# idonahum/photoVerse

Hardware: NVIDIA B200
Metric: images/sec @50 steps 512^2; dual-branch cross-attn TFLOP/s as % of B200 peak (higher is better)
Workload: dtype bf16

## Files before the change

include/photoverse_b200.h:

```cpp
#ifndef PHOTOVERSE_B200_H_
#define PHOTOVERSE_B200_H_

#include <stdint.h>

#ifdef __cplusplus
extern "C" {
#endif

#define PV_ABI_VERSION 2

enum { PV_OK = 0, PV_ERR_INVALID = 1, PV_ERR_CUDA = 2, PV_ERR_UNSUPPORTED = 3 };
typedef enum { PV_F32 = 0, PV_BF16 = 1, PV_F16 = 2 } pv_dtype;

#define PV_KEYS_PAD 96
#define PV_IMG_KEY_OFFSET 80

int pv_version(void);
const char* pv_last_error(void);
unsigned long long pv_launch_count(void);
int pv_set_option(const char* name, int value);
int pv_debug_trace(void* buf, int capacity_events);

int pv_pack_weight(pv_dtype out_dt, const float* W, const float* lora_A, const float* lora_B, float scaling,
                   void* W_eff, int out_features, int in_features, int r, void* stream);

int pv_linear_fwd(pv_dtype dt, pv_dtype out_dt, const void* A, const void* W, const float* bias, void* D,
                  int64_t M, int64_t N, int64_t K, int64_t batch, int64_t lda, int64_t ldw, int64_t ldd,
                  int64_t strideA, int64_t strideW, int64_t strideBias, int64_t strideD, void* stream);

int64_t pv_kv_tile_bytes(pv_dtype dt, int C, int H, int Lt, int Li);
int pv_kv_pack_fwd(pv_dtype dt, const void* text, const void* img, const void* Wkv_text, const void* Wkv_img,
                   float* kv_text_ws, float* kv_img_ws, void* Kp, void* Vp, float* v_ip_norm, int B, int Lt, int Li,
                   int Dc, int C, int H, void* stream);

int64_t pv_dual_attn_sync_words(int B, int S);
int pv_dual_attn_fwd(pv_dtype dt, const void* X, const void* Wq, const void* Kp, const void* Vp, const void* Wo,
                     const float* bo, void* Y, float* ws_q, void* ws_o, float* stats, unsigned int* ws_sync, int B, int S,
                     int C, int H, int Lt, int Li, float w_text, float w_img, void* stream);

int pv_dual_attn_core_fwd(pv_dtype dt, const void* XorQ, const void* Wq, const void* Kp, const void* Vp, void* O,
                          float* stats, int B, int S, int C, int H, int Lt, int Li, float w_text, float w_img,
                          void* stream);

int pv_ln_lrelu_fwd(pv_dtype out_dt, const float* x, const float* gamma, const float* beta, void* y,
                    float* save_mean, float* save_rstd, int64_t rows, int cols, int64_t ldx, int64_t ldy,
                    int64_t rows_per_group, float eps, float slope, void* stream);
int pv_group_mean_fwd(pv_dtype in_dt, pv_dtype out_dt, const void* x, void* y, int64_t groups, int P, int cols,
                      int64_t ldy, void* stream);


int pv_pack_weight_t(pv_dtype out_dt, const float* W, const float* lora_A, const float* lora_B, float scaling,
                     void* W_eff_t, int out_features, int in_features, int r, void* stream);

int pv_transpose_2d(pv_dtype dt, const void* in, void* out, int64_t rows, int64_t cols, int64_t ldi, int64_t ldo, void* stream);

int64_t pv_linear_bwd_weight_ws_bytes(pv_dtype dt, int64_t M, int64_t N, int64_t K);
int pv_linear_bwd_weight(pv_dtype dt, const void* G, const void* X, float* dW, void* ws, int64_t M, int64_t N, int64_t K,
                         int64_t ldg, int64_t ldx, float alpha, float beta, void* stream);

int64_t pv_lora_bwd_ws_bytes(int64_t M, int in_features, int out_features, int r);
int pv_lora_bwd(pv_dtype dt, const void* X, const void* G, const float* lora_A, const float* lora_B, float scaling, float* dAB,
                void* ws, int64_t M, int in_features, int out_features, int r, int64_t ldx, int64_t ldg, void* stream);

int64_t pv_col_sum_ws_bytes(int64_t M, int64_t N);
int pv_col_sum(pv_dtype dt, const void* G, float* out, void* ws, int64_t M, int64_t N, int64_t ldg, void* stream);

int64_t pv_ln_lrelu_bwd_ws_bytes(int64_t groups, int64_t rows_per_group, int cols);
int pv_ln_lrelu_bwd(pv_dtype dt, const void* da, const float* x, const float* mean, const float* rstd, const float* gamma,
                    const float* beta, void* dx, float* dgamma, float* dbeta, void* ws, int64_t groups,
                    int64_t rows_per_group, int cols, float slope, void* stream);

int pv_group_mean_bwd(pv_dtype dt, const void* dy, void* dx, int64_t groups, int P, int cols, int64_t ldy, void* stream);

int64_t pv_dual_attn_bwd_ws_bytes(int B, int S, int C, int H, int Lt, int Li);
int pv_dual_attn_bwd(pv_dtype dt, const void* dO, const void* Q, const float* kv_text, const float* kv_img,
                     const float* stats, void* dQ, void* ws, int B, int S, int C, int H, int Lt, int Li, float w_text,
                     float w_img, void* stream);
int pv_kv_pack_bwd(pv_dtype dt, const void* ws, const float* kv_img, const float* v_ip_norm, const float* d_v_ip_norm,
                   void* dkv_text, void* dkv_img, int B, int S, int Lt, int Li, int C, int H, void* stream);

int pv_inject_concept_fwd(pv_dtype dt, const void* inputs_embeds, const void* concept, const int* placeholder_idx,
                          void* out, int B, int L, int T, int cols, void* stream);
int pv_inject_concept_bwd(pv_dtype dt, const void* d_out, const int* placeholder_idx, void* d_inputs_embeds,
                          void* d_concept, int B, int L, int T, int cols, void* stream);

int64_t pv_train_loss_ws_bytes(void);
int pv_train_loss_fwd(pv_dtype dt, const void* noise_pred, const void* noise, int64_t n, const void* concept, int64_t m,
                      const void* v_ip_norms, int64_t k, float w_text, float w_vis, float* out4, void* ws, void* stream);
int pv_train_loss_bwd(pv_dtype dt, const void* noise_pred, const void* noise, int64_t n, const void* concept, int64_t m, int64_t k,
                      float w_text, float w_vis, const float* d_loss, void* d_noise_pred, void* d_concept, void* d_v_ip_norms,
                      void* stream);

int64_t pv_self_attn_ws_bytes(int B, int S, int C, int heads);
int pv_self_attn_fwd(const void* q, const void* k, const void* v, int64_t ld, void* out, void* ws, int B, int S, int C,
                     int heads, void* stream);

int pv_dropout_bwd_acc(pv_dtype dt, void* dst, const void* src, const uint8_t* keep_mask, float alpha, int64_t n,
                       void* stream);

int64_t pv_group_norm_nhwc_ws_bytes(int64_t B, int64_t HW, int C, int groups);
int pv_group_norm_nhwc_fwd(pv_dtype dt, const void* x, const float* add_bc, const float* gamma, const float* beta, void* y,
                           float* save_stats, void* ws, int64_t B, int64_t HW, int C, int groups, float eps, int silu,
                           void* stream);
int pv_group_norm_nhwc_bwd(pv_dtype dt, const void* x, const float* add_bc, const void* dy, const float* stats,
                           const float* gamma, const float* beta, void* dx, void* ws, int64_t B, int64_t HW, int C, int groups,
                           int silu, void* stream);
int pv_add_bias_nhwc_fwd(pv_dtype dt, const void* a, const void* b, const float* bias, void* out, int64_t rows, int C,
                         void* stream);
int pv_layer_norm_fwd(pv_dtype dt, const void* x, const void* residual, void* sum_out, const float* gamma, const float* beta,
                      void* y, int64_t rows, int C, float eps, void* stream);
int pv_layer_norm_bwd(pv_dtype dt, const void* x, const void* dy, const float* gamma, void* dx, int64_t rows, int C, float eps,
                      void* stream);
int pv_geglu_fwd(pv_dtype dt, const void* h, void* y, int64_t M, int N, int64_t ldh, void* stream);
int pv_geglu_bwd(pv_dtype dt, const void* h, const void* dy, void* dh, int64_t M, int N, int64_t ldh, void* stream);
int pv_linear_geglu_fwd(pv_dtype dt, const void* x, const void* w_packed, const float* b_packed, void* y, int64_t M, int64_t N,
                        int64_t K, int64_t ldx, int64_t ldy, void* stream);

int pv_convert_fwd(pv_dtype in_dt, pv_dtype out_dt, const void* src, void* dst, int64_t n, void* stream);

#ifdef __cplusplus
}
#endif
#endif
```

photoverse_b200/_lib.py:

```python
import ctypes
import os
from ctypes import c_char_p, c_float, c_int, c_int64, c_ulonglong, c_void_p

_HERE = os.path.dirname(os.path.abspath(__file__))
LIB_PATH = os.environ.get("PV_LIB_PATH") or os.path.join(_HERE, "libphotoverse_b200.so")

PV_F32 = 0
PV_BF16 = 1
PV_F16 = 2
PV_KEYS_PAD = 96


class PhotoverseB200Error(RuntimeError):
    pass


_lib = None

_SIGNATURES = {
    "pv_version": (c_int, []),
    "pv_last_error": (c_char_p, []),
    "pv_launch_count": (c_ulonglong, []),
    "pv_set_option": (c_int, [c_char_p, c_int]),
    "pv_debug_trace": (c_int, [c_void_p, c_int]),
    "pv_pack_weight": (c_int, [c_int, c_void_p, c_void_p, c_void_p, c_float, c_void_p, c_int, c_int, c_int, c_void_p]),
    "pv_linear_fwd": (c_int, [c_int, c_int, c_void_p, c_void_p, c_void_p, c_void_p] + [c_int64] * 11 + [c_void_p]),
    "pv_kv_tile_bytes": (c_int64, [c_int, c_int, c_int, c_int, c_int]),
    "pv_kv_pack_fwd": (c_int, [c_int] + [c_void_p] * 9 + [c_int] * 6 + [c_void_p]),
    "pv_dual_attn_sync_words": (c_int64, [c_int, c_int]),
    "pv_dual_attn_fwd": (c_int, [c_int] + [c_void_p] * 11 + [c_int] * 6 + [c_float, c_float, c_void_p]),
    "pv_dual_attn_core_fwd": (c_int, [c_int] + [c_void_p] * 6 + [c_int] * 6 + [c_float, c_float, c_void_p]),
    "pv_ln_lrelu_fwd": (c_int, [c_int] + [c_void_p] * 6 + [c_int64, c_int, c_int64, c_int64, c_int64, c_float, c_float, c_void_p]),
    "pv_group_mean_fwd": (c_int, [c_int, c_int, c_void_p, c_void_p, c_int64, c_int, c_int, c_int64, c_void_p]),
    "pv_inject_concept_fwd": (c_int, [c_int, c_void_p, c_void_p, c_void_p, c_void_p, c_int, c_int, c_int, c_int, c_void_p]),
    "pv_inject_concept_bwd": (c_int, [c_int, c_void_p, c_void_p, c_void_p, c_void_p, c_int, c_int, c_int, c_int, c_void_p]),
    "pv_train_loss_ws_bytes": (c_int64, []),
    "pv_train_loss_fwd": (c_int, [c_int, c_void_p, c_void_p, c_int64, c_void_p, c_int64, c_void_p, c_int64, c_float, c_float, c_void_p,
                                  c_void_p, c_void_p]),
    "pv_train_loss_bwd": (c_int, [c_int, c_void_p, c_void_p, c_int64, c_void_p, c_int64, c_int64, c_float, c_float, c_void_p, c_void_p,
                                  c_void_p, c_void_p, c_void_p]),
    "pv_self_attn_ws_bytes": (c_int64, [c_int, c_int, c_int, c_int]),
    "pv_self_attn_fwd": (c_int, [c_void_p, c_void_p, c_void_p, c_int64, c_void_p, c_void_p, c_int, c_int, c_int, c_int, c_void_p]),
    "pv_dropout_bwd_acc": (c_int, [c_int, c_void_p, c_void_p, c_void_p, c_float, c_int64, c_void_p]),
    "pv_pack_weight_t": (c_int, [c_int, c_void_p, c_void_p, c_void_p, c_float, c_void_p, c_int, c_int, c_int, c_void_p]),
    "pv_transpose_2d": (c_int, [c_int, c_void_p, c_void_p, c_int64, c_int64, c_int64, c_int64, c_void_p]),
    "pv_linear_bwd_weight_ws_bytes": (c_int64, [c_int, c_int64, c_int64, c_int64]),
    "pv_linear_bwd_weight": (c_int, [c_int, c_void_p, c_void_p, c_void_p, c_void_p] + [c_int64] * 5 + [c_float, c_float, c_void_p]),
    "pv_lora_bwd_ws_bytes": (c_int64, [c_int64, c_int, c_int, c_int]),
    "pv_lora_bwd": (c_int, [c_int, c_void_p, c_void_p, c_void_p, c_void_p, c_float, c_void_p, c_void_p, c_int64, c_int, c_int, c_int,
                            c_int64, c_int64, c_void_p]),
    "pv_col_sum_ws_bytes": (c_int64, [c_int64, c_int64]),
    "pv_col_sum": (c_int, [c_int, c_void_p, c_void_p, c_void_p, c_int64, c_int64, c_int64, c_void_p]),
    "pv_ln_lrelu_bwd_ws_bytes": (c_int64, [c_int64, c_int64, c_int]),
    "pv_ln_lrelu_bwd": (c_int, [c_int] + [c_void_p] * 10 + [c_int64, c_int64, c_int, c_float, c_void_p]),
    "pv_group_mean_bwd": (c_int, [c_int, c_void_p, c_void_p, c_int64, c_int, c_int, c_int64, c_void_p]),
    "pv_dual_attn_bwd_ws_bytes": (c_int64, [c_int] * 6),
    "pv_dual_attn_bwd": (c_int, [c_int] + [c_void_p] * 7 + [c_int] * 6 + [c_float, c_float, c_void_p]),
    "pv_kv_pack_bwd": (c_int, [c_int] + [c_void_p] * 6 + [c_int] * 6 + [c_void_p]),
    "pv_group_norm_nhwc_ws_bytes": (c_int64, [c_int64, c_int64, c_int, c_int]),
    "pv_group_norm_nhwc_fwd": (c_int, [c_int] + [c_void_p] * 7 + [c_int64, c_int64, c_int, c_int, c_float, c_int, c_void_p]),
    "pv_group_norm_nhwc_bwd": (c_int, [c_int] + [c_void_p] * 8 + [c_int64, c_int64, c_int, c_int, c_int, c_void_p]),
    "pv_add_bias_nhwc_fwd": (c_int, [c_int, c_void_p, c_void_p, c_void_p, c_void_p, c_int64, c_int, c_void_p]),
    "pv_layer_norm_fwd": (c_int, [c_int, c_void_p, c_void_p, c_void_p, c_void_p, c_void_p, c_void_p, c_int64, c_int, c_float, c_void_p]),
    "pv_layer_norm_bwd": (c_int, [c_int, c_void_p, c_void_p, c_void_p, c_void_p, c_int64, c_int, c_float, c_void_p]),
    "pv_geglu_fwd": (c_int, [c_int, c_void_p, c_void_p, c_int64, c_int, c_int64, c_void_p]),
    "pv_geglu_bwd": (c_int, [c_int, c_void_p, c_void_p, c_void_p, c_int64, c_int, c_int64, c_void_p]),
    "pv_linear_geglu_fwd": (c_int, [c_int, c_void_p, c_void_p, c_void_p, c_void_p] + [c_int64] * 5 + [c_void_p]),
    "pv_convert_fwd": (c_int, [c_int, c_int, c_void_p, c_void_p, c_int64, c_void_p]),
}

REQUIRED_SYMBOLS = list(_SIGNATURES)


def lib() -> ctypes.CDLL:
    global _lib
    if _lib is None:
        if not os.path.exists(LIB_PATH):
            raise PhotoverseB200Error(
                f"{LIB_PATH} is missing: build it with `python -m photoverse_b200.build` "
                "(photoverse_b200 has no CPU / PyTorch fallback)")
        l = ctypes.CDLL(LIB_PATH)
        for name, (res, args) in _SIGNATURES.items():
            try:
                fn = getattr(l, name)
            except AttributeError:
                if name in REQUIRED_SYMBOLS:
                    raise PhotoverseB200Error(f"{LIB_PATH} does not export {name}")
                continue
            fn.restype = res
            fn.argtypes = args
        _lib = l
    return _lib


def check(rc: int, what: str = "") -> None:
    if rc != 0:
        msg = lib().pv_last_error()
        raise PhotoverseB200Error(f"{what or 'photoverse_b200 call'} failed (code {rc}): "
                                  f"{msg.decode() if msg else '?'}")


def launch_count() -> int:
    return int(lib().pv_launch_count())


def set_option(name: str, value: int) -> None:
    check(lib().pv_set_option(name.encode(), int(value)), f"pv_set_option({name})")
```

photoverse_b200/csrc/pv_api.cu:

```cuda
#include <string.h>

#include <mutex>
#include <unordered_map>

#include "pv_host.h"
#include "../../include/photoverse_b200.h"

namespace pv {

int gemm_bf16(const void* A, const void* W, const float* bias, void* D, bool out_f32, long long M, long long N,
              long long K, long long batch, long long lda, long long ldw, long long ldd, long long strideA,
              long long strideW, long long strideBias, long long strideD, cudaStream_t stream, bool w_static = false,
              bool f16 = false);
int gemm_f32(const float* A, const float* W, const float* bias, float* D, long long M, long long N, long long K,
             long long batch, long long lda, long long ldw, long long ldd, long long strideA, long long strideW,
             long long strideBias, long long strideD, cudaStream_t stream);
int dual_attn_core_bf16_persistent(const void* X, const void* Wq, const void* Kp, const void* Vp, void* O, float* stats,
                                   int B, int S, int C, int H, int Lt, int Li, float w_text, float w_img,
                                   cudaStream_t stream, bool f16);
bool dual_attn_pair_roles_supported(int S, int C, int H);
bool dual_attn_pair_roles_fused_supported(int S, int C, int H);
int dual_attn_core_bf16_pair_roles(const void* X, const void* Wq, const void* Kp, const void* Vp, void* O, float* stats,
                                   int B, int S, int C, int H, int Lt, int Li, float w_text, float w_img,
                                   cudaStream_t stream, const void* Wo, const float* bo, void* Y, unsigned int* sync,
                                   bool f16);
int dual_attn_core_bf16_pair(const void* X, const void* Wq, const void* Kp, const void* Vp, void* O, float* stats, int B,
                             int S, int C, int H, int Lt, int Li, float w_text, float w_img, cudaStream_t stream,
                             const void* Wo, const float* bo, void* Y, unsigned int* sync, bool f16);
int dual_attn_core_f32(const float* Q, const float* Kp, const float* Vp, float* O, float* stats, int B, int S, int C,
                       int H, int Lt, int Li, float w_text, float w_img, cudaStream_t stream);
static int64_t attn_kv_tile_bytes(int d) { return static_cast<int64_t>(PV_KEYS_PAD) * ((d + 15) / 16 * 16) * 2; }
int pack_weight(pv_dtype out_dt, const float* W, const float* A, const float* Bm, float scaling, void* out, int out_f,
                int in_f, int r, cudaStream_t stream);
int kv_pack(pv_dtype dt, const float* kv_text, const float* kv_img, void* Kp, void* Vp, float* v_ip_norm, int B, int Lt,
            int Li, int C, int H, cudaStream_t stream);
int ln_lrelu(pv_dtype out_dt, const float* x, const float* gamma, const float* beta, void* y, float* save_mean,
             float* save_rstd, long long rows, int cols, long long ldx, long long ldy, long long rows_per_group,
             float eps, float slope, cudaStream_t stream);
int group_mean(pv_dtype in_dt, pv_dtype out_dt, const void* x, void* y, long long groups, int P, int cols, long long ldy,
               cudaStream_t stream);

int pack_weight_t(bool out_bf16, const float* W, const float* A, const float* Bm, float scaling, void* out, int out_f,
                  int in_f, int r, cudaStream_t stream);
int transpose_2d(bool bf16, const void* in, void* out, long long R, long long Cc, long long ldi, long long ldo, cudaStream_t stream);
long long wgrad_ws_bytes(bool bf16, long long M, long long N, long long K);
int linear_bwd_weight(bool bf16, const void* G, const void* X, float* dW, void* ws, long long M, long long N, long long K,
                      long long ldg, long long ldx, float alpha, float beta, cudaStream_t stream);
long long colsum_ws_bytes(long long M, long long N);
int col_sum(bool bf16, const void* G, float* out, void* ws, long long M, long long N, long long ldg, cudaStream_t stream);
long long ln_bwd_ws_bytes(long long groups, long long rows_per_group, int cols);
int ln_lrelu_bwd(bool bf16, const void* da, const float* x, const float* mean, const float* rstd, const float* gamma,
                 const float* beta, void* dx, float* dgamma, float* dbeta, void* ws, long long groups,
                 long long rows_per_group, int cols, float slope, cudaStream_t stream);
int group_mean_bwd(bool bf16, const void* dy, void* dx, long long groups, int P, int cols, long long ldy, cudaStream_t stream);
int attn_bwd_chunks(int S);
long long self_attn_ws_bytes(int B, int S, int C, int H);
int self_attn_fwd_bf16(const void* q, const void* k, const void* v, long long ld, void* out, void* ws, int B, int S, int C, int H,
                       cudaStream_t stream);
long long train_loss_ws_bytes();
int train_loss_fwd(bool bf16, const void* pred, const void* target, long long n, const void* concept, long long m, const void* vnorm,
                   long long k, float w_text, float w_vis, float* out4, void* ws, cudaStream_t stream);
int train_loss_bwd(bool bf16, const void* pred, const void* target, long long n, const void* concept, long long m, long long k,
                   float w_text, float w_vis, const float* gloss, void* d_pred, void* d_concept, void* d_vnorm, cudaStream_t stream);
bool lora_bwd_supported(int in_f, int out_f, int r);
long long lora_bwd_ws_bytes(long long M, int in_f, int out_f, int r);
int lora_bwd(bool bf16, const void* X, const void* G, const float* A, const float* Bm, float scaling, float* dAB, void* ws,
             long long M, int in_f, int out_f, int r, long long ldx, long long ldg, cudaStream_t stream);
int attn_bwd_chunks_used(bool bf16, int S, int d);
int dual_attn_bwd(bool bf16, const void* dO, const void* Q, const float* kv_text, const float* kv_img, const float* stats,
                  void* dQ, float* part, int B, int S, int C, int H, int Lt, int Li, float w_text, float w_img,
                  cudaStream_t stream);
int kv_pack_bwd(bool bf16, const float* part, const float* kv_img, const float* v_ip_norm, const float* d_vnorm,
                void* dkv_text, void* dkv_img, int nchunk, int B, int Lt, int Li, int C, int H, cudaStream_t stream);

int inject_concept_fwd(bool bf16, const void* in, const void* concept, const int* idx, void* out, int B, int L, int T,
                       int cols, cudaStream_t stream);
int inject_concept_bwd(bool bf16, const void* dout, const int* idx, void* din, void* dconcept, int B, int L, int T, int cols,
                       cudaStream_t stream);
long long group_norm_nhwc_ws_bytes(long long B, long long HW, int C, int G);
int group_norm_nhwc(const void* x, const float* add_bc, const float* gamma, const float* beta, void* y, float* save_stats,
                    void* ws, long long B, long long HW, int C, int G, float eps, bool silu, cudaStream_t stream);
int group_norm_nhwc_bwd(const void* x, const float* add_bc, const void* dy, const float* stats, const float* gamma,
                        const float* beta, void* dx, void* ws, long long B, long long HW, int C, int G, bool silu,
                        cudaStream_t stream);
int add_bias_nhwc(const void* a, const void* b, const float* bias, void* out, long long rows, int C, cudaStream_t stream);
int layer_norm_bf16(const void* x, const void* res, void* sum_out, const float* gamma, const float* beta, void* y, long long rows,
                    int C, float eps, cudaStream_t stream);
int layer_norm_bwd_bf16(const void* x, const void* dy, const float* gamma, void* dx, long long rows, int C, float eps,
                        cudaStream_t stream);
int geglu(const void* h, void* y, long long M, int N, long long ldh, cudaStream_t stream);
int linear_geglu_bf16(const void* x, const void* Wp, const float* bp, void* y, long long M, long long N, long long K,
                      long long ldx, long long ldy, cudaStream_t stream);
int geglu_bwd(const void* h, const void* dy, void* dh, long long M, int N, long long ldh, cudaStream_t stream);
int dropout_bwd_acc(bool bf16, void* dst, const void* src, const uint8_t* mask, float alpha, long long n,
                    cudaStream_t stream);

std::atomic<unsigned long long> g_launches{0};
int g_opt_epi_swizzle = 1;
int g_opt_force_bn = 0;
int g_opt_gemm_two_cta = 1;
int g_opt_pdl = 1;
int g_opt_gemm_persistent = 1;
int g_opt_fuse_out = 1;
int g_opt_bwd_mma = 1;
unsigned long long* g_attn3_trace = nullptr;
int g_attn3_trace_cap = 0;
int g_opt_bwd_tc = 1;
int g_opt_sattn_poly = 2;
int g_opt_attn6_prefetch = 1;
int g_opt_attn6_token = 1;
int g_opt_trace_block = 0;
static thread_local std::string t_error;

void set_error(const std::string& msg) { t_error = msg; }
const char* last_error_cstr() { return t_error.c_str(); }

int sm_count() {
  static std::atomic<int> cache[64];
  int dev = 0;
  if (cudaGetDevice(&dev) != cudaSuccess || dev < 0 || dev >= 64) return 148;
  int n = cache[dev].load(std::memory_order_relaxed);
  if (n == 0) {
    if (cudaDeviceGetAttribute(&n, cudaDevAttrMultiProcessorCount, dev) != cudaSuccess || n <= 0) n = 148;
    cache[dev].store(n, std::memory_order_relaxed);
  }
  return n;
}

cudaError_t set_max_smem_once_impl(const void* kern, int bytes, bool max_carveout) {
  static std::mutex mu;
  static std::unordered_map<uint64_t, int> done;
  int dev = 0;
  cudaError_t e = cudaGetDevice(&dev);
  if (e != cudaSuccess) return e;
  const uint64_t key = reinterpret_cast<uint64_t>(kern) * 131u + static_cast<uint64_t>(dev);
  std::lock_guard<std::mutex> lk(mu);
  auto it = done.find(key);
  if (it != done.end() && it->second >= bytes) return cudaSuccess;
  e = cudaFuncSetAttribute(kern, cudaFuncAttributeMaxDynamicSharedMemorySize, bytes);
  if (e == cudaSuccess && max_carveout)
    e = cudaFuncSetAttribute(kern, cudaFuncAttributePreferredSharedMemoryCarveout, cudaSharedmemCarveoutMaxShared);
  if (e == cudaSuccess) done[key] = bytes;
  return e;
}

typedef CUresult (*EncodeTiledFn)(CUtensorMap*, CUtensorMapDataType, cuuint32_t, void*, const cuuint64_t*,
                                  const cuuint64_t*, const cuuint32_t*, const cuuint32_t*, CUtensorMapInterleave,
                                  CUtensorMapSwizzle, CUtensorMapL2promotion, CUtensorMapFloatOOBfill);

static EncodeTiledFn get_encode_fn() {
  static EncodeTiledFn fn = nullptr;
  static std::once_flag once;
  std::call_once(once, [] {
    void* p = nullptr;
    cudaDriverEntryPointQueryResult qres;
    if (cudaGetDriverEntryPoint("cuTensorMapEncodeTiled", &p, cudaEnableDefault, &qres) == cudaSuccess &&
        qres == cudaDriverEntryPointSuccess)
      fn = reinterpret_cast<EncodeTiledFn>(p);
  });
  return fn;
}

struct TmapKey {
  uint64_t v[12];
  bool operator==(const TmapKey& o) const { return memcmp(v, o.v, sizeof(v)) == 0; }
};
struct TmapKeyHash {
  size_t operator()(const TmapKey& k) const {
    uint64_t h = 1469598103934665603ull;
    for (uint64_t x : k.v) { h ^= x; h *= 1099511628211ull; }
    return static_cast<size_t>(h);
  }
};

int make_tmap_3d(CUtensorMap* out, const void* base, int elem_bytes, uint64_t d0, uint64_t d1, uint64_t d2,
                 uint64_t stride1_bytes, uint64_t stride2_bytes, uint32_t b0, uint32_t b1, uint32_t b2, Swz swz, bool f16) {
  static std::mutex mu;
  static std::unordered_map<TmapKey, CUtensorMap, TmapKeyHash> cache;
  TmapKey key = {{reinterpret_cast<uint64_t>(base), static_cast<uint64_t>(elem_bytes), d0, d1, d2, stride1_bytes,
                  stride2_bytes, b0, b1, b2, static_cast<uint64_t>(swz), static_cast<uint64_t>(f16)}};
  {
    std::lock_guard<std::mutex> lk(mu);
    auto it = cache.find(key);
    if (it != cache.end()) { *out = it->second; return 0; }
  }
  EncodeTiledFn fn = get_encode_fn();
  if (!fn) { set_error("cuTensorMapEncodeTiled unavailable (no CUDA driver / device)"); return 1; }
  CUtensorMapDataType dt = elem_bytes != 2 ? CU_TENSOR_MAP_DATA_TYPE_FLOAT32
                           : f16       ? CU_TENSOR_MAP_DATA_TYPE_FLOAT16 : CU_TENSOR_MAP_DATA_TYPE_BFLOAT16;
  cuuint64_t dims[3] = {d0, d1, d2};
  cuuint64_t strides[2] = {stride1_bytes, stride2_bytes};
  cuuint32_t box[3] = {b0, b1, b2};
  cuuint32_t estr[3] = {1, 1, 1};
  CUtensorMapSwizzle sw = swz == Swz::B128 ? CU_TENSOR_MAP_SWIZZLE_128B
                          : swz == Swz::B64 ? CU_TENSOR_MAP_SWIZZLE_64B : CU_TENSOR_MAP_SWIZZLE_NONE;
  CUresult r = fn(out, dt, 3, const_cast<void*>(base), dims, strides, box, estr, CU_TENSOR_MAP_INTERLEAVE_NONE, sw,
                  CU_TENSOR_MAP_L2_PROMOTION_L2_256B, CU_TENSOR_MAP_FLOAT_OOB_FILL_NONE);
  if (r != CUDA_SUCCESS) {
    char buf[384];
    snprintf(buf, sizeof(buf),
             "cuTensorMapEncodeTiled failed (%d): base=%p elem=%d dims=(%llu,%llu,%llu) strides=(%llu,%llu) box=(%u,%u,%u) swz=%d",
             (int)r, base, elem_bytes, (unsigned long long)d0, (unsigned long long)d1, (unsigned long long)d2,
             (unsigned long long)stride1_bytes, (unsigned long long)stride2_bytes, b0, b1, b2, (int)swz);
    set_error(buf);
    return 1;
  }
  {
    std::lock_guard<std::mutex> lk(mu);
    if (cache.size() > 8192) cache.clear();
    cache.emplace(key, *out);
  }
  return 0;
}

static inline cudaStream_t as_stream(void* s) { return static_cast<cudaStream_t>(s); }
static inline bool is_16bit(pv_dtype dt) { return dt == PV_BF16 || dt == PV_F16; }
#define PV_NO_F16(dt)                                                                                             \
  do {                                                                                                            \
    if ((dt) == PV_F16) PV_FAIL(PV_ERR_UNSUPPORTED, "PV_F16 is not supported (fp16 runs the inference path only)"); \
  } while (0)

static int attn_core_bf16(const void* X, const void* Wq, const void* Kp, const void* Vp, void* O, float* stats, int B,
                          int S, int C, int H, int Lt, int Li, float w_text, float w_img, cudaStream_t st, bool f16,
                          const void* Wo = nullptr, const float* bo = nullptr, void* Y = nullptr, unsigned int* sync = nullptr,
                          bool* fused = nullptr) {
  if (fused) *fused = false;
  if (S > 128) {
    const bool want = Wo != nullptr && sync != nullptr && (g_opt_fuse_out >= 2 || (g_opt_fuse_out == 1 && C <= 320));
    if (dual_attn_pair_roles_supported(S, C, H)) {
      const bool f = want && dual_attn_pair_roles_fused_supported(S, C, H);
      if (fused) *fused = f;
      return dual_attn_core_bf16_pair_roles(X, Wq, Kp, Vp, O, stats, B, S, C, H, Lt, Li, w_text, w_img, st,
                                            f ? Wo : nullptr, bo, f ? Y : nullptr, f ? sync : nullptr, f16);
    }
    if (fused) *fused = want;
    return dual_attn_core_bf16_pair(X, Wq, Kp, Vp, O, stats, B, S, C, H, Lt, Li, w_text, w_img, st, want ? Wo : nullptr, bo,
                                    want ? Y : nullptr, want ? sync : nullptr, f16);
  }
  return dual_attn_core_bf16_persistent(X, Wq, Kp, Vp, O, stats, B, S, C, H, Lt, Li, w_text, w_img, st, f16);
}

}

using namespace pv;

extern "C" {

int pv_version(void) { return PV_ABI_VERSION; }
const char* pv_last_error(void) { return last_error_cstr(); }
unsigned long long pv_launch_count(void) { return g_launches.load(std::memory_order_relaxed); }

int pv_set_option(const char* name, int value) {
  if (!name) PV_FAIL(PV_ERR_INVALID, "null option name");
  if (!strcmp(name, "epi_swizzle")) { g_opt_epi_swizzle = value; return PV_OK; }
  if (!strcmp(name, "force_bn")) { g_opt_force_bn = value; return PV_OK; }
  if (!strcmp(name, "gemm_two_cta")) { g_opt_gemm_two_cta = value; return PV_OK; }
  if (!strcmp(name, "gemm_persistent")) { g_opt_gemm_persistent = value; return PV_OK; }
  if (!strcmp(name, "fuse_out")) { g_opt_fuse_out = value; return PV_OK; }
  if (!strcmp(name, "pdl")) { g_opt_pdl = value; return PV_OK; }
  if (!strcmp(name, "bwd_mma")) { g_opt_bwd_mma = value; return PV_OK; }
  if (!strcmp(name, "bwd_tc")) { g_opt_bwd_tc = value; return PV_OK; }
  if (!strcmp(name, "sattn_poly")) { g_opt_sattn_poly = value; return PV_OK; }
  if (!strcmp(name, "attn6_prefetch")) { g_opt_attn6_prefetch = value; return PV_OK; }
  if (!strcmp(name, "attn6_token")) { g_opt_attn6_token = value; return PV_OK; }
  if (!strcmp(name, "trace_block")) { g_opt_trace_block = value; return PV_OK; }
  PV_FAIL(PV_ERR_INVALID, "unknown option '%s'", name);
}

int pv_debug_trace(void* buf, int capacity_events) {
#ifdef PV_TRACE
  g_attn3_trace = static_cast<unsigned long long*>(buf);
  g_attn3_trace_cap = buf ? capacity_events : 0;
  return PV_OK;
#else
  (void)capacity_events;
  if (buf == nullptr) return PV_OK;
  PV_FAIL(PV_ERR_INVALID, "this build records no device timeline (rebuild with PV_TRACE=1 python -m photoverse_b200.build --force)");
#endif
}

int pv_pack_weight(pv_dtype out_dt, const float* W, const float* lora_A, const float* lora_B, float scaling,
                   void* W_eff, int out_features, int in_features, int r, void* stream) {
  PV_REQUIRE(W && W_eff, "null pointer");
  PV_REQUIRE(out_dt == PV_F32 || is_16bit(out_dt), "unknown dtype %d", (int)out_dt);
  return pack_weight(out_dt, W, lora_A, lora_B, scaling, W_eff, out_features, in_features, r, as_stream(stream));
}

int pv_linear_fwd(pv_dtype dt, pv_dtype out_dt, const void* A, const void* W, const float* bias, void* D, int64_t M,
                  int64_t N, int64_t K, int64_t batch, int64_t lda, int64_t ldw, int64_t ldd, int64_t strideA,
                  int64_t strideW, int64_t strideBias, int64_t strideD, void* stream) {
  PV_REQUIRE(A && W && D, "null pointer");
  if (is_16bit(dt)) {
    PV_REQUIRE(out_dt == dt || out_dt == PV_F32, "%s inputs produce %s or fp32 outputs", dt == PV_F16 ? "PV_F16" : "PV_BF16",
               dt == PV_F16 ? "PV_F16" : "PV_BF16");
    return gemm_bf16(A, W, bias, D, out_dt == PV_F32, M, N, K, batch, lda, ldw, ldd, strideA, strideW, strideBias,
                     strideD, as_stream(stream), false, dt == PV_F16);
  }
  PV_REQUIRE(out_dt == PV_F32, "fp32 inputs produce fp32 outputs");
  return gemm_f32(static_cast<const float*>(A), static_cast<const float*>(W), bias, static_cast<float*>(D), M, N, K,
                  batch, lda, ldw, ldd, strideA, strideW, strideBias, strideD, as_stream(stream));
}

int64_t pv_kv_tile_bytes(pv_dtype dt, int C, int H, int Lt, int Li) {
  if (H <= 0 || C % H != 0) return -1;
  const int d = C / H;
  if (is_16bit(dt)) return attn_kv_tile_bytes(d);
  return static_cast<int64_t>(Lt + Li) * d * 4;
}

int pv_kv_pack_fwd(pv_dtype dt, const void* text, const void* img, const void* Wkv_text, const void* Wkv_img,
                   float* kv_text_ws, float* kv_img_ws, void* Kp, void* Vp, float* v_ip_norm, int B, int Lt, int Li,
                   int Dc, int C, int H, void* stream) {
  PV_REQUIRE(text && img && Wkv_text && Wkv_img && kv_text_ws && kv_img_ws && Kp && Vp && v_ip_norm, "null pointer");
  PV_REQUIRE(B > 0 && Lt >= 1 && Li >= 1 && Lt + Li <= PV_KEYS_PAD && C > 0 && H > 0 && C % H == 0 && Dc > 0,
             "bad shape B=%d Lt=%d Li=%d Dc=%d C=%d H=%d", B, Lt, Li, Dc, C, H);
  PV_REQUIRE(dt == PV_F32 || is_16bit(dt), "unknown dtype %d", (int)dt);
  PV_REQUIRE(!is_16bit(dt) || (Lt <= PV_IMG_KEY_OFFSET && Li <= PV_KEYS_PAD - PV_IMG_KEY_OFFSET),
             "PV_BF16 / PV_F16 tiles hold at most %d text and %d image keys (Lt=%d Li=%d)", PV_IMG_KEY_OFFSET,
             PV_KEYS_PAD - PV_IMG_KEY_OFFSET, Lt, Li);
  cudaStream_t st = as_stream(stream);
  int rc;
  if (is_16bit(dt)) {
    const bool f16 = dt == PV_F16;
    rc = gemm_bf16(text, Wkv_text, nullptr, kv_text_ws, true, (long long)B * Lt, 2 * C, Dc, 1, Dc, Dc, 2 * C, 0, 0, 0, 0, st,
                   false, f16);
    if (rc) return rc;
    rc = gemm_bf16(img, Wkv_img, nullptr, kv_img_ws, true, (long long)B * Li, 2 * C, Dc, 1, Dc, Dc, 2 * C, 0, 0, 0, 0, st,
                   false, f16);
    if (rc) return rc;
  } else {
    rc = gemm_f32(static_cast<const float*>(text), static_cast<const float*>(Wkv_text), nullptr, kv_text_ws,
                  (long long)B * Lt, 2 * C, Dc, 1, Dc, Dc, 2 * C, 0, 0, 0, 0, st);
    if (rc) return rc;
    rc = gemm_f32(static_cast<const float*>(img), static_cast<const float*>(Wkv_img), nullptr, kv_img_ws,
                  (long long)B * Li, 2 * C, Dc, 1, Dc, Dc, 2 * C, 0, 0, 0, 0, st);
    if (rc) return rc;
  }
  return kv_pack(dt, kv_text_ws, kv_img_ws, Kp, Vp, v_ip_norm, B, Lt, Li, C, H, st);
}

int64_t pv_dual_attn_sync_words(int B, int S) {
  if (B <= 0 || S <= 0) return -1;
  return 2ll * B * ((S + 255) / 256);
}

int pv_dual_attn_fwd(pv_dtype dt, const void* X, const void* Wq, const void* Kp, const void* Vp, const void* Wo,
                     const float* bo, void* Y, float* ws_q, void* ws_o, float* stats, unsigned int* ws_sync, int B, int S,
                     int C, int H, int Lt, int Li, float w_text, float w_img, void* stream) {
  PV_REQUIRE(X && Wq && Kp && Vp && Wo && Y && ws_o, "null pointer");
  cudaStream_t st = as_stream(stream);
  int rc;
  if (is_16bit(dt)) {
    const bool f16 = dt == PV_F16;
    bool fused = false;
    rc = attn_core_bf16(X, Wq, Kp, Vp, ws_o, stats, B, S, C, H, Lt, Li, w_text, w_img, st, f16, Wo, bo, Y, ws_sync, &fused);
    if (rc || fused) return rc;
    return gemm_bf16(ws_o, Wo, bo, Y, false, (long long)B * S, C, C, 1, C, C, C, 0, 0, 0, 0, st, true, f16);
  }
  PV_REQUIRE(dt == PV_F32, "unknown dtype %d", (int)dt);
  PV_REQUIRE(ws_q != nullptr, "PV_F32 needs the ws_q scratch");
  rc = gemm_f32(static_cast<const float*>(X), static_cast<const float*>(Wq), nullptr, ws_q, (long long)B * S, C, C, 1, C,
                C, C, 0, 0, 0, 0, st);
  if (rc) return rc;
  rc = dual_attn_core_f32(ws_q, static_cast<const float*>(Kp), static_cast<const float*>(Vp),
                          static_cast<float*>(ws_o), stats, B, S, C, H, Lt, Li, w_text, w_img, st);
  if (rc) return rc;
  return gemm_f32(static_cast<const float*>(ws_o), static_cast<const float*>(Wo), bo, static_cast<float*>(Y),
                  (long long)B * S, C, C, 1, C, C, C, 0, 0, 0, 0, st);
}

int pv_dual_attn_core_fwd(pv_dtype dt, const void* XorQ, const void* Wq, const void* Kp, const void* Vp, void* O,
                          float* stats, int B, int S, int C, int H, int Lt, int Li, float w_text, float w_img,
                          void* stream) {
  PV_REQUIRE(XorQ && Kp && Vp && O, "null pointer");
  if (is_16bit(dt)) {
    PV_REQUIRE(Wq != nullptr, "PV_BF16 / PV_F16 fuse the Q projection: Wq required");
    return attn_core_bf16(XorQ, Wq, Kp, Vp, O, stats, B, S, C, H, Lt, Li, w_text, w_img, as_stream(stream), dt == PV_F16);
  }
  PV_REQUIRE(dt == PV_F32, "unknown dtype %d", (int)dt);
  return dual_attn_core_f32(static_cast<const float*>(XorQ), static_cast<const float*>(Kp),
                            static_cast<const float*>(Vp), static_cast<float*>(O), stats, B, S, C, H, Lt, Li, w_text,
                            w_img, as_stream(stream));
}

int pv_ln_lrelu_fwd(pv_dtype out_dt, const float* x, const float* gamma, const float* beta, void* y, float* save_mean,
                    float* save_rstd, int64_t rows, int cols, int64_t ldx, int64_t ldy, int64_t rows_per_group,
                    float eps, float slope, void* stream) {
  PV_REQUIRE(x && gamma && beta && y, "null pointer");
  PV_REQUIRE(out_dt == PV_F32 || is_16bit(out_dt), "unknown dtype %d", (int)out_dt);
  return ln_lrelu(out_dt, x, gamma, beta, y, save_mean, save_rstd, rows, cols, ldx, ldy, rows_per_group, eps,
                  slope, as_stream(stream));
}

int pv_group_mean_fwd(pv_dtype in_dt, pv_dtype out_dt, const void* x, void* y, int64_t groups, int P, int cols,
                      int64_t ldy, void* stream) {
  PV_REQUIRE(x && y, "null pointer");
  PV_REQUIRE((in_dt == PV_F32 || is_16bit(in_dt)) && (out_dt == PV_F32 || is_16bit(out_dt)), "unknown dtype");
  PV_REQUIRE(!(is_16bit(in_dt) && is_16bit(out_dt) && in_dt != out_dt), "16-bit input and output must have one type");
  return group_mean(in_dt, out_dt, x, y, groups, P, cols, ldy, as_stream(stream));
}

int pv_pack_weight_t(pv_dtype out_dt, const float* W, const float* lora_A, const float* lora_B, float scaling,
                     void* W_eff_t, int out_features, int in_features, int r, void* stream) {
  PV_NO_F16(out_dt);
  PV_REQUIRE(W && W_eff_t, "null pointer");
  return pack_weight_t(out_dt == PV_BF16, W, lora_A, lora_B, scaling, W_eff_t, out_features, in_features, r, as_stream(stream));
}

int pv_transpose_2d(pv_dtype dt, const void* in, void* out, int64_t rows, int64_t cols, int64_t ldi, int64_t ldo, void* stream) {
  PV_NO_F16(dt);
  PV_REQUIRE(in && out, "null pointer");
  return transpose_2d(dt == PV_BF16, in, out, rows, cols, ldi, ldo, as_stream(stream));
}

int64_t pv_linear_bwd_weight_ws_bytes(pv_dtype dt, int64_t M, int64_t N, int64_t K) {
  if (dt == PV_F16) { set_error("pv_linear_bwd_weight_ws_bytes: PV_F16 is not supported (fp16 runs the inference path only)"); return -1; }
  return wgrad_ws_bytes(dt == PV_BF16, M, N, K);
}

int pv_linear_bwd_weight(pv_dtype dt, const void* G, const void* X, float* dW, void* ws, int64_t M, int64_t N, int64_t K,
                         int64_t ldg, int64_t ldx, float alpha, float beta, void* stream) {
  PV_NO_F16(dt);
  PV_REQUIRE(G && X && dW, "null pointer");
  return linear_bwd_weight(dt == PV_BF16, G, X, dW, ws, M, N, K, ldg, ldx, alpha, beta, as_stream(stream));
}

int64_t pv_lora_bwd_ws_bytes(int64_t M, int in_features, int out_features, int r) {
  if (M <= 0 || !lora_bwd_supported(in_features, out_features, r)) return -1;
  return lora_bwd_ws_bytes(M, in_features, out_features, r);
}

int pv_lora_bwd(pv_dtype dt, const void* X, const void* G, const float* lora_A, const float* lora_B, float scaling, float* dAB,
                void* ws, int64_t M, int in_features, int out_features, int r, int64_t ldx, int64_t ldg, void* stream) {
  PV_NO_F16(dt);
  PV_REQUIRE(X && G && lora_A && lora_B && dAB, "null pointer");
  return lora_bwd(dt == PV_BF16, X, G, lora_A, lora_B, scaling, dAB, ws, M, in_features, out_features, r, ldx, ldg, as_stream(stream));
}

int64_t pv_col_sum_ws_bytes(int64_t M, int64_t N) { return colsum_ws_bytes(M, N); }

int pv_col_sum(pv_dtype dt, const void* G, float* out, void* ws, int64_t M, int64_t N, int64_t ldg, void* stream) {
  PV_NO_F16(dt);
  PV_REQUIRE(G && out, "null pointer");
  return col_sum(dt == PV_BF16, G, out, ws, M, N, ldg, as_stream(stream));
}

int64_t pv_ln_lrelu_bwd_ws_bytes(int64_t groups, int64_t rows_per_group, int cols) {
  return ln_bwd_ws_bytes(groups, rows_per_group, cols);
}

int pv_ln_lrelu_bwd(pv_dtype dt, const void* da, const float* x, const float* mean, const float* rstd, const float* gamma,
                    const float* beta, void* dx, float* dgamma, float* dbeta, void* ws, int64_t groups,
                    int64_t rows_per_group, int cols, float slope, void* stream) {
  PV_NO_F16(dt);
  PV_REQUIRE(da && x && mean && rstd && gamma && beta && dx && dgamma && dbeta && ws, "null pointer");
  return ln_lrelu_bwd(dt == PV_BF16, da, x, mean, rstd, gamma, beta, dx, dgamma, dbeta, ws, groups, rows_per_group, cols,
                      slope, as_stream(stream));
}

int pv_group_mean_bwd(pv_dtype dt, const void* dy, void* dx, int64_t groups, int P, int cols, int64_t ldy, void* stream) {
  PV_NO_F16(dt);
  PV_REQUIRE(dy && dx, "null pointer");
  return group_mean_bwd(dt == PV_BF16, dy, dx, groups, P, cols, ldy, as_stream(stream));
}

int64_t pv_dual_attn_bwd_ws_bytes(int B, int S, int C, int H, int Lt, int Li) {
  if (H <= 0 || C % H != 0) return -1;
  return static_cast<int64_t>(attn_bwd_chunks(S)) * B * H * 2 * (Lt + Li) * (C / H) * 4;
}

int pv_dual_attn_bwd(pv_dtype dt, const void* dO, const void* Q, const float* kv_text, const float* kv_img,
                     const float* stats, void* dQ, void* ws, int B, int S, int C, int H, int Lt, int Li, float w_text,
                     float w_img, void* stream) {
  PV_NO_F16(dt);
  PV_REQUIRE(dO && Q && kv_text && kv_img && stats && dQ && ws, "null pointer");
  return dual_attn_bwd(dt == PV_BF16, dO, Q, kv_text, kv_img, stats, dQ, static_cast<float*>(ws), B, S, C, H, Lt, Li, w_text,
                       w_img, as_stream(stream));
}

int pv_kv_pack_bwd(pv_dtype dt, const void* ws, const float* kv_img, const float* v_ip_norm, const float* d_v_ip_norm,
                   void* dkv_text, void* dkv_img, int B, int S, int Lt, int Li, int C, int H, void* stream) {
  PV_NO_F16(dt);
  PV_REQUIRE(ws && kv_img && v_ip_norm && dkv_text && dkv_img, "null pointer");
  return kv_pack_bwd(dt == PV_BF16, static_cast<const float*>(ws), kv_img, v_ip_norm, d_v_ip_norm, dkv_text, dkv_img,
                     attn_bwd_chunks_used(dt == PV_BF16, S, H > 0 ? C / H : 0), B, Lt, Li, C, H, as_stream(stream));
}

int pv_inject_concept_fwd(pv_dtype dt, const void* inputs_embeds, const void* concept, const int* placeholder_idx,
                          void* out, int B, int L, int T, int cols, void* stream) {
  PV_NO_F16(dt);
  PV_REQUIRE(inputs_embeds && concept && placeholder_idx && out, "null pointer");
  return inject_concept_fwd(dt == PV_BF16, inputs_embeds, concept, placeholder_idx, out, B, L, T, cols, as_stream(stream));
}

int pv_inject_concept_bwd(pv_dtype dt, const void* d_out, const int* placeholder_idx, void* d_inputs_embeds,
                          void* d_concept, int B, int L, int T, int cols, void* stream) {
  PV_NO_F16(dt);
  PV_REQUIRE(d_out && placeholder_idx && d_inputs_embeds && d_concept, "null pointer");
  return inject_concept_bwd(dt == PV_BF16, d_out, placeholder_idx, d_inputs_embeds, d_concept, B, L, T, cols, as_stream(stream));
}

int64_t pv_train_loss_ws_bytes(void) { return train_loss_ws_bytes(); }

int pv_train_loss_fwd(pv_dtype dt, const void* noise_pred, const void* noise, int64_t n, const void* concept, int64_t m,
                      const void* v_ip_norms, int64_t k, float w_text, float w_vis, float* out4, void* ws, void* stream) {
  PV_NO_F16(dt);
  PV_REQUIRE(noise_pred && noise && out4 && (m == 0 || concept) && (k == 0 || v_ip_norms), "null pointer");
  return train_loss_fwd(dt == PV_BF16, noise_pred, noise, n, concept, m, v_ip_norms, k, w_text, w_vis, out4, ws, as_stream(stream));
}

int pv_train_loss_bwd(pv_dtype dt, const void* noise_pred, const void* noise, int64_t n, const void* concept, int64_t m, int64_t k,
                      float w_text, float w_vis, const float* d_loss, void* d_noise_pred, void* d_concept, void* d_v_ip_norms,
                      void* stream) {
  PV_NO_F16(dt);
  PV_REQUIRE(noise_pred && noise && d_loss && d_noise_pred && (m == 0 || (concept && d_concept)) && (k == 0 || d_v_ip_norms), "null pointer");
  return train_loss_bwd(dt == PV_BF16, noise_pred, noise, n, concept, m, k, w_text, w_vis, d_loss, d_noise_pred, d_concept,
                        d_v_ip_norms, as_stream(stream));
}

int64_t pv_self_attn_ws_bytes(int B, int S, int C, int heads) { return self_attn_ws_bytes(B, S, C, heads); }

int pv_self_attn_fwd(const void* q, const void* k, const void* v, int64_t ld, void* out, void* ws, int B, int S, int C,
                     int heads, void* stream) {
  PV_REQUIRE(q && k && v && out && ws, "null pointer");
  return self_attn_fwd_bf16(q, k, v, ld, out, ws, B, S, C, heads, as_stream(stream));
}

int pv_dropout_bwd_acc(pv_dtype dt, void* dst, const void* src, const uint8_t* keep_mask, float alpha, int64_t n,
                       void* stream) {
  PV_NO_F16(dt);
  PV_REQUIRE(dst && src && keep_mask, "null pointer");
  return dropout_bwd_acc(dt == PV_BF16, dst, src, keep_mask, alpha, n, as_stream(stream));
}

int64_t pv_group_norm_nhwc_ws_bytes(int64_t B, int64_t HW, int C, int groups) { return group_norm_nhwc_ws_bytes(B, HW, C, groups); }

int pv_group_norm_nhwc_fwd(pv_dtype dt, const void* x, const float* add_bc, const float* gamma, const float* beta, void* y,
                           float* save_stats, void* ws, int64_t B, int64_t HW, int C, int groups, float eps, int silu,
                           void* stream) {
  PV_NO_F16(dt);
  PV_REQUIRE(x && gamma && beta && y && ws, "null pointer");
  PV_REQUIRE(dt == PV_BF16, "bf16 activations only (the fp32 parity mode keeps the stock GroupNorm)");
  return group_norm_nhwc(x, add_bc, gamma, beta, y, save_stats, ws, B, HW, C, groups, eps, silu != 0, as_stream(stream));
}

int pv_group_norm_nhwc_bwd(pv_dtype dt, const void* x, const float* add_bc, const void* dy, const float* stats,
                           const float* gamma, const float* beta, void* dx, void* ws, int64_t B, int64_t HW, int C, int groups,
                           int silu, void* stream) {
  PV_NO_F16(dt);
  PV_REQUIRE(x && dy && stats && gamma && beta && dx && ws, "null pointer");
  PV_REQUIRE(dt == PV_BF16, "bf16 activations only");
  return group_norm_nhwc_bwd(x, add_bc, dy, stats, gamma, beta, dx, ws, B, HW, C, groups, silu != 0, as_stream(stream));
}

int pv_add_bias_nhwc_fwd(pv_dtype dt, const void* a, const void* b, const float* bias, void* out, int64_t rows, int C,
                         void* stream) {
  PV_NO_F16(dt);
  PV_REQUIRE(a && b && bias && out, "null pointer");
  PV_REQUIRE(dt == PV_BF16, "bf16 activations only");
  return add_bias_nhwc(a, b, bias, out, rows, C, as_stream(stream));
}

int pv_layer_norm_fwd(pv_dtype dt, const void* x, const void* residual, void* sum_out, const float* gamma, const float* beta,
                      void* y, int64_t rows, int C, float eps, void* stream) {
  PV_NO_F16(dt);
  PV_REQUIRE(x && gamma && beta && y, "null pointer");
  PV_REQUIRE(dt == PV_BF16, "bf16 activations only");
  return layer_norm_bf16(x, residual, sum_out, gamma, beta, y, rows, C, eps, as_stream(stream));
}

int pv_layer_norm_bwd(pv_dtype dt, const void* x, const void* dy, const float* gamma, void* dx, int64_t rows, int C, float eps,
                      void* stream) {
  PV_NO_F16(dt);
  PV_REQUIRE(x && dy && gamma && dx, "null pointer");
  PV_REQUIRE(dt == PV_BF16, "bf16 activations only");
  return layer_norm_bwd_bf16(x, dy, gamma, dx, rows, C, eps, as_stream(stream));
}

int pv_geglu_fwd(pv_dtype dt, const void* h, void* y, int64_t M, int N, int64_t ldh, void* stream) {
  PV_NO_F16(dt);
  PV_REQUIRE(h && y, "null pointer");
  PV_REQUIRE(dt == PV_BF16, "bf16 activations only");
  return geglu(h, y, M, N, ldh, as_stream(stream));
}

int pv_geglu_bwd(pv_dtype dt, const void* h, const void* dy, void* dh, int64_t M, int N, int64_t ldh, void* stream) {
  PV_NO_F16(dt);
  PV_REQUIRE(h && dy && dh, "null pointer");
  PV_REQUIRE(dt == PV_BF16, "bf16 activations only");
  return geglu_bwd(h, dy, dh, M, N, ldh, as_stream(stream));
}

int pv_linear_geglu_fwd(pv_dtype dt, const void* x, const void* w_packed, const float* b_packed, void* y, int64_t M, int64_t N,
                        int64_t K, int64_t ldx, int64_t ldy, void* stream) {
  PV_NO_F16(dt);
  PV_REQUIRE(x && w_packed && y, "null pointer");
  PV_REQUIRE(dt == PV_BF16, "bf16 activations only");
  return linear_geglu_bf16(x, w_packed, b_packed, y, M, N, K, ldx, ldy, as_stream(stream));
}

}
```

photoverse_b200/csrc/pv_backbone.cu:

```cuda
#include "pv_common.cuh"
#include "pv_host.h"
#include "../../include/photoverse_b200.h"

namespace pv {

constexpr int GN_THREADS_MAX = 512;
constexpr int GN_MAX_G = 64;
constexpr int GN_UNROLL = 4;

__device__ __forceinline__ void bf16x8_unpack(const uint4& v, float* f) {
  const uint32_t w[4] = {v.x, v.y, v.z, v.w};
#pragma unroll
  for (int i = 0; i < 4; ++i) {
    f[2 * i] = __uint_as_float(w[i] << 16);
    f[2 * i + 1] = __uint_as_float(w[i] & 0xffff0000u);
  }
}
__device__ __forceinline__ uint4 bf16x8_pack(const float* f) {
  uint32_t w[4];
#pragma unroll
  for (int i = 0; i < 4; ++i) {
    const __nv_bfloat162 p = __floats2bfloat162_rn(f[2 * i], f[2 * i + 1]);
    w[i] = *reinterpret_cast<const uint32_t*>(&p);
  }
  return make_uint4(w[0], w[1], w[2], w[3]);
}

__global__ void __launch_bounds__(GN_THREADS_MAX)
gn_stats_nhwc_kernel(const __nv_bfloat16* __restrict__ x, const float* __restrict__ addv, float* __restrict__ part,
                     long long HW, int C, int G, int rows_per_cta, int k) {
  extern __shared__ float gn_smem[];
  const int vecs = C >> 3;
  const int v = threadIdx.x % vecs;
  const int pl = threadIdx.x / vecs;
  const int b = blockIdx.y;
  const int cpg = C / G;
  const __nv_bfloat16* xb = x + static_cast<size_t>(b) * HW * C;
  float shift[8];
#pragma unroll
  for (int j = 0; j < 8; ++j) {
    const int c = v * 8 + j, c0 = (c / cpg) * cpg;
    shift[j] = __bfloat162float(xb[c0]);
    if (addv != nullptr) shift[j] += addv[static_cast<size_t>(b) * C + c0] - addv[static_cast<size_t>(b) * C + c];
  }
  float s[8], q[8];
#pragma unroll
  for (int j = 0; j < 8; ++j) s[j] = q[j] = 0.f;
  const long long p0 = static_cast<long long>(blockIdx.x) * rows_per_cta;
  const long long p1 = p0 + rows_per_cta < HW ? p0 + rows_per_cta : HW;
  const uint4* xv = reinterpret_cast<const uint4*>(xb);
  for (long long p = p0 + pl; p < p1; p += static_cast<long long>(GN_UNROLL) * k) {
    uint4 raw[GN_UNROLL];
#pragma unroll
    for (int u = 0; u < GN_UNROLL; ++u) {
      const long long pp = p + static_cast<long long>(u) * k;
      if (pp < p1) raw[u] = __ldg(xv + pp * vecs + v);
    }
#pragma unroll
    for (int u = 0; u < GN_UNROLL; ++u) {
      if (p + static_cast<long long>(u) * k < p1) {
        float f[8];
        bf16x8_unpack(raw[u], f);
#pragma unroll
        for (int j = 0; j < 8; ++j) {
          const float d = f[j] - shift[j];
          s[j] += d;
          q[j] = fmaf(d, d, q[j]);
        }
      }
    }
  }
  float* ss = gn_smem;
  float* sq = gn_smem + k * C;
#pragma unroll
  for (int j = 0; j < 8; ++j) {
    ss[pl * C + v * 8 + j] = s[j];
    sq[pl * C + v * 8 + j] = q[j];
  }
  __syncthreads();
  for (int c = threadIdx.x; c < C; c += blockDim.x) {
    float a = 0.f, d = 0.f;
    for (int l = 0; l < k; ++l) {
      a += ss[l * C + c];
      d += sq[l * C + c];
    }
    ss[c] = a;
    sq[c] = d;
  }
  __syncthreads();
  for (int g = threadIdx.x; g < G; g += blockDim.x) {
    float a = 0.f, d = 0.f;
    for (int c = g * cpg; c < (g + 1) * cpg; ++c) {
      a += ss[c];
      d += sq[c];
    }
    float* o = part + ((static_cast<size_t>(b) * gridDim.x + blockIdx.x) * G + g) * 2;
    o[0] = a;
    o[1] = d;
  }
}

template <bool SILU>
__global__ void __launch_bounds__(GN_THREADS_MAX)
gn_apply_nhwc_kernel(const __nv_bfloat16* __restrict__ x, const float* __restrict__ addv, const float* __restrict__ part,
                     const float* __restrict__ gamma, const float* __restrict__ beta, __nv_bfloat16* __restrict__ y,
                     float* __restrict__ save_stats, long long HW, int C, int G, int stat_chunks, int rows_per_cta, int k,
                     float eps) {
  __shared__ float s_mean[GN_MAX_G], s_rstd[GN_MAX_G];
  const int vecs = C >> 3;
  const int v = threadIdx.x % vecs;
  const int pl = threadIdx.x / vecs;
  const int b = blockIdx.y;
  const int cpg = C / G;
  const __nv_bfloat16* xb = x + static_cast<size_t>(b) * HW * C;
  for (int g = threadIdx.x; g < G; g += blockDim.x) {
    float a = 0.f, d = 0.f;
    const float* pp = part + (static_cast<size_t>(b) * stat_chunks * G + g) * 2;
    for (int c = 0; c < stat_chunks; ++c) {
      a += pp[static_cast<size_t>(c) * G * 2];
      d += pp[static_cast<size_t>(c) * G * 2 + 1];
    }
    const float n = static_cast<float>(HW) * static_cast<float>(cpg);
    const float m = a / n;
    const float var = fmaxf(d / n - m * m, 0.f);
    s_mean[g] = __bfloat162float(xb[g * cpg]) + (addv != nullptr ? addv[static_cast<size_t>(b) * C + g * cpg] : 0.f) + m;
    s_rstd[g] = rsqrtf(var + eps);
    if (save_stats != nullptr && blockIdx.x == 0) {
      save_stats[(static_cast<size_t>(b) * G + g) * 2] = s_mean[g];
      save_stats[(static_cast<size_t>(b) * G + g) * 2 + 1] = s_rstd[g];
    }
  }
  __syncthreads();
  float sc[8], sf[8];
#pragma unroll
  for (int j = 0; j < 8; ++j) {
    const int c = v * 8 + j;
    const int g = c / cpg;
    sc[j] = __ldg(gamma + c) * s_rstd[g];
    const float a = addv != nullptr ? addv[static_cast<size_t>(b) * C + c] : 0.f;
    sf[j] = fmaf(a - s_mean[g], sc[j], __ldg(beta + c));
  }
  const long long p0 = static_cast<long long>(blockIdx.x) * rows_per_cta;
  const long long p1 = p0 + rows_per_cta < HW ? p0 + rows_per_cta : HW;
  const uint4* xv = reinterpret_cast<const uint4*>(xb);
  uint4* yv = reinterpret_cast<uint4*>(y + static_cast<size_t>(b) * HW * C);
  for (long long p = p0 + pl; p < p1; p += static_cast<long long>(GN_UNROLL) * k) {
    uint4 raw[GN_UNROLL];
#pragma unroll
    for (int u = 0; u < GN_UNROLL; ++u) {
      const long long pp = p + static_cast<long long>(u) * k;
      if (pp < p1) raw[u] = __ldg(xv + pp * vecs + v);
    }
#pragma unroll
    for (int u = 0; u < GN_UNROLL; ++u) {
      const long long pp = p + static_cast<long long>(u) * k;
      if (pp < p1) {
        float f[8];
        bf16x8_unpack(raw[u], f);
#pragma unroll
        for (int j = 0; j < 8; ++j) {
          float t = fmaf(f[j], sc[j], sf[j]);
          if (SILU) t = __fdividef(t, 1.f + __expf(-t));
          f[j] = t;
        }
        yv[pp * vecs + v] = bf16x8_pack(f);
      }
    }
  }
}

static void gn_geometry(long long B, long long HW, int C, int* k, int* chunks, int* rows_per_cta) {
  (void)B;
  const int vecs = C / 8;
  int kk = GN_THREADS_MAX / vecs;
  if (kk < 1) kk = 1;
  if (kk > 16) kk = 16;
  if (kk > HW) kk = static_cast<int>(HW);
  long long rows = (65536 + 2ll * C - 1) / (2ll * C);
  rows = (rows + kk - 1) / kk * kk;
  if (rows > HW) rows = (HW + kk - 1) / kk * kk;
  *k = kk;
  *rows_per_cta = static_cast<int>(rows);
  *chunks = static_cast<int>((HW + rows - 1) / rows);
}

long long group_norm_nhwc_ws_bytes(long long B, long long HW, int C, int G) {
  if (B <= 0 || HW <= 0 || C <= 0 || G <= 0 || C % 8 != 0 || C % G != 0 || G > GN_MAX_G || C / 8 > GN_THREADS_MAX) return -1;
  int k, chunks, rows;
  gn_geometry(B, HW, C, &k, &chunks, &rows);
  return B * chunks * G * 2ll * static_cast<long long>(sizeof(float));
}

int group_norm_nhwc(const void* x, const float* add_bc, const float* gamma, const float* beta, void* y, float* save_stats,
                    void* ws, long long B, long long HW, int C, int G, float eps, bool silu, cudaStream_t stream) {
  PV_REQUIRE(group_norm_nhwc_ws_bytes(B, HW, C, G) >= 0,
             "need C %% 8 == 0, C %% G == 0, G <= %d, C <= %d (B=%lld HW=%lld C=%d G=%d)", GN_MAX_G, 8 * GN_THREADS_MAX, B, HW, C, G);
  PV_REQUIRE(B <= 65535, "batch too large for one launch (B=%lld)", B);
  PV_REQUIRE((reinterpret_cast<uintptr_t>(x) | reinterpret_cast<uintptr_t>(y)) % 16 == 0, "x / y must be 16-byte aligned");
  int k, chunks, rows;
  gn_geometry(B, HW, C, &k, &chunks, &rows);
  const int threads = (C / 8) * k;
  const size_t smem = 2ull * k * C * sizeof(float);
  auto stats = gn_stats_nhwc_kernel;
  if (smem > 48 * 1024) PV_CUDA(set_max_smem_once(stats, static_cast<int>(smem)));
  stats<<<dim3(chunks, static_cast<unsigned>(B)), threads, smem, stream>>>(static_cast<const __nv_bfloat16*>(x), add_bc,
                                                                            static_cast<float*>(ws), HW, C, G, rows, k);
  PV_LAUNCHED();
  if (silu)
    gn_apply_nhwc_kernel<true><<<dim3(chunks, static_cast<unsigned>(B)), threads, 0, stream>>>(
        static_cast<const __nv_bfloat16*>(x), add_bc, static_cast<const float*>(ws), gamma, beta, static_cast<__nv_bfloat16*>(y),
        save_stats, HW, C, G, chunks, rows, k, eps);
  else
    gn_apply_nhwc_kernel<false><<<dim3(chunks, static_cast<unsigned>(B)), threads, 0, stream>>>(
        static_cast<const __nv_bfloat16*>(x), add_bc, static_cast<const float*>(ws), gamma, beta, static_cast<__nv_bfloat16*>(y),
        save_stats, HW, C, G, chunks, rows, k, eps);
  PV_LAUNCHED();
  return PV_OK;
}

struct GnBwdChan {
  float g[8], bt[8], xs[8], xo[8];
};
__device__ __forceinline__ void gn_bwd_chan(GnBwdChan& ch, const float* __restrict__ stats, const float* __restrict__ addv,
                                            const float* __restrict__ gamma, const float* __restrict__ beta, int b, int v,
                                            int C, int G, int cpg) {
#pragma unroll
  for (int j = 0; j < 8; ++j) {
    const int c = v * 8 + j;
    const int g = c / cpg;
    const float mean = stats[(static_cast<size_t>(b) * G + g) * 2], rstd = stats[(static_cast<size_t>(b) * G + g) * 2 + 1];
    const float a = addv != nullptr ? addv[static_cast<size_t>(b) * C + c] : 0.f;
    ch.g[j] = __ldg(gamma + c);
    ch.bt[j] = __ldg(beta + c);
    ch.xs[j] = rstd;
    ch.xo[j] = (a - mean) * rstd;
  }
}
template <bool SILU>
__device__ __forceinline__ float gn_dz(float dy, float z) {
  if (!SILU) return dy;
  const float sg = __fdividef(1.f, 1.f + __expf(-z));
  return dy * sg * fmaf(z, 1.f - sg, 1.f);
}

template <bool SILU>
__global__ void __launch_bounds__(GN_THREADS_MAX)
gn_bwd_stats_nhwc_kernel(const __nv_bfloat16* __restrict__ x, const float* __restrict__ addv, const __nv_bfloat16* __restrict__ dy,
                         const float* __restrict__ stats, const float* __restrict__ gamma, const float* __restrict__ beta,
                         float* __restrict__ part, long long HW, int C, int G, int rows_per_cta, int k) {
  extern __shared__ float gn_smem[];
  const int vecs = C >> 3;
  const int v = threadIdx.x % vecs;
  const int pl = threadIdx.x / vecs;
  const int b = blockIdx.y;
  const int cpg = C / G;
  GnBwdChan ch;
  gn_bwd_chan(ch, stats, addv, gamma, beta, b, v, C, G, cpg);
  float s[8], q[8];
#pragma unroll
  for (int j = 0; j < 8; ++j) s[j] = q[j] = 0.f;
  const long long p0 = static_cast<long long>(blockIdx.x) * rows_per_cta;
  const long long p1 = p0 + rows_per_cta < HW ? p0 + rows_per_cta : HW;
  const uint4* xv = reinterpret_cast<const uint4*>(x + static_cast<size_t>(b) * HW * C);
  const uint4* dv = reinterpret_cast<const uint4*>(dy + static_cast<size_t>(b) * HW * C);
  for (long long p = p0 + pl; p < p1; p += 2ll * k) {
    uint4 rx[2], rd[2];
#pragma unroll
    for (int u = 0; u < 2; ++u) {
      const long long pp = p + static_cast<long long>(u) * k;
      if (pp < p1) {
        rx[u] = __ldg(xv + pp * vecs + v);
        rd[u] = __ldg(dv + pp * vecs + v);
      }
    }
#pragma unroll
    for (int u = 0; u < 2; ++u) {
      if (p + static_cast<long long>(u) * k < p1) {
        float f[8], d[8];
        bf16x8_unpack(rx[u], f);
        bf16x8_unpack(rd[u], d);
#pragma unroll
        for (int j = 0; j < 8; ++j) {
          const float xh = fmaf(f[j], ch.xs[j], ch.xo[j]);
          const float t = gn_dz<SILU>(d[j], fmaf(xh, ch.g[j], ch.bt[j])) * ch.g[j];
          s[j] += t;
          q[j] = fmaf(t, xh, q[j]);
        }
      }
    }
  }
  float* ss = gn_smem;
  float* sq = gn_smem + k * C;
#pragma unroll
  for (int j = 0; j < 8; ++j) {
    ss[pl * C + v * 8 + j] = s[j];
    sq[pl * C + v * 8 + j] = q[j];
  }
  __syncthreads();
  for (int c = threadIdx.x; c < C; c += blockDim.x) {
    float a = 0.f, d = 0.f;
    for (int l = 0; l < k; ++l) {
      a += ss[l * C + c];
      d += sq[l * C + c];
    }
    ss[c] = a;
    sq[c] = d;
  }
  __syncthreads();
  for (int g = threadIdx.x; g < G; g += blockDim.x) {
    float a = 0.f, d = 0.f;
    for (int c = g * cpg; c < (g + 1) * cpg; ++c) {
      a += ss[c];
      d += sq[c];
    }
    float* o = part + ((static_cast<size_t>(b) * gridDim.x + blockIdx.x) * G + g) * 2;
    o[0] = a;
    o[1] = d;
  }
}

template <bool SILU>
__global__ void __launch_bounds__(GN_THREADS_MAX)
gn_bwd_apply_nhwc_kernel(const __nv_bfloat16* __restrict__ x, const float* __restrict__ addv, const __nv_bfloat16* __restrict__ dy,
                         const float* __restrict__ stats, const float* __restrict__ part, const float* __restrict__ gamma,
                         const float* __restrict__ beta, __nv_bfloat16* __restrict__ dx, long long HW, int C, int G,
                         int stat_chunks, int rows_per_cta, int k) {
  __shared__ float s_m1[GN_MAX_G], s_m2[GN_MAX_G];
  const int vecs = C >> 3;
  const int v = threadIdx.x % vecs;
  const int pl = threadIdx.x / vecs;
  const int b = blockIdx.y;
  const int cpg = C / G;
  for (int g = threadIdx.x; g < G; g += blockDim.x) {
    float a = 0.f, d = 0.f;
    const float* pp = part + (static_cast<size_t>(b) * stat_chunks * G + g) * 2;
    for (int c = 0; c < stat_chunks; ++c) {
      a += pp[static_cast<size_t>(c) * G * 2];
      d += pp[static_cast<size_t>(c) * G * 2 + 1];
    }
    const float n = static_cast<float>(HW) * static_cast<float>(cpg);
    s_m1[g] = a / n;
    s_m2[g] = d / n;
  }
  GnBwdChan ch;
  gn_bwd_chan(ch, stats, addv, gamma, beta, b, v, C, G, cpg);
  __syncthreads();
  float m1[8], m2[8];
#pragma unroll
  for (int j = 0; j < 8; ++j) {
    const int g = (v * 8 + j) / cpg;
    m1[j] = s_m1[g];
    m2[j] = s_m2[g];
  }
  const long long p0 = static_cast<long long>(blockIdx.x) * rows_per_cta;
  const long long p1 = p0 + rows_per_cta < HW ? p0 + rows_per_cta : HW;
  const uint4* xv = reinterpret_cast<const uint4*>(x + static_cast<size_t>(b) * HW * C);
  const uint4* dv = reinterpret_cast<const uint4*>(dy + static_cast<size_t>(b) * HW * C);
  uint4* ov = reinterpret_cast<uint4*>(dx + static_cast<size_t>(b) * HW * C);
  for (long long p = p0 + pl; p < p1; p += 2ll * k) {
    uint4 rx[2], rd[2];
#pragma unroll
    for (int u = 0; u < 2; ++u) {
      const long long pp = p + static_cast<long long>(u) * k;
      if (pp < p1) {
        rx[u] = __ldg(xv + pp * vecs + v);
        rd[u] = __ldg(dv + pp * vecs + v);
      }
    }
#pragma unroll
    for (int u = 0; u < 2; ++u) {
      const long long pp = p + static_cast<long long>(u) * k;
      if (pp < p1) {
        float f[8], d[8];
        bf16x8_unpack(rx[u], f);
        bf16x8_unpack(rd[u], d);
#pragma unroll
        for (int j = 0; j < 8; ++j) {
          const float xh = fmaf(f[j], ch.xs[j], ch.xo[j]);
          const float t = gn_dz<SILU>(d[j], fmaf(xh, ch.g[j], ch.bt[j])) * ch.g[j];
          f[j] = ch.xs[j] * (t - m1[j] - xh * m2[j]);
        }
        ov[pp * vecs + v] = bf16x8_pack(f);
      }
    }
  }
}

int group_norm_nhwc_bwd(const void* x, const float* add_bc, const void* dy, const float* stats, const float* gamma,
                        const float* beta, void* dx, void* ws, long long B, long long HW, int C, int G, bool silu,
                        cudaStream_t stream) {
  PV_REQUIRE(group_norm_nhwc_ws_bytes(B, HW, C, G) >= 0,
             "need C %% 8 == 0, C %% G == 0, G <= %d, C <= %d (B=%lld HW=%lld C=%d G=%d)", GN_MAX_G, 8 * GN_THREADS_MAX, B, HW, C, G);
  PV_REQUIRE(B <= 65535, "batch too large for one launch (B=%lld)", B);
  PV_REQUIRE((reinterpret_cast<uintptr_t>(x) | reinterpret_cast<uintptr_t>(dy) | reinterpret_cast<uintptr_t>(dx)) % 16 == 0,
             "x / dy / dx must be 16-byte aligned");
  int k, chunks, rows;
  gn_geometry(B, HW, C, &k, &chunks, &rows);
  const int threads = (C / 8) * k;
  const size_t smem = 2ull * k * C * sizeof(float);
  const dim3 grid(chunks, static_cast<unsigned>(B));
  const __nv_bfloat16* xx = static_cast<const __nv_bfloat16*>(x);
  const __nv_bfloat16* dd = static_cast<const __nv_bfloat16*>(dy);
  if (silu) {
    gn_bwd_stats_nhwc_kernel<true><<<grid, threads, smem, stream>>>(xx, add_bc, dd, stats, gamma, beta, static_cast<float*>(ws), HW, C, G, rows, k);
    PV_LAUNCHED();
    gn_bwd_apply_nhwc_kernel<true><<<grid, threads, 0, stream>>>(xx, add_bc, dd, stats, static_cast<const float*>(ws), gamma, beta,
                                                                 static_cast<__nv_bfloat16*>(dx), HW, C, G, chunks, rows, k);
  } else {
    gn_bwd_stats_nhwc_kernel<false><<<grid, threads, smem, stream>>>(xx, add_bc, dd, stats, gamma, beta, static_cast<float*>(ws), HW, C, G, rows, k);
    PV_LAUNCHED();
    gn_bwd_apply_nhwc_kernel<false><<<grid, threads, 0, stream>>>(xx, add_bc, dd, stats, static_cast<const float*>(ws), gamma, beta,
                                                                  static_cast<__nv_bfloat16*>(dx), HW, C, G, chunks, rows, k);
  }
  PV_LAUNCHED();
  return PV_OK;
}

__global__ void __launch_bounds__(256)
add_bias_nhwc_kernel(const __nv_bfloat16* a, const __nv_bfloat16* b, const float* __restrict__ bias, __nv_bfloat16* out,
                     long long rows, int C) {
  const int vecs = C >> 3;
  const long long total = rows * vecs;
  for (long long i = static_cast<long long>(blockIdx.x) * blockDim.x + threadIdx.x; i < total;
       i += static_cast<long long>(gridDim.x) * blockDim.x) {
    const int v = static_cast<int>(i % vecs);
    float fa[8], fb[8];
    bf16x8_unpack(reinterpret_cast<const uint4*>(a)[i], fa);
    bf16x8_unpack(reinterpret_cast<const uint4*>(b)[i], fb);
    const float4 b0 = __ldg(reinterpret_cast<const float4*>(bias) + 2 * v), b1 = __ldg(reinterpret_cast<const float4*>(bias) + 2 * v + 1);
    const float bb[8] = {b0.x, b0.y, b0.z, b0.w, b1.x, b1.y, b1.z, b1.w};
#pragma unroll
    for (int j = 0; j < 8; ++j) fa[j] = fa[j] + (fb[j] + bb[j]);
    reinterpret_cast<uint4*>(out)[i] = bf16x8_pack(fa);
  }
}

int add_bias_nhwc(const void* a, const void* b, const float* bias, void* out, long long rows, int C, cudaStream_t stream) {
  PV_REQUIRE(rows > 0 && C > 0 && C % 8 == 0, "need C %% 8 == 0 (rows=%lld C=%d)", rows, C);
  PV_REQUIRE((reinterpret_cast<uintptr_t>(a) | reinterpret_cast<uintptr_t>(b) | reinterpret_cast<uintptr_t>(out) |
              reinterpret_cast<uintptr_t>(bias)) % 16 == 0, "pointers must be 16-byte aligned");
  const long long total = rows * (C / 8);
  long long blocks = (total + 255) / 256;
  const long long cap = 8ll * sm_count();
  if (blocks > cap) blocks = cap;
  add_bias_nhwc_kernel<<<static_cast<unsigned>(blocks), 256, 0, stream>>>(static_cast<const __nv_bfloat16*>(a), static_cast<const __nv_bfloat16*>(b),
                                                                         bias, static_cast<__nv_bfloat16*>(out), rows, C);
  PV_LAUNCHED();
  return PV_OK;
}

template <int NV>
__global__ void __launch_bounds__(256)
layer_norm_bf16_kernel(const __nv_bfloat16* __restrict__ x, const __nv_bfloat16* __restrict__ res,
                       __nv_bfloat16* __restrict__ sum_out, const float* __restrict__ gamma, const float* __restrict__ beta,
                       __nv_bfloat16* __restrict__ y, long long rows, int C, float eps) {
  const long long row = static_cast<long long>(blockIdx.x) * (blockDim.x >> 5) + (threadIdx.x >> 5);
  if (row >= rows) return;
  const int lane = threadIdx.x & 31;
  const int vecs = C >> 3;
  const uint4* xr = reinterpret_cast<const uint4*>(x + row * C);
  float f[NV][8];
  float s = 0.f;
#pragma unroll
  for (int i = 0; i < NV; ++i) {
    const int idx = i * 32 + lane;
    if (idx < vecs) {
      bf16x8_unpack(__ldg(xr + idx), f[i]);
      if (res != nullptr) {
        float r[8];
        bf16x8_unpack(__ldg(reinterpret_cast<const uint4*>(res + row * C) + idx), r);
#pragma unroll
        for (int j = 0; j < 8; ++j) f[i][j] += r[j];
        const uint4 packed = bf16x8_pack(f[i]);
        reinterpret_cast<uint4*>(sum_out + row * C)[idx] = packed;
        bf16x8_unpack(packed, f[i]);
      }
#pragma unroll
      for (int j = 0; j < 8; ++j) s += f[i][j];
    }
  }
#pragma unroll
  for (int o = 16; o > 0; o >>= 1) s += __shfl_xor_sync(0xffffffffu, s, o);
  const float mean = s / static_cast<float>(C);
  float ss = 0.f;
#pragma unroll
  for (int i = 0; i < NV; ++i) {
    if (i * 32 + lane < vecs) {
#pragma unroll
      for (int j = 0; j < 8; ++j) {
        const float d = f[i][j] - mean;
        ss = fmaf(d, d, ss);
      }
    }
  }
#pragma unroll
  for (int o = 16; o > 0; o >>= 1) ss += __shfl_xor_sync(0xffffffffu, ss, o);
  const float rstd = rsqrtf(ss / static_cast<float>(C) + eps);
  uint4* yr = reinterpret_cast<uint4*>(y + row * C);
#pragma unroll
  for (int i = 0; i < NV; ++i) {
    const int idx = i * 32 + lane;
    if (idx < vecs) {
      const float4 g0 = __ldg(reinterpret_cast<const float4*>(gamma) + 2 * idx), g1 = __ldg(reinterpret_cast<const float4*>(gamma) + 2 * idx + 1);
      const float4 b0 = __ldg(reinterpret_cast<const float4*>(beta) + 2 * idx), b1 = __ldg(reinterpret_cast<const float4*>(beta) + 2 * idx + 1);
      const float gg[8] = {g0.x, g0.y, g0.z, g0.w, g1.x, g1.y, g1.z, g1.w};
      const float bb[8] = {b0.x, b0.y, b0.z, b0.w, b1.x, b1.y, b1.z, b1.w};
      float o[8];
#pragma unroll
      for (int j = 0; j < 8; ++j) o[j] = fmaf((f[i][j] - mean) * rstd, gg[j], bb[j]);
      yr[idx] = bf16x8_pack(o);
    }
  }
}

int layer_norm_bf16(const void* x, const void* res, void* sum_out, const float* gamma, const float* beta, void* y, long long rows,
                    int C, float eps, cudaStream_t stream) {
  PV_REQUIRE(rows > 0 && C > 0 && C % 8 == 0 && C <= 8 * 32 * 5, "need C %% 8 == 0 and C <= 1280 (rows=%lld C=%d)", rows, C);
  PV_REQUIRE((res == nullptr) == (sum_out == nullptr), "res and sum_out go together");
  PV_REQUIRE((reinterpret_cast<uintptr_t>(x) | reinterpret_cast<uintptr_t>(y) | reinterpret_cast<uintptr_t>(gamma) |
              reinterpret_cast<uintptr_t>(beta) | reinterpret_cast<uintptr_t>(res) | reinterpret_cast<uintptr_t>(sum_out)) % 16 == 0,
             "pointers must be 16-byte aligned");
  const int nv = (C / 8 + 31) / 32;
  const unsigned blocks = static_cast<unsigned>((rows + 7) / 8);
  const __nv_bfloat16* xx = static_cast<const __nv_bfloat16*>(x);
  const __nv_bfloat16* rr = static_cast<const __nv_bfloat16*>(res);
  __nv_bfloat16* so = static_cast<__nv_bfloat16*>(sum_out);
  __nv_bfloat16* yy = static_cast<__nv_bfloat16*>(y);
  switch (nv) {
    case 1: layer_norm_bf16_kernel<1><<<blocks, 256, 0, stream>>>(xx, rr, so, gamma, beta, yy, rows, C, eps); break;
    case 2: layer_norm_bf16_kernel<2><<<blocks, 256, 0, stream>>>(xx, rr, so, gamma, beta, yy, rows, C, eps); break;
    case 3: layer_norm_bf16_kernel<3><<<blocks, 256, 0, stream>>>(xx, rr, so, gamma, beta, yy, rows, C, eps); break;
    case 4: layer_norm_bf16_kernel<4><<<blocks, 256, 0, stream>>>(xx, rr, so, gamma, beta, yy, rows, C, eps); break;
    default: layer_norm_bf16_kernel<5><<<blocks, 256, 0, stream>>>(xx, rr, so, gamma, beta, yy, rows, C, eps); break;
  }
  PV_LAUNCHED();
  return PV_OK;
}

template <int NV>
__global__ void __launch_bounds__(256)
layer_norm_bwd_bf16_kernel(const __nv_bfloat16* __restrict__ x, const __nv_bfloat16* __restrict__ dy, const float* __restrict__ gamma,
                           __nv_bfloat16* __restrict__ dx, long long rows, int C, float eps) {
  const long long row = static_cast<long long>(blockIdx.x) * (blockDim.x >> 5) + (threadIdx.x >> 5);
  if (row >= rows) return;
  const int lane = threadIdx.x & 31;
  const int vecs = C >> 3;
  const uint4* xr = reinterpret_cast<const uint4*>(x + row * C);
  const uint4* dr = reinterpret_cast<const uint4*>(dy + row * C);
  float f[NV][8], t[NV][8];
  float s = 0.f;
#pragma unroll
  for (int i = 0; i < NV; ++i) {
    const int idx = i * 32 + lane;
    if (idx < vecs) {
      bf16x8_unpack(__ldg(xr + idx), f[i]);
      bf16x8_unpack(__ldg(dr + idx), t[i]);
#pragma unroll
      for (int j = 0; j < 8; ++j) s += f[i][j];
    }
  }
#pragma unroll
  for (int o = 16; o > 0; o >>= 1) s += __shfl_xor_sync(0xffffffffu, s, o);
  const float mean = s / static_cast<float>(C);
  float ss = 0.f;
#pragma unroll
  for (int i = 0; i < NV; ++i) {
    if (i * 32 + lane < vecs) {
#pragma unroll
      for (int j = 0; j < 8; ++j) {
        const float d = f[i][j] - mean;
        ss = fmaf(d, d, ss);
      }
    }
  }
#pragma unroll
  for (int o = 16; o > 0; o >>= 1) ss += __shfl_xor_sync(0xffffffffu, ss, o);
  const float rstd = rsqrtf(ss / static_cast<float>(C) + eps);
  float s1 = 0.f, s2 = 0.f;
#pragma unroll
  for (int i = 0; i < NV; ++i) {
    const int idx = i * 32 + lane;
    if (idx < vecs) {
      const float4 g0 = __ldg(reinterpret_cast<const float4*>(gamma) + 2 * idx), g1 = __ldg(reinterpret_cast<const float4*>(gamma) + 2 * idx + 1);
      const float gg[8] = {g0.x, g0.y, g0.z, g0.w, g1.x, g1.y, g1.z, g1.w};
#pragma unroll
      for (int j = 0; j < 8; ++j) {
        f[i][j] = (f[i][j] - mean) * rstd;
        t[i][j] *= gg[j];
        s1 += t[i][j];
        s2 = fmaf(t[i][j], f[i][j], s2);
      }
    }
  }
#pragma unroll
  for (int o = 16; o > 0; o >>= 1) {
    s1 += __shfl_xor_sync(0xffffffffu, s1, o);
    s2 += __shfl_xor_sync(0xffffffffu, s2, o);
  }
  const float m1 = s1 / static_cast<float>(C), m2 = s2 / static_cast<float>(C);
  uint4* outr = reinterpret_cast<uint4*>(dx + row * C);
#pragma unroll
  for (int i = 0; i < NV; ++i) {
    const int idx = i * 32 + lane;
    if (idx < vecs) {
      float o[8];
#pragma unroll
      for (int j = 0; j < 8; ++j) o[j] = rstd * (t[i][j] - m1 - f[i][j] * m2);
      outr[idx] = bf16x8_pack(o);
    }
  }
}

int layer_norm_bwd_bf16(const void* x, const void* dy, const float* gamma, void* dx, long long rows, int C, float eps,
                        cudaStream_t stream) {
  PV_REQUIRE(rows > 0 && C > 0 && C % 8 == 0 && C <= 8 * 32 * 5, "need C %% 8 == 0 and C <= 1280 (rows=%lld C=%d)", rows, C);
  PV_REQUIRE((reinterpret_cast<uintptr_t>(x) | reinterpret_cast<uintptr_t>(dy) | reinterpret_cast<uintptr_t>(dx) |
              reinterpret_cast<uintptr_t>(gamma)) % 16 == 0, "pointers must be 16-byte aligned");
  const int nv = (C / 8 + 31) / 32;
  const unsigned blocks = static_cast<unsigned>((rows + 7) / 8);
  const __nv_bfloat16* xx = static_cast<const __nv_bfloat16*>(x);
  const __nv_bfloat16* dd = static_cast<const __nv_bfloat16*>(dy);
  __nv_bfloat16* oo = static_cast<__nv_bfloat16*>(dx);
  switch (nv) {
    case 1: layer_norm_bwd_bf16_kernel<1><<<blocks, 256, 0, stream>>>(xx, dd, gamma, oo, rows, C, eps); break;
    case 2: layer_norm_bwd_bf16_kernel<2><<<blocks, 256, 0, stream>>>(xx, dd, gamma, oo, rows, C, eps); break;
    case 3: layer_norm_bwd_bf16_kernel<3><<<blocks, 256, 0, stream>>>(xx, dd, gamma, oo, rows, C, eps); break;
    case 4: layer_norm_bwd_bf16_kernel<4><<<blocks, 256, 0, stream>>>(xx, dd, gamma, oo, rows, C, eps); break;
    default: layer_norm_bwd_bf16_kernel<5><<<blocks, 256, 0, stream>>>(xx, dd, gamma, oo, rows, C, eps); break;
  }
  PV_LAUNCHED();
  return PV_OK;
}

__global__ void __launch_bounds__(256)
geglu_kernel(const __nv_bfloat16* __restrict__ h, __nv_bfloat16* __restrict__ y, long long M, int N, long long ldh) {
  const int vecs = N >> 3;
  const long long total = M * vecs;
  for (long long i = static_cast<long long>(blockIdx.x) * blockDim.x + threadIdx.x; i < total;
       i += static_cast<long long>(gridDim.x) * blockDim.x) {
    const long long m = i / vecs;
    const int v = static_cast<int>(i - m * vecs);
    const uint4* row = reinterpret_cast<const uint4*>(h + m * ldh);
    float a[8], g[8];
    bf16x8_unpack(__ldg(row + v), a);
    bf16x8_unpack(__ldg(row + vecs + v), g);
#pragma unroll
    for (int j = 0; j < 8; ++j) {
      const float ge = __bfloat162float(__float2bfloat16_rn(0.5f * g[j] * (1.f + erff(g[j] * 0.70710678118654752f))));
      a[j] *= ge;
    }
    reinterpret_cast<uint4*>(y + m * N)[v] = bf16x8_pack(a);
  }
}

int geglu(const void* h, void* y, long long M, int N, long long ldh, cudaStream_t stream) {
  PV_REQUIRE(M > 0 && N > 0 && N % 8 == 0 && ldh >= 2ll * N && ldh % 8 == 0, "need N %% 8 == 0 and ldh >= 2N, ldh %% 8 == 0 (M=%lld N=%d ldh=%lld)", M, N, ldh);
  PV_REQUIRE((reinterpret_cast<uintptr_t>(h) | reinterpret_cast<uintptr_t>(y)) % 16 == 0, "h / y must be 16-byte aligned");
  const long long total = M * (N / 8);
  long long blocks = (total + 255) / 256;
  const long long cap = 8ll * sm_count();
  if (blocks > cap) blocks = cap;
  geglu_kernel<<<static_cast<unsigned>(blocks), 256, 0, stream>>>(static_cast<const __nv_bfloat16*>(h), static_cast<__nv_bfloat16*>(y), M, N, ldh);
  PV_LAUNCHED();
  return PV_OK;
}

__global__ void __launch_bounds__(256)
geglu_bwd_kernel(const __nv_bfloat16* __restrict__ h, const __nv_bfloat16* __restrict__ dy, __nv_bfloat16* __restrict__ dh,
                 long long M, int N, long long ldh) {
  const int vecs = N >> 3;
  const long long total = M * vecs;
  for (long long i = static_cast<long long>(blockIdx.x) * blockDim.x + threadIdx.x; i < total;
       i += static_cast<long long>(gridDim.x) * blockDim.x) {
    const long long m = i / vecs;
    const int v = static_cast<int>(i - m * vecs);
    const uint4* row = reinterpret_cast<const uint4*>(h + m * ldh);
    float a[8], g[8], d[8];
    bf16x8_unpack(__ldg(row + v), a);
    bf16x8_unpack(__ldg(row + vecs + v), g);
    bf16x8_unpack(__ldg(reinterpret_cast<const uint4*>(dy + m * N) + v), d);
#pragma unroll
    for (int j = 0; j < 8; ++j) {
      const float cdf = 0.5f * (1.f + erff(g[j] * 0.70710678118654752f));
      const float pdf = 0.3989422804014327f * __expf(-0.5f * g[j] * g[j]);
      const float da = d[j] * (g[j] * cdf);
      const float dg = d[j] * a[j] * fmaf(g[j], pdf, cdf);
      a[j] = da;
      g[j] = dg;
    }
    uint4* orow = reinterpret_cast<uint4*>(dh + m * 2 * N);
    orow[v] = bf16x8_pack(a);
    orow[vecs + v] = bf16x8_pack(g);
  }
}

int geglu_bwd(const void* h, const void* dy, void* dh, long long M, int N, long long ldh, cudaStream_t stream) {
  PV_REQUIRE(M > 0 && N > 0 && N % 8 == 0 && ldh >= 2ll * N && ldh % 8 == 0, "need N %% 8 == 0 and ldh >= 2N, ldh %% 8 == 0 (M=%lld N=%d ldh=%lld)", M, N, ldh);
  PV_REQUIRE((reinterpret_cast<uintptr_t>(h) | reinterpret_cast<uintptr_t>(dy) | reinterpret_cast<uintptr_t>(dh)) % 16 == 0,
             "h / dy / dh must be 16-byte aligned");
  const long long total = M * (N / 8);
  long long blocks = (total + 255) / 256;
  const long long cap = 8ll * sm_count();
  if (blocks > cap) blocks = cap;
  geglu_bwd_kernel<<<static_cast<unsigned>(blocks), 256, 0, stream>>>(static_cast<const __nv_bfloat16*>(h), static_cast<const __nv_bfloat16*>(dy),
                                                                     static_cast<__nv_bfloat16*>(dh), M, N, ldh);
  PV_LAUNCHED();
  return PV_OK;
}

}
```

photoverse_b200/csrc/pv_gemm3.cu:

```cuda
#include "pv_common.cuh"
#include "pv_outproj.cuh"
#include "pv_host.h"
#include "../../include/photoverse_b200.h"

namespace pv {

constexpr int G3_THREADS = 384;

template <typename Cfg, int EPI, typename T>
__global__ void __cluster_dims__(2, 1, 1) __launch_bounds__(G3_THREADS, 1)
gemm3_pair_persistent_kernel(const __grid_constant__ CUtensorMap tmA, const __grid_constant__ CUtensorMap tmW,
                             const __grid_constant__ CUtensorMap tmD, const float* __restrict__ bias, int G, int V, int K,
                             int w_static) {
  extern __shared__ uint8_t smem_raw[];
  uint8_t* smem = reinterpret_cast<uint8_t*>((reinterpret_cast<uintptr_t>(smem_raw) + 1023) & ~uintptr_t(1023));
  uint64_t* bars = reinterpret_cast<uint64_t*>(smem + (Cfg::BYTES + 15) / 16 * 16);
  uint32_t* tmem_slot = reinterpret_cast<uint32_t*>(bars + OP_BAR_BYTES / 8 + (EPI == OP_EPI_GEGLU ? 1 : 0));
  const int warp = threadIdx.x >> 5;
  const int pair = blockIdx.x >> 1;
  const int npairs = gridDim.x >> 1;
  int g, u0, u1;
  if constexpr (EPI == OP_EPI_GEGLU) {
    const long long T = static_cast<long long>(G) * V;
    u0 = static_cast<int>(T * pair / npairs);
    u1 = static_cast<int>(T * (pair + 1) / npairs);
    g = u0 / V;
  } else {
    g = pair % G;
    const int r_pair = pair / G;
    const int npair_g = (npairs - g + G - 1) / G;
    u0 = static_cast<int>((static_cast<long long>(V) * r_pair) / npair_g);
    u1 = static_cast<int>((static_cast<long long>(V) * (r_pair + 1)) / npair_g);
  }

  if (warp == 0 && (threadIdx.x & 31) == 0) {
    tma_prefetch_desc(&tmA);
    tma_prefetch_desc(&tmW);
    tma_prefetch_desc(&tmD);
    op_mbar_init(bars);
    if constexpr (EPI == OP_EPI_GEGLU) mbar_init(bars + OP_W_FREE, 1);
    fence_barrier_init();
  }
  if (warp == 2) tmem_alloc_2sm<512>(tmem_slot);
  tc_fence_before();
  __syncthreads();
  cluster_sync_all();
  tc_fence_after();
  const uint32_t tmem = *tmem_slot;
  if constexpr (Cfg::WSTAT) {
    if (w_static && warp == 0 && u0 < u1) {
      if (elect_one()) op_preload_w<Cfg>(smem, bars, &tmW, g, cluster_ctarank());
      __syncwarp();
    }
  }
  pdl_wait();
  pdl_launch_dependents();

  OutProjArgs oa;
  oa.bias = bias;
  oa.sync = nullptr;
  oa.G = G; oa.C = K; oa.V = V;
  oa.MTP = V > 0 ? V : 1;
  oa.u0 = u0;
  oa.u1 = u1;
  oa.g = g;
  oa.ready_target = 0;
  oa.w_preloaded = Cfg::WSTAT && w_static && u0 < u1;
  oa.trace = nullptr; oa.trace_cap = 0; oa.trace_block = 0;
  outproj_phase<Cfg, EPI, T>(smem, bars, tmem, &tmA, &tmW, &tmD, oa);

  tc_fence_before();
  __syncthreads();
  cluster_sync_all();
  tc_fence_after();
  if (warp == 2) tmem_dealloc_2sm<512>(tmem);
}

template <int KB_RES, int STAGES, int EPI, typename T>
static int launch_g3(const CUtensorMap& tmA, const CUtensorMap& tmW, const CUtensorMap& tmD, const float* bias, int G, int V,
                     int K, int w_static, cudaStream_t stream) {
  using Cfg = OutProjCfg<KB_RES, STAGES>;
  constexpr int SMEM_BYTES = (Cfg::BYTES + 15) / 16 * 16 + 256 + 1024;
  static_assert(OP_BAR_BYTES + 8 + 8 <= 256 && SMEM_BYTES <= 227 * 1024, "shared memory budget");
  auto kern = gemm3_pair_persistent_kernel<Cfg, EPI, T>;
  PV_CUDA(set_max_smem_once(kern, SMEM_BYTES));
  const long long units = static_cast<long long>(G) * V;
  const long long max_pairs = sm_count() / 2;
  const int npairs = static_cast<int>(units < max_pairs ? units : max_pairs);
  PV_CUDA(launch_pdl(kern, dim3(2 * npairs), dim3(G3_THREADS), SMEM_BYTES, stream, tmA, tmW, tmD, bias, G, V, K, w_static));
  PV_LAUNCHED();
  return PV_OK;
}

int gemm3_bf16(const void* A, const void* W, const float* bias, void* D, long long M, long long N, long long K, long long lda,
               long long ldw, long long ldd, cudaStream_t stream, bool w_static, bool f16) {
  PV_REQUIRE(M > 0 && N % OP_BN == 0 && K % OP_BK == 0 && N > 0 && K > 0, "gemm3: need N %% 160 == 0 and K %% 64 == 0 (N=%lld K=%lld)", N, K);
  PV_REQUIRE((lda * 2) % 16 == 0 && (ldw * 2) % 16 == 0 && (ldd * 2) % 16 == 0, "row strides must be 16-byte multiples");
  CUtensorMap tmA, tmW, tmD;
  if (make_tmap_3d(&tmA, A, 2, K, M, 1, lda * 2, lda * M * 2, OP_BK, 128, 1, Swz::B128, f16)) return PV_ERR_CUDA;
  if (make_tmap_3d(&tmW, W, 2, K, N, 1, ldw * 2, ldw * N * 2, OP_BK, OP_BN / 2, 1, Swz::B128, f16)) return PV_ERR_CUDA;
  if (make_tmap_3d(&tmD, D, 2, N, M, 1, ldd * 2, ldd * M * 2, 80, 32, 1, Swz::None, f16)) return PV_ERR_CUDA;
  const int G = static_cast<int>(N / OP_BN);
  const long long V = (M + 255) / 256;
  PV_REQUIRE(V * G < (1ll << 30), "too many tiles");
#define PV_G3(KB, ST)                                                                                                    \
  (f16 ? launch_g3<KB, ST, OP_EPI_BIAS, __half>(tmA, tmW, tmD, bias, G, static_cast<int>(V), static_cast<int>(K), w_static, stream) \
       : launch_g3<KB, ST, OP_EPI_BIAS, __nv_bfloat16>(tmA, tmW, tmD, bias, G, static_cast<int>(V), static_cast<int>(K), w_static, stream))
  if (K == 320) return PV_G3(5, 8);
  if (K == 640) return PV_G3(10, 5);
  return PV_G3(0, 7);
#undef PV_G3
}

int linear_geglu_bf16(const void* x, const void* Wp, const float* bp, void* y, long long M, long long N, long long K,
                      long long ldx, long long ldy, cudaStream_t stream) {
  PV_REQUIRE(M > 0 && N > 0 && K > 0 && N % (OP_BN / 2) == 0 && K % OP_BK == 0,
             "linear_geglu: need M > 0, N %% 80 == 0 and K %% 64 == 0 (M=%lld N=%lld K=%lld)", M, N, K);
  PV_REQUIRE(ldx >= K && ldy >= N && ldx % 8 == 0 && ldy % 8 == 0, "linear_geglu: row strides must be >= the row and 16-byte multiples (ldx=%lld ldy=%lld)", ldx, ldy);
  PV_REQUIRE((reinterpret_cast<uintptr_t>(x) | reinterpret_cast<uintptr_t>(Wp) | reinterpret_cast<uintptr_t>(y)) % 16 == 0,
             "linear_geglu: pointers must be 16-byte aligned");
  const long long G = 2 * N / OP_BN;
  const long long V = (M + 255) / 256;
  PV_REQUIRE(V * G < (1ll << 30), "too many tiles");
  CUtensorMap tmA, tmW, tmD;
  if (make_tmap_3d(&tmA, x, 2, K, M, 1, ldx * 2, ldx * M * 2, OP_BK, 128, 1, Swz::B128)) return PV_ERR_CUDA;
  if (make_tmap_3d(&tmW, Wp, 2, K, 2 * N, 1, K * 2, K * 2 * N * 2, OP_BK, OP_BN / 2, 1, Swz::B128)) return PV_ERR_CUDA;
  if (make_tmap_3d(&tmD, y, 2, N, M, 1, ldy * 2, ldy * M * 2, 40, 32, 1, Swz::None)) return PV_ERR_CUDA;
  if (K == 320) return launch_g3<5, 8, OP_EPI_GEGLU, __nv_bfloat16>(tmA, tmW, tmD, bp, static_cast<int>(G), static_cast<int>(V), static_cast<int>(K), 1, stream);
  if (K == 640) return launch_g3<10, 5, OP_EPI_GEGLU, __nv_bfloat16>(tmA, tmW, tmD, bp, static_cast<int>(G), static_cast<int>(V), static_cast<int>(K), 1, stream);
  return launch_g3<0, 7, OP_EPI_GEGLU, __nv_bfloat16>(tmA, tmW, tmD, bp, static_cast<int>(G), static_cast<int>(V), static_cast<int>(K), 1, stream);
}

}
```

photoverse_b200/csrc/pv_outproj.cuh:

```cuda
#pragma once
#include "pv_common.cuh"
#include "pv_softmax.cuh"

namespace pv {

constexpr int OP_BN = 160;
constexpr int OP_BK = 64;
constexpr int OP_A_BYTES = 128 * OP_BK * 2;
constexpr int OP_WH_BYTES = (OP_BN / 2) * OP_BK * 2;
constexpr int OP_MAX_STAGES = 8;
constexpr int OP_BAR_BYTES = (2 * OP_MAX_STAGES + 5) * 8;
constexpr int OP_W_FREE = 2 * OP_MAX_STAGES + 5;

constexpr int OP_EPI_BIAS = 0;
constexpr int OP_EPI_GEGLU = 1;

template <int KB_RES, int NSTAGES>
struct OutProjCfg {
  static constexpr bool WSTAT = KB_RES > 0;
  static constexpr int KB_RESIDENT = KB_RES;
  static constexpr int W_RES_BYTES = KB_RES * OP_WH_BYTES;
  static constexpr int STAGES = NSTAGES;
  static constexpr int STAGE_BYTES = WSTAT ? OP_A_BYTES : OP_A_BYTES + OP_WH_BYTES;
  static constexpr int OFF_W = 0;
  static constexpr int OFF_STAGES = W_RES_BYTES;
  static constexpr int OFF_OST = OFF_STAGES + STAGES * STAGE_BYTES;
  static constexpr int OST_WARP_BYTES = 32 * 80 * 2;
  static constexpr int OFF_BIAS = OFF_OST + 8 * OST_WARP_BYTES;
  static constexpr int BYTES = OFF_BIAS + OP_BN * 4;
  static_assert(STAGES <= OP_MAX_STAGES, "barrier array");
};

struct OutProjArgs {
  const float* bias;
  unsigned int* sync;
  int G, MTP, C;
  int V;
  int u0, u1;
  int g;
  unsigned int ready_target;
  int w_preloaded;
  unsigned long long* trace;
  int trace_cap, trace_block;
};

__device__ __forceinline__ void op_mbar_init(uint64_t* pb) {
  uint64_t* full = pb;
  uint64_t* empty = full + OP_MAX_STAGES;
  uint64_t* acc_full = empty + OP_MAX_STAGES;
  uint64_t* slot_free = acc_full + 2;
  uint64_t* w_full = slot_free + 2;
  for (int s = 0; s < OP_MAX_STAGES; ++s) {
    mbar_init(&full[s], 1);
    mbar_init(&empty[s], 1);
  }
  for (int i = 0; i < 2; ++i) {
    mbar_init(&acc_full[i], 1);
    mbar_init(&slot_free[i], 16);
  }
  mbar_init(w_full, 1);
}

template <typename Cfg>
__device__ __forceinline__ void op_preload_w(uint8_t* smem, uint64_t* pb, const CUtensorMap* tmW, int g, uint32_t rank) {
  uint64_t* w_full = pb + 2 * OP_MAX_STAGES + 4;
  const uint32_t bar = mapa_u32(smem_u32(w_full), 0);
  const uint64_t pol_w = l2_policy_evict_last();
  if (rank == 0) mbar_expect_tx(w_full, 2 * Cfg::W_RES_BYTES);
  for (int kb = 0; kb < Cfg::KB_RESIDENT; ++kb)
    tma_load_3d_2sm_hint(smem + Cfg::OFF_W + kb * OP_WH_BYTES, tmW, bar, kb * OP_BK, g * OP_BN + static_cast<int>(rank) * (OP_BN / 2), 0,
                         pol_w);
}

__device__ __forceinline__ void op_signal_unit(unsigned int* sync, int u) {
  asm volatile("fence.proxy.async;" ::: "memory");
  asm volatile("red.release.gpu.global.add.u32 [%0], 1;" ::"l"(sync + u) : "memory");
}
__device__ __forceinline__ void op_signal_units(unsigned int* sync, int u0, int n) {
  asm volatile("fence.proxy.async;" ::: "memory");
  asm volatile("fence.acq_rel.gpu;" ::: "memory");
  for (int k = 0; k < n; ++k) asm volatile("red.relaxed.gpu.global.add.u32 [%0], 1;" ::"l"(sync + u0 + k) : "memory");
}
template <int N>
__device__ __forceinline__ void bulk_wait_all() {
  asm volatile("cp.async.bulk.wait_group %0;" ::"n"(N) : "memory");
}

__device__ __forceinline__ float op_gelu_erf(float g) { return 0.5f * g * (1.f + erff(g * 0.70710678118654752f)); }

__device__ __forceinline__ void op_geglu_epilogue(uint8_t* smem_ost, float* sbias, uint64_t* acc_full, uint64_t* slot_free,
                                                  uint32_t tmem, const CUtensorMap* tmD, const OutProjArgs& a) {
  const int warp = threadIdx.x >> 5;
  const int lane = threadIdx.x & 31;
  const uint32_t rank = cluster_ctarank();
  const int w = (warp - 4) >> 2;
  const int q = warp & 3;
  const uint32_t tlane = tmem + (static_cast<uint32_t>(q * 32) << 16);
  uint8_t* ost = smem_ost + (warp - 4) * (32 * 80 * 2);
  float* gbias = sbias + 80 * w;
  const uint32_t bias_a = smem_u32(gbias);
  const uint32_t ost_a = smem_u32(ost);
  auto load_bias = [&](int g) {
    for (int c = q * 32 + lane; c < 80; c += 128)
      gbias[c] = a.bias ? a.bias[g * OP_BN + (c < 40 ? 40 * w + c : 80 + 40 * w + (c - 40))] : 0.f;
  };
  int gb = a.u0 < a.u1 ? a.u0 / a.V : 0;
  load_bias(gb);
  named_bar_sync(9 + w, 128);
  int i = 0;
  for (int f = a.u0; f < a.u1; ++f, ++i) {
    const int g = f / a.V;
    const int u = f - g * a.V;
    const int slot = i & 1;
    const int m0 = (2 * u + static_cast<int>(rank)) * 128;
    if (g != gb) {
      named_bar_sync(9 + w, 128);
      gb = g;
      load_bias(gb);
      named_bar_sync(9 + w, 128);
    }
    mbar_wait(&acc_full[slot], (i >> 1) & 1);
    tc_fence_after();
    uint32_t v[80];
    const uint32_t src = tlane + slot * OP_BN + 40 * w;
    tmem_ld32_raw(src, v);
    tmem_ld_x8(src + 32, *reinterpret_cast<uint32_t(*)[8]>(v + 32));
    tmem_ld32_raw(src + 80, v + 40);
    tmem_ld_x8(src + 112, *reinterpret_cast<uint32_t(*)[8]>(v + 72));
    tmem_ld_wait();
    tc_fence_before();
    __syncwarp();
    if (elect_one()) mbar_arrive_cluster(mapa_u32(smem_u32(&slot_free[slot]), 0));
    if (elect_one()) bulk_wait_read<0>();
    __syncwarp();
    uint32_t y[20];
#pragma unroll
    for (int c = 0; c < 10; ++c) {
      float4 ba, bg;
      asm volatile("ld.shared.v4.f32 {%0, %1, %2, %3}, [%4];" : "=f"(ba.x), "=f"(ba.y), "=f"(ba.z), "=f"(ba.w) : "r"(bias_a + c * 16));
      asm volatile("ld.shared.v4.f32 {%0, %1, %2, %3}, [%4];" : "=f"(bg.x), "=f"(bg.y), "=f"(bg.z), "=f"(bg.w) : "r"(bias_a + 160 + c * 16));
      const float bav[4] = {ba.x, ba.y, ba.z, ba.w};
      const float bgv[4] = {bg.x, bg.y, bg.z, bg.w};
#pragma unroll
      for (int k = 0; k < 2; ++k) {
        const int j = 4 * c + 2 * k;
        const uint32_t ha = pack_bf16x2(__uint_as_float(v[j]) + bav[2 * k], __uint_as_float(v[j + 1]) + bav[2 * k + 1]);
        const uint32_t hg = pack_bf16x2(__uint_as_float(v[40 + j]) + bgv[2 * k], __uint_as_float(v[41 + j]) + bgv[2 * k + 1]);
        const uint32_t ge = pack_bf16x2(op_gelu_erf(__uint_as_float(hg << 16)), op_gelu_erf(__uint_as_float(hg & 0xffff0000u)));
        uint32_t p;
        asm("fma.rn.bf16x2 %0, %1, %2, %3;" : "=r"(p) : "r"(ha), "r"(ge), "r"(0x80008000u));
        y[2 * c + k] = p;
      }
    }
    const uint32_t row_a = ost_a + lane * 80;
#pragma unroll
    for (int c = 0; c < 5; ++c) st_shared_v4_a(row_a + c * 16, y[4 * c], y[4 * c + 1], y[4 * c + 2], y[4 * c + 3]);
    fence_proxy_async_smem();
    __syncwarp();
    if (elect_one()) {
      tma_store_3d(tmD, ost, 80 * g + 40 * w, m0 + q * 32, 0);
      bulk_commit();
    }
    __syncwarp();
  }
  if (elect_one()) bulk_wait_read<0>();
  __syncwarp();
}

template <typename Cfg, int EPI = OP_EPI_BIAS, typename T = __nv_bfloat16>
__device__ __forceinline__ void outproj_phase(uint8_t* smem, uint64_t* pb, uint32_t tmem, const CUtensorMap* tmA,
                                              const CUtensorMap* tmW, const CUtensorMap* tmD, const OutProjArgs& a) {
  constexpr bool WSTAT = Cfg::WSTAT;
  constexpr bool GEGLU = EPI == OP_EPI_GEGLU;
  static_assert(!GEGLU || std::is_same<T, __nv_bfloat16>::value, "the GEGLU epilogue rounds like the bf16 geglu_kernel");
  constexpr int nst = Cfg::STAGES;
  uint64_t* full = pb;
  uint64_t* empty = full + OP_MAX_STAGES;
  uint64_t* acc_full = empty + OP_MAX_STAGES;
  uint64_t* slot_free = acc_full + 2;
  uint64_t* w_full = slot_free + 2;
  uint64_t* w_free = pb + OP_W_FREE;
  float* sbias = reinterpret_cast<float*>(smem + Cfg::OFF_BIAS);
  const int warp = threadIdx.x >> 5;
  const int lane = threadIdx.x & 31;
  const uint32_t rank = cluster_ctarank();
  const int kblocks = a.C / OP_BK;
  const int n0 = a.g * OP_BN;
  auto group_of = [&](int u) -> int {
    if constexpr (GEGLU) return u / a.V;
    else return a.g;
  };
  auto unit_of = [&](int u) -> int {
    if constexpr (GEGLU) return u - (u / a.V) * a.V;
    else return u;
  };

  if (warp == 0) {
    A3Trace tr = a3_trace_init_raw(a.trace, a.trace_cap, 4, a.trace_block);
    a3_trace(tr, 50, 0);
    uint32_t it = 0;
    const uint64_t pol_a = l2_policy_evict_first();
    const bool has_sync = a.sync != nullptr;
    const unsigned int target = a.ready_target;
    unsigned int* ready = a.sync;
    unsigned int* seen = a.sync + a.V;
    auto probe32 = [&](int t0, uint32_t known) -> uint32_t {
      const int u = a.u0 + t0 + lane;
      bool ok = false;
      if (u < a.u1 && !((known >> lane) & 1u)) {
        unsigned int v;
        asm volatile("ld.acquire.gpu.global.u32 %0, [%1];" : "=r"(v) : "l"(ready + u) : "memory");
        ok = v >= target;
      }
      return known | __ballot_sync(0xffffffffu, ok);
    };
    uint32_t ready_mask = 0;
    if (has_sync && a.u0 < a.u1) {
      ready_mask = probe32(0, 0u);
      __syncwarp();
      a3_pair_time(a.trace, a.trace_block, 5);
      asm volatile("fence.proxy.async;" ::: "memory");
    }
    if constexpr (WSTAT) {
      if (!a.w_preloaded && a.u0 < a.u1 && elect_one()) op_preload_w<Cfg>(smem, pb, tmW, a.g, rank);
      __syncwarp();
    }
    [[maybe_unused]] int gw = a.g;
    [[maybe_unused]] uint32_t w_loads = 0;
    for (int u = a.u0; u < a.u1; ++u) {
      if constexpr (GEGLU && WSTAT) {
        if (group_of(u) != gw) {
          mbar_wait(w_free, w_loads & 1);
          ++w_loads;
          gw = group_of(u);
          if (elect_one()) op_preload_w<Cfg>(smem, pb, tmW, gw, rank);
          __syncwarp();
        }
      }
      const int b = unit_of(u) / a.MTP;
      const int mt = 2 * (unit_of(u) - b * a.MTP) + static_cast<int>(rank);
      const int t = u - a.u0;
      if (has_sync) {
        bool observed = false;
        if ((t & 31) == 0 && t > 0) { ready_mask = probe32(t, 0u); observed = true; }
        if (!((ready_mask >> (t & 31)) & 1u)) {
          ready_mask = probe32(t & ~31, ready_mask);
          observed = true;
          if (!((ready_mask >> (t & 31)) & 1u)) {
            if (lane == 0) {
              unsigned int v;
              uint32_t tries = 0;
              for (;;) {
                asm volatile("ld.acquire.gpu.global.u32 %0, [%1];" : "=r"(v) : "l"(ready + u) : "memory");
                if (v >= target) break;
                __nanosleep(32);
                if (++tries > 20000000u) __trap();
              }
            }
            ready_mask |= 1u << (t & 31);
          }
        }
        a3_trace(tr, 51, t);
        if (t == 0) a3_pair_time(a.trace, a.trace_block, 2);
        if (u == a.u1 - 1) a3_pair_time(a.trace, a.trace_block, 6);
        if (observed) {
          __syncwarp();
          asm volatile("fence.proxy.async;" ::: "memory");
        }
      }
      for (int kb = 0; kb < kblocks; ++kb, ++it) {
        const int s = it % nst;
        const uint32_t ph = (it / nst) & 1;
        mbar_wait(&empty[s], ph ^ 1);
        if (elect_one()) {
          uint8_t* a_dst = smem + Cfg::OFF_STAGES + s * Cfg::STAGE_BYTES;
          const uint32_t bar = mapa_u32(smem_u32(&full[s]), 0);
          if (rank == 0) mbar_expect_tx(&full[s], 2 * Cfg::STAGE_BYTES);
          tma_load_3d_2sm_hint(a_dst, tmA, bar, kb * OP_BK, mt * 128, b, pol_a);
          if constexpr (!WSTAT)
            tma_load_3d_2sm(a_dst + OP_A_BYTES, tmW, bar, kb * OP_BK, group_of(u) * OP_BN + static_cast<int>(rank) * (OP_BN / 2), 0);
        }
        __syncwarp();
      }
      a3_trace(tr, 52, t);
    }
    if (has_sync) {
      for (int u = a.u0 + lane; u < a.u1; u += 32) {
        unsigned int old;
        asm volatile("atom.acq_rel.gpu.global.add.u32 %0, [%1], 1;" : "=r"(old) : "l"(seen + u) : "memory");
        if (old == static_cast<unsigned int>(2 * a.G - 1)) {
          asm volatile("st.relaxed.gpu.global.u32 [%0], %1;" ::"l"(ready + u), "r"(0u) : "memory");
          asm volatile("st.relaxed.gpu.global.u32 [%0], %1;" ::"l"(seen + u), "r"(0u) : "memory");
        }
      }
    }
    a3_trace_done_raw(a.trace, tr, 4);
  } else if (warp == 1) {
    if (rank == 0) {
      constexpr uint32_t idesc = umma_idesc<T>(256, OP_BN);
      A3Trace tr = a3_trace_init_raw(a.trace, a.trace_cap, 5, a.trace_block);
      uint32_t it = 0;
      int i = 0;
      if constexpr (WSTAT) {
        if (a.u0 < a.u1) mbar_wait(w_full, 0);
      }
      [[maybe_unused]] int gw = a.g;
      [[maybe_unused]] uint32_t w_loads = 0;
      for (int u = a.u0; u < a.u1; ++u, ++i) {
        const int slot = i & 1;
        if (i >= 2) mbar_wait(&slot_free[slot], ((i >> 1) - 1) & 1);
        if constexpr (GEGLU && WSTAT) {
          if (group_of(u) != gw) {
            ++w_loads;
            gw = group_of(u);
            mbar_wait(w_full, w_loads & 1);
          }
        }
        tc_fence_after();
        for (int kb = 0; kb < kblocks; ++kb, ++it) {
          const int s = it % nst;
          const uint32_t ph = (it / nst) & 1;
          mbar_wait(&full[s], ph);
          tc_fence_after();
          if (kb == 0) a3_trace(tr, 60, i);
          if (elect_one()) {
            const uint8_t* a_src = smem + Cfg::OFF_STAGES + s * Cfg::STAGE_BYTES;
            const uint64_t da = umma_desc_sw128(a_src);
            const uint64_t dw = umma_desc_sw128(WSTAT ? smem + Cfg::OFF_W + kb * OP_WH_BYTES : a_src + OP_A_BYTES);
#pragma unroll
            for (int k = 0; k < OP_BK / 16; ++k) umma_bf16_ss_2sm(tmem + slot * OP_BN, da + 2 * k, dw + 2 * k, idesc, (kb | k) != 0);
            umma_commit_2sm(&empty[s]);
            if (kb == kblocks - 1) umma_commit_2sm(&acc_full[slot]);
            if constexpr (GEGLU && WSTAT) {
              if (kb == kblocks - 1 && u + 1 < a.u1 && group_of(u + 1) != gw) umma_commit_2sm(w_free);
            }
          }
          __syncwarp();
        }
        a3_trace(tr, 61, i);
      }
      a3_trace_done_raw(a.trace, tr, 5);
    }
  } else if (GEGLU && warp >= 4 && warp < 12) {
    op_geglu_epilogue(smem + Cfg::OFF_OST, sbias, acc_full, slot_free, tmem, tmD, a);
  } else if (warp >= 4 && warp < 12) {
    const int w = (warp - 4) >> 2;
    const int q = warp & 3;
    const uint32_t tlane = tmem + (static_cast<uint32_t>(q * 32) << 16);
    uint8_t* ost = smem + Cfg::OFF_OST + (warp - 4) * Cfg::OST_WARP_BYTES;
    const uint32_t bias_a = smem_u32(sbias + 80 * w);
    const uint32_t ost_a = smem_u32(ost);
    for (int c = (warp & 3) * 32 + lane; c < 80; c += 128) sbias[80 * w + c] = a.bias ? a.bias[n0 + 80 * w + c] : 0.f;
    named_bar_sync(9 + w, 128);
    A3Trace tr = a3_trace_init_raw(a.trace, a.trace_cap, 6, a.trace_block);
    if (warp != 4) tr.base = nullptr;
    int i = 0;
    for (int u = a.u0; u < a.u1; ++u, ++i) {
      const int slot = i & 1;
      const int b = u / a.MTP;
      const int m0 = (2 * (u - b * a.MTP) + static_cast<int>(rank)) * 128;
      mbar_wait(&acc_full[slot], (i >> 1) & 1);
      tc_fence_after();
      a3_trace(tr, 70, i);
      uint32_t v[80];
      const uint32_t src = tlane + slot * OP_BN + 80 * w;
      tmem_ld32_raw(src, v);
      tmem_ld32_raw(src + 32, v + 32);
      tmem_ld16_raw(src + 64, v + 64);
      tmem_ld_wait();
      tc_fence_before();
      __syncwarp();
      a3_trace(tr, 73, i);
      if (elect_one()) mbar_arrive_cluster(mapa_u32(smem_u32(&slot_free[slot]), 0));
      if (elect_one()) bulk_wait_read<0>();
      __syncwarp();
      a3_trace(tr, 74, i);
#pragma unroll
      for (int c = 0; c < 10; ++c) {
        float4 b0, b1;
        asm volatile("ld.shared.v4.f32 {%0, %1, %2, %3}, [%4];" : "=f"(b0.x), "=f"(b0.y), "=f"(b0.z), "=f"(b0.w) : "r"(bias_a + c * 32));
        asm volatile("ld.shared.v4.f32 {%0, %1, %2, %3}, [%4];" : "=f"(b1.x), "=f"(b1.y), "=f"(b1.z), "=f"(b1.w) : "r"(bias_a + c * 32 + 16));
        v[4 * c + 0] = pack_x2<T>(__uint_as_float(v[8 * c + 0]) + b0.x, __uint_as_float(v[8 * c + 1]) + b0.y);
        v[4 * c + 1] = pack_x2<T>(__uint_as_float(v[8 * c + 2]) + b0.z, __uint_as_float(v[8 * c + 3]) + b0.w);
        v[4 * c + 2] = pack_x2<T>(__uint_as_float(v[8 * c + 4]) + b1.x, __uint_as_float(v[8 * c + 5]) + b1.y);
        v[4 * c + 3] = pack_x2<T>(__uint_as_float(v[8 * c + 6]) + b1.z, __uint_as_float(v[8 * c + 7]) + b1.w);
      }
      {
        const bool hi = (lane & 4) != 0;
        const uint32_t row_a = ost_a + lane * 160;
#pragma unroll
        for (int c = 0; c < 10; ++c) {
          const int c2 = (c + 1) % 10;
          const uint32_t w0 = hi ? v[4 * c2 + 0] : v[4 * c + 0];
          const uint32_t w1 = hi ? v[4 * c2 + 1] : v[4 * c + 1];
          const uint32_t w2 = hi ? v[4 * c2 + 2] : v[4 * c + 2];
          const uint32_t w3 = hi ? v[4 * c2 + 3] : v[4 * c + 3];
          st_shared_v4_a(row_a + (hi ? c2 : c) * 16, w0, w1, w2, w3);
        }
      }
      a3_trace(tr, 75, i);
      fence_proxy_async_smem();
      __syncwarp();
      if (elect_one()) {
        tma_store_3d(tmD, ost, n0 + 80 * w, m0 + q * 32, b);
        bulk_commit();
      }
      __syncwarp();
      a3_trace(tr, 71, i);
    }
    if (elect_one()) bulk_wait_read<0>();
    __syncwarp();
    a3_trace(tr, 72, 0);
    a3_trace_done_raw(a.trace, tr, 6);
  }
}

}
```

photoverse_b200/host/unet_sd15.py:

```python
import math
from types import SimpleNamespace
from typing import Dict, Optional, Tuple

import torch
import torch.nn.functional as F
from torch import nn


FUSED_EPILOGUES = True


def _enabled(mod: nn.Module, x: torch.Tensor) -> bool:
    return FUSED_EPILOGUES and getattr(mod, "_pv_fused", True) and x.is_cuda and x.dtype == torch.bfloat16


def _fused(mod: nn.Module, x: torch.Tensor) -> bool:
    return _enabled(mod, x) and not torch.is_grad_enabled()


def _frozen(*tensors) -> bool:
    return not any(t is not None and t.requires_grad for t in tensors)


def _f32_params(mod: nn.Module, *names):
    ps = [getattr(mod, n) for n in names]
    key = tuple((p.data_ptr(), p._version) for p in ps)
    cached = getattr(mod, "_pv_f32", None)
    if cached is None or cached[0] != key:
        cached = (key, [p.detach().float().contiguous() for p in ps])
        mod._pv_f32 = cached
    return cached[1]


def _nhwc(x: torch.Tensor) -> bool:
    return (x.dim() == 4 and x.shape[1] % 8 == 0 and x.shape[1] <= 4096 and x.is_contiguous(memory_format=torch.channels_last)
            and not x.is_contiguous())


class _GroupNormActFn(torch.autograd.Function):

    @staticmethod
    def forward(ctx, x, add, gamma, beta, groups, eps, silu):
        from .. import ops
        y, stats = ops.group_norm_nhwc(x, gamma, beta, groups, eps, silu, add, save_stats=True)
        ctx.save_for_backward(x, stats, gamma, beta, *([] if add is None else [add]))
        ctx.cfg = (groups, silu)
        return y

    @staticmethod
    def backward(ctx, dy):
        from .. import ops
        x, stats, gamma, beta, *rest = ctx.saved_tensors
        dy = dy.contiguous(memory_format=torch.channels_last)
        dx = ops.group_norm_nhwc_bwd(x, dy, stats, gamma, beta, *ctx.cfg, add=rest[0] if rest else None)
        return dx, None, None, None, None, None, None


class _AddBiasFn(torch.autograd.Function):

    @staticmethod
    def forward(ctx, a, b, bias):
        from .. import ops
        return ops.add_bias_nhwc(a, b, bias)

    @staticmethod
    def backward(ctx, dy):
        return dy, dy, None


def group_norm_act(norm: nn.GroupNorm, x: torch.Tensor, silu: bool, add: Optional[torch.Tensor] = None) -> torch.Tensor:
    if _enabled(norm, x) and _nhwc(x):
        gamma, beta = _f32_params(norm, "weight", "bias")
        if not torch.is_grad_enabled():
            from .. import ops
            return ops.group_norm_nhwc(x, gamma, beta, norm.num_groups, norm.eps, silu, add)
        if _frozen(norm.weight, norm.bias, add):
            return _GroupNormActFn.apply(x, add, gamma, beta, norm.num_groups, norm.eps, silu)
    if add is not None:
        x = x + add.to(x.dtype)[:, :, None, None]
    y = norm(x)
    return F.silu(y) if silu else y


class _LayerNormFn(torch.autograd.Function):

    @staticmethod
    def forward(ctx, x, gamma, beta, eps):
        from .. import ops
        ctx.save_for_backward(x, gamma)
        ctx.eps = eps
        return ops.layer_norm(x, gamma, beta, eps)

    @staticmethod
    def backward(ctx, dy):
        from .. import ops
        x, gamma = ctx.saved_tensors
        return ops.layer_norm_bwd(x, dy.contiguous(), gamma, ctx.eps), None, None, None


def layer_norm(norm: nn.LayerNorm, x: torch.Tensor) -> torch.Tensor:
    if _enabled(norm, x) and x.is_contiguous() and x.shape[-1] % 8 == 0 and x.shape[-1] <= 1280:
        gamma, beta = _f32_params(norm, "weight", "bias")
        if not torch.is_grad_enabled():
            from .. import ops
            return ops.layer_norm(x, gamma, beta, norm.eps)
        if _frozen(norm.weight, norm.bias):
            return _LayerNormFn.apply(x, gamma, beta, norm.eps)
    return norm(x)


class AttnProcessor2_0:

    def __call__(self, attn, hidden_states, encoder_hidden_states=None, attention_mask=None, temb=None, **kw):
        B, S, C = hidden_states.shape
        ctx = hidden_states if encoder_hidden_states is None else encoder_hidden_states
        if isinstance(ctx, tuple):
            ctx = ctx[0]
        h = attn.heads
        q = attn.to_q(hidden_states).view(B, -1, h, C // h).transpose(1, 2)
        k = attn.to_k(ctx).view(B, -1, h, C // h).transpose(1, 2)
        v = attn.to_v(ctx).view(B, -1, h, C // h).transpose(1, 2)
        o = F.scaled_dot_product_attention(q, k, v, dropout_p=0.0, is_causal=False)
        o = o.transpose(1, 2).reshape(B, -1, C).to(q.dtype)
        return attn.to_out[1](attn.to_out[0](o))


class Attention(nn.Module):

    def __init__(self, query_dim: int, cross_attention_dim: Optional[int] = None, heads: int = 8):
        super().__init__()
        self.heads = heads
        self.inner_dim = query_dim
        self.cross_attention_dim = cross_attention_dim if cross_attention_dim is not None else query_dim
        self.scale = (query_dim // heads) ** -0.5
        self.to_q = nn.Linear(query_dim, query_dim, bias=False)
        self.to_k = nn.Linear(self.cross_attention_dim, query_dim, bias=False)
        self.to_v = nn.Linear(self.cross_attention_dim, query_dim, bias=False)
        self.to_out = nn.ModuleList([nn.Linear(query_dim, query_dim, bias=True), nn.Dropout(0.0)])
        self.spatial_norm = None
        self.group_norm = None
        self.norm_cross = None
        self.norm_encoder_hidden_states = None
        self.residual_connection = False
        self.rescale_output_factor = 1.0
        self.processor = AttnProcessor2_0()

    def set_processor(self, processor):
        if isinstance(getattr(self, "processor", None), nn.Module) and not isinstance(processor, nn.Module):
            self._modules.pop("processor", None)
        self.processor = processor

    def prepare_attention_mask(self, *a, **k):
        raise NotImplementedError("attention masks are not used by SD-1.5")

    def forward(self, hidden_states, encoder_hidden_states=None, attention_mask=None, **kw):
        return self.processor(self, hidden_states, encoder_hidden_states=encoder_hidden_states,
                              attention_mask=attention_mask, **kw)


class _GegluFn(torch.autograd.Function):

    @staticmethod
    def forward(ctx, h):
        from .. import ops
        ctx.save_for_backward(h)
        return ops.geglu(h)

    @staticmethod
    def backward(ctx, dy):
        from .. import ops
        (h,) = ctx.saved_tensors
        return ops.geglu_bwd(h, dy.contiguous())


class GEGLU(nn.Module):
    def __init__(self, dim_in, dim_out):
        super().__init__()
        self.proj = nn.Linear(dim_in, dim_out * 2)

    def _packed(self):
        ps = (self.proj.weight, self.proj.bias)
        key = tuple((p.data_ptr(), p._version) for p in ps)
        cached = getattr(self, "_pv_geglu", None)
        if cached is None or cached[0] != key:
            from .. import ops
            cached = (key, ops.pack_geglu_weight(*ps))
            self._pv_geglu = cached
        return cached[1]

    def forward(self, x):
        if (_fused(self, x) and x.is_contiguous() and x.shape[-1] % 64 == 0 and self.proj.out_features % 160 == 0
                and self.proj.bias is not None):
            from .. import ops
            return ops.linear_geglu(x, *self._packed())
        h = self.proj(x)
        if _enabled(self, h) and h.is_contiguous() and h.shape[-1] % 16 == 0:
            if torch.is_grad_enabled() and h.requires_grad:
                return _GegluFn.apply(h)
            from .. import ops
            return ops.geglu(h)
        x, gate = h.chunk(2, dim=-1)
        return x * F.gelu(gate)


class FeedForward(nn.Module):
    def __init__(self, dim):
        super().__init__()
        self.net = nn.ModuleList([GEGLU(dim, dim * 4), nn.Dropout(0.0), nn.Linear(dim * 4, dim)])

    def forward(self, x):
        for m in self.net:
            x = m(x)
        return x


class BasicTransformerBlock(nn.Module):
    def __init__(self, dim, heads, cross_attention_dim):
        super().__init__()
        self.norm1 = nn.LayerNorm(dim)
        self.attn1 = Attention(dim, None, heads)
        self.norm2 = nn.LayerNorm(dim)
        self.attn2 = Attention(dim, cross_attention_dim, heads)
        self.norm3 = nn.LayerNorm(dim)
        self.ff = FeedForward(dim)

    def forward(self, x, encoder_hidden_states):
        if (_fused(self.norm2, x) and _fused(self.norm3, x) and x.is_contiguous() and x.shape[-1] % 8 == 0
                and x.shape[-1] <= 1280):
            from .. import ops
            h = self.attn1(layer_norm(self.norm1, x))
            x, n = ops.add_layer_norm(h.contiguous(), x, *_f32_params(self.norm2, "weight", "bias"), self.norm2.eps)
            h = self.attn2(n, encoder_hidden_states=encoder_hidden_states)
            x, n = ops.add_layer_norm(h.contiguous(), x, *_f32_params(self.norm3, "weight", "bias"), self.norm3.eps)
            return self.ff(n) + x
        x = self.attn1(layer_norm(self.norm1, x)) + x
        x = self.attn2(layer_norm(self.norm2, x), encoder_hidden_states=encoder_hidden_states) + x
        return self.ff(layer_norm(self.norm3, x)) + x


class Transformer2DModel(nn.Module):
    def __init__(self, channels, heads, cross_attention_dim, groups=32):
        super().__init__()
        self.norm = nn.GroupNorm(groups, channels, eps=1e-6)
        self.proj_in = nn.Conv2d(channels, channels, 1)
        self.transformer_blocks = nn.ModuleList([BasicTransformerBlock(channels, heads, cross_attention_dim)])
        self.proj_out = nn.Conv2d(channels, channels, 1)

    def forward(self, x, encoder_hidden_states):
        B, C, H, W = x.shape
        res = x
        if _enabled(self.norm, x) and _nhwc(x):
            h = group_norm_act(self.norm, x, False).permute(0, 2, 3, 1).reshape(B, H * W, C)
            h = F.linear(h, self.proj_in.weight.view(C, C), self.proj_in.bias)
            for blk in self.transformer_blocks:
                h = blk(h, encoder_hidden_states)
            h = F.linear(h, self.proj_out.weight.view(C, C), self.proj_out.bias)
            h = h + res.permute(0, 2, 3, 1).reshape(B, H * W, C)
            return h.reshape(B, H, W, C).permute(0, 3, 1, 2)
        h = self.proj_in(group_norm_act(self.norm, x, False))
        h = h.permute(0, 2, 3, 1).reshape(B, H * W, C)
        for blk in self.transformer_blocks:
            h = blk(h, encoder_hidden_states)
        h = h.reshape(B, H, W, C).permute(0, 3, 1, 2)
        return self.proj_out(h) + res


class ResnetBlock2D(nn.Module):
    def __init__(self, cin, cout, temb_ch, groups=32):
        super().__init__()
        self.norm1 = nn.GroupNorm(groups, cin, eps=1e-5)
        self.conv1 = nn.Conv2d(cin, cout, 3, padding=1)
        self.time_emb_proj = nn.Linear(temb_ch, cout)
        self.norm2 = nn.GroupNorm(groups, cout, eps=1e-5)
        self.dropout = nn.Dropout(0.0)
        self.conv2 = nn.Conv2d(cout, cout, 3, padding=1)
        self.conv_shortcut = nn.Conv2d(cin, cout, 1) if cin != cout else None

    def forward(self, x, temb):
        if (_enabled(self.norm1, x) and _nhwc(x) and self.conv1.out_channels % 8 == 0
                and (not torch.is_grad_enabled()
                     or _frozen(temb, self.conv1.bias, self.conv2.bias, self.time_emb_proj.weight, self.time_emb_proj.bias,
                                None if self.conv_shortcut is None else self.conv_shortcut.bias))):
            c1, c2, cs = self.conv1, self.conv2, self.conv_shortcut
            h = F.conv2d(group_norm_act(self.norm1, x, True), c1.weight, None, c1.stride, c1.padding)
            add = self.time_emb_proj(F.silu(temb)).float() + _f32_params(c1, "bias")[0]
            h = F.conv2d(group_norm_act(self.norm2, h, True, add), c2.weight, None, c2.stride, c2.padding)
            bias = _f32_params(c2, "bias")[0]
            if cs is not None:
                x = F.conv2d(x, cs.weight, None, cs.stride, cs.padding)
                bias = self._shortcut_bias()
            if torch.is_grad_enabled() and (x.requires_grad or h.requires_grad):
                return _AddBiasFn.apply(x, h, bias)
            from .. import ops
            return ops.add_bias_nhwc(x, h, bias)
        h = self.conv1(group_norm_act(self.norm1, x, True))
        h = h + self.time_emb_proj(F.silu(temb))[:, :, None, None]
        h = self.conv2(self.dropout(group_norm_act(self.norm2, h, True)))
        if self.conv_shortcut is not None:
            x = self.conv_shortcut(x)
        return x + h


def _resnet_shortcut_bias(self):
    c2, cs = self.conv2, self.conv_shortcut
    key = (c2.bias.data_ptr(), c2.bias._version, cs.bias.data_ptr(), cs.bias._version)
    cached = getattr(self, "_pv_sum_bias", None)
    if cached is None or cached[0] != key:
        cached = (key, (c2.bias.detach().float() + cs.bias.detach().float()).contiguous())
        self._pv_sum_bias = cached
    return cached[1]


ResnetBlock2D._shortcut_bias = _resnet_shortcut_bias


class Downsample2D(nn.Module):
    def __init__(self, ch):
        super().__init__()
        self.conv = nn.Conv2d(ch, ch, 3, stride=2, padding=1)

    def forward(self, x):
        return self.conv(x)


class Upsample2D(nn.Module):
    def __init__(self, ch):
        super().__init__()
        self.conv = nn.Conv2d(ch, ch, 3, padding=1)

    def forward(self, x):
        return self.conv(F.interpolate(x, scale_factor=2.0, mode="nearest"))


class DownBlock(nn.Module):
    def __init__(self, cin, cout, temb_ch, layers, heads, cross_dim, has_attn, add_down):
        super().__init__()
        self.resnets = nn.ModuleList([ResnetBlock2D(cin if i == 0 else cout, cout, temb_ch) for i in range(layers)])
        self.attentions = nn.ModuleList(
            [Transformer2DModel(cout, heads, cross_dim) for _ in range(layers)]) if has_attn else None
        self.downsamplers = nn.ModuleList([Downsample2D(cout)]) if add_down else None

    def forward(self, x, temb, ctx):
        outs = []
        for i, r in enumerate(self.resnets):
            x = r(x, temb)
            if self.attentions is not None:
                x = self.attentions[i](x, ctx)
            outs.append(x)
        if self.downsamplers is not None:
            x = self.downsamplers[0](x)
            outs.append(x)
        return x, outs


class UpBlock(nn.Module):
    def __init__(self, cin, cout, prev_out, temb_ch, layers, heads, cross_dim, has_attn, add_up):
        super().__init__()
        res = []
        for i in range(layers):
            skip = cin if i == layers - 1 else cout
            rin = prev_out if i == 0 else cout
            res.append(ResnetBlock2D(rin + skip, cout, temb_ch))
        self.resnets = nn.ModuleList(res)
        self.attentions = nn.ModuleList(
            [Transformer2DModel(cout, heads, cross_dim) for _ in range(layers)]) if has_attn else None
        self.upsamplers = nn.ModuleList([Upsample2D(cout)]) if add_up else None

    def forward(self, x, skips, temb, ctx):
        for i, r in enumerate(self.resnets):
            x = torch.cat([x, skips.pop()], dim=1)
            x = r(x, temb)
            if self.attentions is not None:
                x = self.attentions[i](x, ctx)
        if self.upsamplers is not None:
            x = self.upsamplers[0](x)
        return x


class MidBlock(nn.Module):
    def __init__(self, ch, temb_ch, heads, cross_dim):
        super().__init__()
        self.resnets = nn.ModuleList([ResnetBlock2D(ch, ch, temb_ch), ResnetBlock2D(ch, ch, temb_ch)])
        self.attentions = nn.ModuleList([Transformer2DModel(ch, heads, cross_dim)])

    def forward(self, x, temb, ctx):
        x = self.resnets[0](x, temb)
        x = self.attentions[0](x, ctx)
        return self.resnets[1](x, temb)


class TimestepEmbedding(nn.Module):
    def __init__(self, cin, cout):
        super().__init__()
        self.linear_1 = nn.Linear(cin, cout)
        self.linear_2 = nn.Linear(cout, cout)

    def forward(self, x):
        return self.linear_2(F.silu(self.linear_1(x)))


def timestep_sinusoid(t: torch.Tensor, dim: int) -> torch.Tensor:
    half = dim // 2
    freqs = torch.exp(-math.log(10000.0) * torch.arange(half, dtype=torch.float32, device=t.device) / half)
    args = t.float()[:, None] * freqs[None]
    return torch.cat([torch.cos(args), torch.sin(args)], dim=-1)


class UNetSD15(nn.Module):

    def __init__(self, in_channels=4, out_channels=4, block_out_channels: Tuple[int, ...] = (320, 640, 1280, 1280),
                 layers_per_block=2, heads=8, cross_attention_dim=768, sample_size=64):
        super().__init__()
        boc = tuple(block_out_channels)
        n = len(boc)
        self.config = SimpleNamespace(in_channels=in_channels, out_channels=out_channels, block_out_channels=boc,
                                      layers_per_block=layers_per_block, attention_head_dim=heads,
                                      cross_attention_dim=cross_attention_dim, sample_size=sample_size)
        temb_ch = boc[0] * 4
        self.conv_in = nn.Conv2d(in_channels, boc[0], 3, padding=1)
        self.time_embedding = TimestepEmbedding(boc[0], temb_ch)
        self.down_blocks = nn.ModuleList()
        cout = boc[0]
        for i in range(n):
            cin, cout = cout, boc[i]
            last = i == n - 1
            self.down_blocks.append(DownBlock(cin, cout, temb_ch, layers_per_block, heads, cross_attention_dim,
                                              has_attn=not last or n == 1, add_down=not last))
        self.mid_block = MidBlock(boc[-1], temb_ch, heads, cross_attention_dim)
        self.up_blocks = nn.ModuleList()
        rev = list(reversed(boc))
        cout = rev[0]
        for i in range(n):
            prev_out, cout = cout, rev[i]
            cin = rev[min(i + 1, n - 1)]
            last = i == n - 1
            self.up_blocks.append(UpBlock(cin, cout, prev_out, temb_ch, layers_per_block + 1, heads,
                                          cross_attention_dim, has_attn=i > 0 or n == 1, add_up=not last))
        self.conv_norm_out = nn.GroupNorm(32, boc[0], eps=1e-5)
        self.conv_out = nn.Conv2d(boc[0], out_channels, 3, padding=1)

    @property
    def attn_processors(self) -> Dict[str, object]:
        procs = {}
        for name, m in self.named_modules():
            if isinstance(m, Attention):
                procs[f"{name}.processor"] = m.processor
        return procs

    def set_attn_processor(self, processor):
        mods = {f"{name}.processor": m for name, m in self.named_modules() if isinstance(m, Attention)}
        if isinstance(processor, dict):
            if len(processor) != len(mods):
                raise ValueError(f"A dict of processors was passed, but the number of processors {len(processor)} "
                                 f"does not match the number of attention layers: {len(mods)}.")
            for k, m in mods.items():
                m.set_processor(processor[k])
        else:
            for m in mods.values():
                m.set_processor(processor)

    def set_fused_epilogues(self, enabled: bool):
        for m in self.modules():
            if isinstance(m, (nn.GroupNorm, nn.LayerNorm, GEGLU)):
                m._pv_fused = bool(enabled)
        return self

    def forward(self, sample, timestep, encoder_hidden_states):
        if not torch.is_tensor(timestep):
            timestep = torch.tensor([timestep], device=sample.device)
        t = timestep.reshape(-1).expand(sample.shape[0]) if timestep.numel() == 1 else timestep
        temb = self.time_embedding(timestep_sinusoid(t, self.config.block_out_channels[0]).to(sample.dtype))
        x = self.conv_in(sample)
        skips = [x]
        for blk in self.down_blocks:
            x, outs = blk(x, temb, encoder_hidden_states)
            skips += outs
        x = self.mid_block(x, temb, encoder_hidden_states)
        for blk in self.up_blocks:
            x = blk(x, skips, temb, encoder_hidden_states)
        x = self.conv_out(group_norm_act(self.conv_norm_out, x, True))
        return SimpleNamespace(sample=x)
```

photoverse_b200/ops.py:

```python
import ctypes
from typing import Optional

import torch

from . import _lib
from ._lib import PV_BF16, PV_F16, PV_F32, PV_KEYS_PAD, check


_CODES = {torch.bfloat16: PV_BF16, torch.float32: PV_F32, torch.float16: PV_F16}
HALF_DTYPES = (torch.bfloat16, torch.float16)


def _code(dtype: torch.dtype) -> int:
    code = _CODES.get(dtype)
    if code is None:
        raise _lib.PhotoverseB200Error(f"unsupported dtype {dtype}: photoverse_b200 computes in bfloat16, float16 "
                                       "(inference only) or float32")
    return code


def _dt(t: torch.Tensor) -> int:
    return _code(t.dtype)


def _ptr(t: Optional[torch.Tensor]):
    if t is None:
        return None
    if not t.is_cuda:
        raise _lib.PhotoverseB200Error("photoverse_b200 ops need CUDA tensors (no CPU fallback)")
    return ctypes.c_void_p(t.data_ptr())


def _stream():
    return ctypes.c_void_p(torch.cuda.current_stream().cuda_stream)


def _f32(t: Optional[torch.Tensor]) -> Optional[torch.Tensor]:
    if t is None:
        return None
    assert t.dtype == torch.float32 and t.is_contiguous()
    return t


def resolve_compute_dtype(tensor_dtype: torch.dtype, grad_mode: bool, autocast_dtype: Optional[torch.dtype]) -> torch.dtype:
    if autocast_dtype not in HALF_DTYPES or tensor_dtype != torch.float32:
        return tensor_dtype
    if autocast_dtype == torch.float16 and grad_mode:
        return torch.float32
    return autocast_dtype


def autocast_dtype() -> Optional[torch.dtype]:
    return torch.get_autocast_dtype("cuda") if torch.is_autocast_enabled("cuda") else None


def compute_dtype(tensor_dtype: torch.dtype, grad_mode: bool) -> torch.dtype:
    return resolve_compute_dtype(tensor_dtype, grad_mode, autocast_dtype())


def convert(x: torch.Tensor, dtype: torch.dtype) -> torch.Tensor:
    if not x.is_cuda:
        raise _lib.PhotoverseB200Error("convert: CUDA tensor required (there is no CPU path)")
    src = x.contiguous()
    out = torch.empty(src.shape, device=src.device, dtype=dtype)
    check(_lib.lib().pv_convert_fwd(_dt(src), _code(dtype), _ptr(src), _ptr(out), src.numel(), _stream()), "pv_convert_fwd")
    return out


def pack_weight(w: torch.Tensor, out: torch.Tensor, lora_A=None, lora_B=None, scaling: float = 0.0) -> torch.Tensor:
    out_f, in_f = w.shape
    assert out.shape == w.shape and out.is_contiguous() and w.is_contiguous() and w.dtype == torch.float32
    r = 0
    if lora_A is not None:
        r = lora_A.shape[0]
        assert lora_A.shape == (r, in_f) and lora_B.shape == (out_f, r)
        lora_A, lora_B = _f32(lora_A.contiguous()), _f32(lora_B.contiguous())
    check(_lib.lib().pv_pack_weight(_dt(out), _ptr(w), _ptr(lora_A), _ptr(lora_B), float(scaling), _ptr(out),
                                    out_f, in_f, r, _stream()), "pv_pack_weight")
    return out


def linear(a: torch.Tensor, w: torch.Tensor, bias: Optional[torch.Tensor] = None,
           out: Optional[torch.Tensor] = None, out_dtype: Optional[torch.dtype] = None) -> torch.Tensor:
    batched = a.dim() == 3
    if not batched:
        a3 = a.unsqueeze(0)
    else:
        a3 = a
    batch, M, K = a3.shape
    w3 = w if w.dim() == 3 else w.unsqueeze(0)
    N = w3.shape[1]
    assert w3.shape[2] == K and a3.stride(2) == 1 and w3.stride(2) == 1
    assert a.dtype == w.dtype, (a.dtype, w.dtype)
    if out_dtype is None:
        out_dtype = a.dtype if out is None else out.dtype
    if out is None:
        out = torch.empty((batch, M, N) if batched else (M, N), device=a.device, dtype=out_dtype)
    o3 = out if out.dim() == 3 else out.unsqueeze(0)
    assert o3.shape == (batch, M, N) and o3.stride(2) == 1
    stride_w = w3.stride(0) if (w.dim() == 3 and w3.shape[0] > 1) else 0
    if w.dim() == 3 and w3.shape[0] not in (1, batch):
        raise ValueError("weight batch must be 1 or match the activation batch")
    stride_b = 0
    if bias is not None:
        assert bias.dtype == torch.float32 and bias.stride(-1) == 1
        stride_b = bias.stride(0) if (bias.dim() == 2 and bias.shape[0] > 1) else 0
    check(_lib.lib().pv_linear_fwd(_dt(a), _code(out_dtype), _ptr(a3), _ptr(w3), _ptr(bias), _ptr(o3),
                                   M, N, K, batch, a3.stride(1), w3.stride(1), o3.stride(1),
                                   a3.stride(0) if batch > 1 else 0, stride_w, stride_b,
                                   o3.stride(0) if batch > 1 else 0, _stream()), "pv_linear_fwd")
    return out


def kv_tile_bytes(dtype: torch.dtype, C: int, H: int, Lt: int, Li: int) -> int:
    n = int(_lib.lib().pv_kv_tile_bytes(_code(dtype), C, H, Lt, Li))
    if n <= 0:
        raise _lib.PhotoverseB200Error(f"bad K/V tile query C={C} H={H}")
    return n


class PackedKV:
    __slots__ = ("Kp", "Vp", "v_ip_norm", "kv_text", "kv_img", "B", "Lt", "Li", "C", "H", "dtype", "_keepalive", "vnorm_act")


def kv_pack(text: torch.Tensor, img: torch.Tensor, wkv_text: torch.Tensor, wkv_img: torch.Tensor, H: int,
            out: Optional["PackedKV"] = None) -> PackedKV:
    B, Lt, Dc = text.shape
    Li = img.shape[1]
    C = wkv_text.shape[0] // 2
    assert text.is_contiguous() and img.is_contiguous() and wkv_text.is_contiguous() and wkv_img.is_contiguous()
    assert text.dtype == img.dtype == wkv_text.dtype == wkv_img.dtype
    dev = text.device
    if out is not None and (out.B, out.Lt, out.Li, out.C, out.H, out.dtype) == (B, Lt, Li, C, H, text.dtype):
        kv = out
    else:
        kv = PackedKV()
        kv.B, kv.Lt, kv.Li, kv.C, kv.H, kv.dtype = B, Lt, Li, C, H, text.dtype
        tile = kv_tile_bytes(text.dtype, C, H, Lt, Li)
        kv.Kp = torch.empty(B * H * tile, device=dev, dtype=torch.uint8)
        kv.Vp = torch.empty(B * H * tile, device=dev, dtype=torch.uint8)
        kv.kv_text = torch.empty(B * Lt, 2 * C, device=dev, dtype=torch.float32)
        kv.kv_img = torch.empty(B * Li, 2 * C, device=dev, dtype=torch.float32)
        kv.v_ip_norm = torch.empty(B, H, Li, device=dev, dtype=torch.float32)
    check(_lib.lib().pv_kv_pack_fwd(_dt(text), _ptr(text), _ptr(img), _ptr(wkv_text), _ptr(wkv_img),
                                    _ptr(kv.kv_text), _ptr(kv.kv_img), _ptr(kv.Kp), _ptr(kv.Vp), _ptr(kv.v_ip_norm),
                                    B, Lt, Li, Dc, C, H, _stream()), "pv_kv_pack_fwd")
    if getattr(kv, "vnorm_act", None) is None:
        kv.vnorm_act = kv.v_ip_norm.to(text.dtype).unsqueeze(-1)
    else:
        kv.vnorm_act.copy_(kv.v_ip_norm.unsqueeze(-1))
    return kv


_SYNC = {}


def _sync_words(B: int, S: int, device) -> torch.Tensor:
    need = int(_lib.lib().pv_dual_attn_sync_words(B, S))
    key = (device.index, torch.cuda.current_stream(device).cuda_stream)
    buf = _SYNC.get(key)
    if buf is None or buf.numel() < need:
        buf = torch.zeros(max(need, 1 << 16), device=device, dtype=torch.int32)
        _SYNC[key] = buf
    return buf


def dual_attn(x: torch.Tensor, wq: torch.Tensor, kv: PackedKV, wo: torch.Tensor, bo: torch.Tensor,
              w_text: float = 1.0, w_img: float = 1.0, want_stats: bool = False):
    B, S, C = x.shape
    sync = _sync_words(B, S, x.device) if x.dtype in HALF_DTYPES else None
    assert x.is_contiguous() and wq.is_contiguous() and wo.is_contiguous()
    assert x.dtype == wq.dtype == wo.dtype == kv.dtype and bo.dtype == torch.float32
    assert (kv.B, kv.C) == (B, C)
    y = torch.empty_like(x)
    o = torch.empty_like(x)
    q = torch.empty(B, S, C, device=x.device, dtype=torch.float32) if x.dtype == torch.float32 else None
    stats = torch.empty(B, kv.H, S, 4, device=x.device, dtype=torch.float32) if want_stats else None
    check(_lib.lib().pv_dual_attn_fwd(_dt(x), _ptr(x), _ptr(wq), _ptr(kv.Kp), _ptr(kv.Vp), _ptr(wo), _ptr(bo),
                                      _ptr(y), _ptr(q), _ptr(o), _ptr(stats), _ptr(sync), B, S, C, kv.H, kv.Lt, kv.Li,
                                      float(w_text), float(w_img), _stream()), "pv_dual_attn_fwd")
    return y, o, stats, q


def dual_attn_core(x_or_q: torch.Tensor, wq: Optional[torch.Tensor], kv: PackedKV, w_text: float = 1.0,
                   w_img: float = 1.0, want_stats: bool = False):
    B, S, C = x_or_q.shape
    assert x_or_q.is_contiguous() and x_or_q.dtype == kv.dtype and (kv.B, kv.C) == (B, C)
    if x_or_q.dtype in HALF_DTYPES:
        assert wq is not None and wq.is_contiguous() and wq.dtype == x_or_q.dtype and wq.shape == (C, C)
    o = torch.empty_like(x_or_q)
    stats = torch.empty(B, kv.H, S, 4, device=o.device, dtype=torch.float32) if want_stats else None
    check(_lib.lib().pv_dual_attn_core_fwd(_dt(x_or_q), _ptr(x_or_q), _ptr(wq), _ptr(kv.Kp), _ptr(kv.Vp), _ptr(o),
                                           _ptr(stats), B, S, C, kv.H, kv.Lt, kv.Li, float(w_text), float(w_img),
                                           _stream()), "pv_dual_attn_core_fwd")
    return o, stats


def ln_lrelu(x: torch.Tensor, gamma: torch.Tensor, beta: torch.Tensor, out: torch.Tensor,
             rows_per_group: int = 0, eps: float = 1e-5, slope: float = 0.01, save_stats: bool = False):
    rows, cols = x.shape
    assert x.dtype == torch.float32 and x.stride(1) == 1 and out.stride(1) == 1 and out.shape == x.shape
    assert gamma.dtype == beta.dtype == torch.float32 and gamma.is_contiguous() and beta.is_contiguous()
    mean = rstd = None
    if save_stats:
        mean = torch.empty(rows, device=x.device, dtype=torch.float32)
        rstd = torch.empty(rows, device=x.device, dtype=torch.float32)
    check(_lib.lib().pv_ln_lrelu_fwd(_dt(out), _ptr(x), _ptr(gamma), _ptr(beta), _ptr(out), _ptr(mean), _ptr(rstd),
                                     rows, cols, x.stride(0), out.stride(0), rows_per_group, eps, slope, _stream()),
          "pv_ln_lrelu_fwd")
    return out, mean, rstd


def group_mean(x: torch.Tensor, out: torch.Tensor) -> torch.Tensor:
    groups, P, cols = x.shape
    assert x.is_contiguous() and out.shape == (groups, cols) and out.stride(1) == 1
    check(_lib.lib().pv_group_mean_fwd(_dt(x), _dt(out), _ptr(x), _ptr(out), groups, P, cols, out.stride(0),
                                       _stream()), "pv_group_mean_fwd")
    return out


_WS = {}


def _workspace(nbytes: int, device) -> torch.Tensor:
    key = (device.type, device.index)
    buf = _WS.get(key)
    if buf is None or buf.numel() < nbytes:
        buf = torch.empty(max(int(nbytes), 1 << 20), device=device, dtype=torch.uint8)
        _WS[key] = buf
    return buf


def transpose(x: torch.Tensor, out: Optional[torch.Tensor] = None) -> torch.Tensor:
    R, C = x.shape
    assert x.stride(1) == 1
    if out is None:
        out = torch.empty(C, R, device=x.device, dtype=x.dtype)
    assert out.shape == (C, R) and out.stride(1) == 1
    if out.stride(0) != R:
        raise ValueError(f"transpose: out must have row stride {R} (got {out.stride(0)}); columns up to the row stride "
                         "would be zero-filled")
    check(_lib.lib().pv_transpose_2d(_dt(x), _ptr(x), _ptr(out), R, C, x.stride(0), out.stride(0), _stream()), "pv_transpose_2d")
    return out


def linear_bwd_weight(g: torch.Tensor, x: torch.Tensor, out: Optional[torch.Tensor] = None, alpha: float = 1.0,
                      beta: float = 0.0) -> torch.Tensor:
    M, N = g.shape
    K = x.shape[1]
    assert x.shape[0] == M and g.dtype == x.dtype and g.stride(1) == 1 and x.stride(1) == 1
    if out is None:
        assert beta == 0.0
        out = torch.empty(N, K, device=g.device, dtype=torch.float32)
    assert out.shape == (N, K) and out.is_contiguous() and out.dtype == torch.float32
    lib = _lib.lib()
    ws = _workspace(lib.pv_linear_bwd_weight_ws_bytes(_dt(g), M, N, K), g.device)
    check(lib.pv_linear_bwd_weight(_dt(g), _ptr(g), _ptr(x), _ptr(out), _ptr(ws), M, N, K, g.stride(0), x.stride(0),
                                   float(alpha), float(beta), _stream()), "pv_linear_bwd_weight")
    return out


def lora_bwd(x: torch.Tensor, g: torch.Tensor, lora_A: torch.Tensor, lora_B: torch.Tensor, scaling: float):
    M, in_f = x.shape
    out_f = g.shape[1]
    r = lora_A.shape[0]
    assert g.shape[0] == M and x.dtype == g.dtype and x.stride(1) == 1 and g.stride(1) == 1
    assert lora_A.shape == (r, in_f) and lora_B.shape == (out_f, r)
    lib = _lib.lib()
    nbytes = int(lib.pv_lora_bwd_ws_bytes(M, in_f, out_f, r))
    if nbytes < 0:
        return None
    a32, b32 = _f32(lora_A.detach().float().contiguous()), _f32(lora_B.detach().float().contiguous())
    out = torch.empty(r * in_f + out_f * r, device=x.device, dtype=torch.float32)
    ws = _workspace(nbytes, x.device)
    check(lib.pv_lora_bwd(_dt(x), _ptr(x), _ptr(g), _ptr(a32), _ptr(b32), float(scaling), _ptr(out), _ptr(ws), M, in_f, out_f, r,
                          x.stride(0), g.stride(0), _stream()), "pv_lora_bwd")
    return out[:r * in_f].view(r, in_f), out[r * in_f:].view(out_f, r)


def col_sum(g: torch.Tensor) -> torch.Tensor:
    M, N = g.shape
    assert g.stride(1) == 1
    out = torch.empty(N, device=g.device, dtype=torch.float32)
    lib = _lib.lib()
    ws = _workspace(lib.pv_col_sum_ws_bytes(M, N), g.device)
    check(lib.pv_col_sum(_dt(g), _ptr(g), _ptr(out), _ptr(ws), M, N, g.stride(0), _stream()), "pv_col_sum")
    return out


def ln_lrelu_bwd(da: torch.Tensor, x: torch.Tensor, mean: torch.Tensor, rstd: torch.Tensor, gamma: torch.Tensor,
                 beta: torch.Tensor, groups: int, rows_per_group: int, slope: float = 0.01):
    rows, cols = da.shape
    assert rows == groups * rows_per_group and da.is_contiguous() and x.is_contiguous() and x.dtype == torch.float32
    dx = torch.empty_like(da)
    dgamma = torch.empty(groups, cols, device=da.device, dtype=torch.float32)
    dbeta = torch.empty_like(dgamma)
    lib = _lib.lib()
    ws = _workspace(lib.pv_ln_lrelu_bwd_ws_bytes(groups, rows_per_group, cols), da.device)
    check(lib.pv_ln_lrelu_bwd(_dt(da), _ptr(da), _ptr(x), _ptr(mean), _ptr(rstd), _ptr(gamma), _ptr(beta), _ptr(dx),
                              _ptr(dgamma), _ptr(dbeta), _ptr(ws), groups, rows_per_group, cols, float(slope), _stream()),
          "pv_ln_lrelu_bwd")
    return dx, dgamma, dbeta


def group_mean_bwd(dy: torch.Tensor, P: int) -> torch.Tensor:
    groups, cols = dy.shape
    assert dy.stride(1) == 1
    dx = torch.empty(groups, P, cols, device=dy.device, dtype=dy.dtype)
    check(_lib.lib().pv_group_mean_bwd(_dt(dy), _ptr(dy), _ptr(dx), groups, P, cols, dy.stride(0), _stream()),
          "pv_group_mean_bwd")
    return dx


def dual_attn_bwd(d_o: torch.Tensor, q: torch.Tensor, kv_text: torch.Tensor, kv_img: torch.Tensor, stats: torch.Tensor,
                  v_ip_norm: torch.Tensor, d_vnorm: Optional[torch.Tensor], H: int, Lt: int, Li: int, w_text: float,
                  w_img: float):
    B, S, C = d_o.shape
    assert d_o.is_contiguous() and q.is_contiguous() and q.dtype == d_o.dtype and stats.is_contiguous()
    dq = torch.empty_like(d_o)
    dkv_text = torch.empty(B * Lt, 2 * C, device=d_o.device, dtype=d_o.dtype)
    dkv_img = torch.empty(B * Li, 2 * C, device=d_o.device, dtype=d_o.dtype)
    lib = _lib.lib()
    ws = _workspace(lib.pv_dual_attn_bwd_ws_bytes(B, S, C, H, Lt, Li), d_o.device)
    check(lib.pv_dual_attn_bwd(_dt(d_o), _ptr(d_o), _ptr(q), _ptr(kv_text), _ptr(kv_img), _ptr(stats), _ptr(dq), _ptr(ws),
                               B, S, C, H, Lt, Li, float(w_text), float(w_img), _stream()), "pv_dual_attn_bwd")
    if d_vnorm is not None:
        d_vnorm = d_vnorm.to(torch.float32).contiguous()
    check(lib.pv_kv_pack_bwd(_dt(d_o), _ptr(ws), _ptr(kv_img), _ptr(v_ip_norm), _ptr(d_vnorm), _ptr(dkv_text), _ptr(dkv_img),
                             B, S, Lt, Li, C, H, _stream()), "pv_kv_pack_bwd")
    return dq, dkv_text, dkv_img


def dropout_bwd_acc(dst: torch.Tensor, src: torch.Tensor, keep_mask: torch.Tensor, p: float) -> torch.Tensor:
    assert dst.is_contiguous() and src.is_contiguous() and keep_mask.is_contiguous()
    assert dst.shape == src.shape == keep_mask.shape and dst.dtype == src.dtype and keep_mask.dtype == torch.bool
    check(_lib.lib().pv_dropout_bwd_acc(_dt(dst), _ptr(dst), _ptr(src), _ptr(keep_mask), 1.0 / (1.0 - float(p)),
                                        dst.numel(), _stream()), "pv_dropout_bwd_acc")
    return dst


_SA_WS = {}


def self_attn(q: torch.Tensor, k: torch.Tensor, v: torch.Tensor, heads: int) -> torch.Tensor:
    if not (q.is_cuda and q.dtype == torch.bfloat16 and k.dtype == v.dtype == q.dtype):
        raise _lib.PhotoverseB200Error("self_attn: CUDA bfloat16 tensors required (there is no CPU path)")
    B, S, C = q.shape
    ld = q.stride(1)
    for t in (q, k, v):
        if t.shape != q.shape or t.stride(2) != 1 or t.stride(1) != ld or (B > 1 and t.stride(0) != S * ld):
            raise _lib.PhotoverseB200Error("self_attn: q, k, v must be [B,S,C] views with the same row stride and batch stride S*ld")
    lib = _lib.lib()
    nbytes = int(lib.pv_self_attn_ws_bytes(B, S, C, heads))
    if nbytes < 0:
        raise _lib.PhotoverseB200Error(f"self_attn: unsupported shape B={B} S={S} C={C} heads={heads}")
    key = (q.device.index, torch.cuda.current_stream(q.device).cuda_stream)
    ws = _SA_WS.get(key)
    if ws is None or ws.numel() < nbytes:
        ws = torch.empty(nbytes, device=q.device, dtype=torch.uint8)
        _SA_WS[key] = ws
    out = torch.empty(B, S, C, device=q.device, dtype=q.dtype)
    _lib.check(lib.pv_self_attn_fwd(_ptr(q), _ptr(k), _ptr(v), ld, _ptr(out), _ptr(ws), B, S, C, heads, _stream()), "pv_self_attn_fwd")
    return out


def _gn_geometry(x: torch.Tensor, what: str):
    if not (x.is_cuda and x.dtype == torch.bfloat16):
        raise _lib.PhotoverseB200Error(f"{what}: CUDA bfloat16 activations required (there is no CPU path)")
    if x.dim() == 4:
        B, C, H, W = x.shape
        if not x.is_contiguous(memory_format=torch.channels_last):
            raise _lib.PhotoverseB200Error(f"{what}: the activation must be channels_last-contiguous")
        return B, H * W, C
    B, HW, C = x.shape
    if not x.is_contiguous():
        raise _lib.PhotoverseB200Error(f"{what}: [B, HW, C] input must be contiguous")
    return B, HW, C


def group_norm_nhwc(x: torch.Tensor, gamma: torch.Tensor, beta: torch.Tensor, groups: int, eps: float, silu: bool,
                    add: Optional[torch.Tensor] = None, save_stats: bool = False):
    B, HW, C = _gn_geometry(x, "group_norm_nhwc")
    assert gamma.dtype == beta.dtype == torch.float32 and gamma.is_contiguous() and beta.is_contiguous() and gamma.numel() == C
    if add is not None:
        assert add.dtype == torch.float32 and add.is_contiguous() and add.shape == (B, C) and add.is_cuda
    lib = _lib.lib()
    nbytes = int(lib.pv_group_norm_nhwc_ws_bytes(B, HW, C, groups))
    if nbytes < 0:
        raise _lib.PhotoverseB200Error(f"group_norm_nhwc: unsupported shape B={B} HW={HW} C={C} groups={groups}")
    ws = torch.empty(nbytes, device=x.device, dtype=torch.uint8)
    y = torch.empty_like(x)
    stats = torch.empty(B, groups, 2, device=x.device, dtype=torch.float32) if save_stats else None
    check(lib.pv_group_norm_nhwc_fwd(PV_BF16, _ptr(x), _ptr(add), _ptr(gamma), _ptr(beta), _ptr(y), _ptr(stats), _ptr(ws), B, HW, C,
                                     groups, float(eps), 1 if silu else 0, _stream()), "pv_group_norm_nhwc_fwd")
    return (y, stats) if save_stats else y


def group_norm_nhwc_bwd(x: torch.Tensor, dy: torch.Tensor, stats: torch.Tensor, gamma: torch.Tensor, beta: torch.Tensor,
                        groups: int, silu: bool, add: Optional[torch.Tensor] = None) -> torch.Tensor:
    B, HW, C = _gn_geometry(x, "group_norm_nhwc_bwd")
    if dy.shape != x.shape or _gn_geometry(dy, "group_norm_nhwc_bwd") != (B, HW, C):
        raise _lib.PhotoverseB200Error("group_norm_nhwc_bwd: dy must have the shape, dtype and memory layout of x")
    assert stats.dtype == torch.float32 and stats.is_contiguous() and stats.shape == (B, groups, 2)
    lib = _lib.lib()
    ws = torch.empty(int(lib.pv_group_norm_nhwc_ws_bytes(B, HW, C, groups)), device=x.device, dtype=torch.uint8)
    dx = torch.empty_like(x)
    check(lib.pv_group_norm_nhwc_bwd(PV_BF16, _ptr(x), _ptr(add), _ptr(dy), _ptr(stats), _ptr(gamma), _ptr(beta), _ptr(dx), _ptr(ws),
                                     B, HW, C, groups, 1 if silu else 0, _stream()), "pv_group_norm_nhwc_bwd")
    return dx


def add_bias_nhwc(a: torch.Tensor, b: torch.Tensor, bias: torch.Tensor) -> torch.Tensor:
    if not (a.is_cuda and a.dtype == torch.bfloat16 and b.dtype == torch.bfloat16 and a.shape == b.shape):
        raise _lib.PhotoverseB200Error("add_bias_nhwc: two CUDA bfloat16 tensors of one shape required (there is no CPU path)")
    if a.dim() == 4:
        if not (a.is_contiguous(memory_format=torch.channels_last) and b.is_contiguous(memory_format=torch.channels_last)):
            raise _lib.PhotoverseB200Error("add_bias_nhwc: 4-D operands must be channels_last-contiguous")
        C = a.shape[1]
    else:
        if not (a.is_contiguous() and b.is_contiguous()):
            raise _lib.PhotoverseB200Error("add_bias_nhwc: operands must be contiguous")
        C = a.shape[-1]
    assert bias.dtype == torch.float32 and bias.is_contiguous() and bias.numel() == C
    out = torch.empty_like(a)
    check(_lib.lib().pv_add_bias_nhwc_fwd(PV_BF16, _ptr(a), _ptr(b), _ptr(bias), _ptr(out), a.numel() // C, C, _stream()),
          "pv_add_bias_nhwc_fwd")
    return out


def layer_norm(x: torch.Tensor, gamma: torch.Tensor, beta: torch.Tensor, eps: float) -> torch.Tensor:
    if not (x.is_cuda and x.dtype == torch.bfloat16 and x.is_contiguous()):
        raise _lib.PhotoverseB200Error("layer_norm: contiguous CUDA bfloat16 input required (there is no CPU path)")
    C = x.shape[-1]
    assert gamma.dtype == beta.dtype == torch.float32 and gamma.is_contiguous() and beta.is_contiguous() and gamma.numel() == C
    y = torch.empty_like(x)
    check(_lib.lib().pv_layer_norm_fwd(PV_BF16, _ptr(x), None, None, _ptr(gamma), _ptr(beta), _ptr(y), x.numel() // C, C, float(eps),
                                       _stream()), "pv_layer_norm_fwd")
    return y


def add_layer_norm(x: torch.Tensor, residual: torch.Tensor, gamma: torch.Tensor, beta: torch.Tensor, eps: float):
    if not (x.is_cuda and x.dtype == torch.bfloat16 and x.is_contiguous() and residual.dtype == x.dtype
            and residual.is_contiguous() and residual.shape == x.shape):
        raise _lib.PhotoverseB200Error("add_layer_norm: two contiguous CUDA bfloat16 tensors of one shape required")
    C = x.shape[-1]
    assert gamma.dtype == beta.dtype == torch.float32 and gamma.is_contiguous() and beta.is_contiguous() and gamma.numel() == C
    s, y = torch.empty_like(x), torch.empty_like(x)
    check(_lib.lib().pv_layer_norm_fwd(PV_BF16, _ptr(x), _ptr(residual), _ptr(s), _ptr(gamma), _ptr(beta), _ptr(y), x.numel() // C, C,
                                       float(eps), _stream()), "pv_layer_norm_fwd")
    return s, y


def layer_norm_bwd(x: torch.Tensor, dy: torch.Tensor, gamma: torch.Tensor, eps: float) -> torch.Tensor:
    if not (x.is_cuda and x.dtype == torch.bfloat16 and x.is_contiguous() and dy.dtype == x.dtype and dy.is_contiguous()
            and dy.shape == x.shape):
        raise _lib.PhotoverseB200Error("layer_norm_bwd: contiguous CUDA bfloat16 x and dy of one shape required")
    C = x.shape[-1]
    assert gamma.dtype == torch.float32 and gamma.is_contiguous() and gamma.numel() == C
    dx = torch.empty_like(x)
    check(_lib.lib().pv_layer_norm_bwd(PV_BF16, _ptr(x), _ptr(dy), _ptr(gamma), _ptr(dx), x.numel() // C, C, float(eps), _stream()),
          "pv_layer_norm_bwd")
    return dx


def geglu(h: torch.Tensor) -> torch.Tensor:
    if not (h.is_cuda and h.dtype == torch.bfloat16 and h.is_contiguous()):
        raise _lib.PhotoverseB200Error("geglu: contiguous CUDA bfloat16 input required (there is no CPU path)")
    N = h.shape[-1] // 2
    M = h.numel() // (2 * N)
    y = torch.empty(*h.shape[:-1], N, device=h.device, dtype=h.dtype)
    check(_lib.lib().pv_geglu_fwd(PV_BF16, _ptr(h), _ptr(y), M, N, 2 * N, _stream()), "pv_geglu_fwd")
    return y


def pack_geglu_weight(w: torch.Tensor, b: Optional[torch.Tensor]):
    two_n, K = w.shape
    N = two_n // 2
    if two_n % 2 or N % 80:
        raise ValueError(f"pack_geglu_weight: need 2N rows with N % 80 == 0 (got {two_n})")
    def regroup(t):
        return torch.stack([t[:N].reshape(N // 80, 80, *t.shape[1:]), t[N:].reshape(N // 80, 80, *t.shape[1:])], 1).reshape(t.shape)
    wp = regroup(w.detach()).to(torch.bfloat16).contiguous()
    bp = None if b is None else regroup(b.detach()).float().contiguous()
    return wp, bp


def linear_geglu(x: torch.Tensor, w_packed: torch.Tensor, b_packed: Optional[torch.Tensor] = None) -> torch.Tensor:
    if not (x.is_cuda and x.dtype == torch.bfloat16 and x.is_contiguous()):
        raise _lib.PhotoverseB200Error("linear_geglu: contiguous CUDA bfloat16 input required (there is no CPU path)")
    if not (w_packed.dtype == torch.bfloat16 and w_packed.dim() == 2 and w_packed.is_contiguous()):
        raise _lib.PhotoverseB200Error("linear_geglu: contiguous bfloat16 [2N, K] packed weight required")
    two_n, K = w_packed.shape
    if x.shape[-1] != K:
        raise _lib.PhotoverseB200Error(f"linear_geglu: input has {x.shape[-1]} features, the weight {K}")
    if b_packed is not None and not (b_packed.dtype == torch.float32 and b_packed.is_contiguous() and b_packed.numel() == two_n):
        raise _lib.PhotoverseB200Error("linear_geglu: contiguous float32 [2N] packed bias required")
    N = two_n // 2
    M = x.numel() // K
    y = torch.empty(*x.shape[:-1], N, device=x.device, dtype=x.dtype)
    check(_lib.lib().pv_linear_geglu_fwd(PV_BF16, _ptr(x), _ptr(w_packed), _ptr(b_packed), _ptr(y), M, N, K, K, N, _stream()),
          "pv_linear_geglu_fwd")
    return y


def geglu_bwd(h: torch.Tensor, dy: torch.Tensor) -> torch.Tensor:
    if not (h.is_cuda and h.dtype == torch.bfloat16 and h.is_contiguous() and dy.dtype == h.dtype and dy.is_contiguous()):
        raise _lib.PhotoverseB200Error("geglu_bwd: contiguous CUDA bfloat16 h and dy required (there is no CPU path)")
    N = h.shape[-1] // 2
    M = h.numel() // (2 * N)
    assert dy.shape == (*h.shape[:-1], N)
    dh = torch.empty_like(h)
    check(_lib.lib().pv_geglu_bwd(PV_BF16, _ptr(h), _ptr(dy), _ptr(dh), M, N, 2 * N, _stream()), "pv_geglu_bwd")
    return dh
```

Baseline: 8.631.

## Fuse residual add into GEMM epilogue, merge QKV, split conv bias

Adds a residual-add epilogue to the persistent paired GEMM. The residual tile is TMA-loaded into the output staging buffer and added before the store, so feed-forward and proj_out skip a separate elementwise add. Self-attention now computes Q, K and V with one concatenated-weight linear, and some convs run without bias followed by a fused NHWC bias kernel. These are several independent changes at once; the residual TMA load now sits before the accumulator wait, which could add latency in the epilogue.

```diff
diff --git a/include/photoverse_b200.h b/include/photoverse_b200.h
--- a/include/photoverse_b200.h
+++ b/include/photoverse_b200.h
@@ -115,6 +115,8 @@
 int pv_geglu_bwd(pv_dtype dt, const void* h, const void* dy, void* dh, int64_t M, int N, int64_t ldh, void* stream);
 int pv_linear_geglu_fwd(pv_dtype dt, const void* x, const void* w_packed, const float* b_packed, void* y, int64_t M, int64_t N,
                         int64_t K, int64_t ldx, int64_t ldy, void* stream);
+int pv_linear_residual_fwd(pv_dtype dt, const void* x, const void* W, const float* bias, const void* r, void* y, int64_t M,
+                           int64_t N, int64_t K, int64_t ldx, int64_t ldr, int64_t ldy, void* stream);
 
 int pv_convert_fwd(pv_dtype in_dt, pv_dtype out_dt, const void* src, void* dst, int64_t n, void* stream);
 
diff --git a/photoverse_b200/_lib.py b/photoverse_b200/_lib.py
--- a/photoverse_b200/_lib.py
+++ b/photoverse_b200/_lib.py
@@ -66,6 +66,7 @@
     "pv_geglu_fwd": (c_int, [c_int, c_void_p, c_void_p, c_int64, c_int, c_int64, c_void_p]),
     "pv_geglu_bwd": (c_int, [c_int, c_void_p, c_void_p, c_void_p, c_int64, c_int, c_int64, c_void_p]),
     "pv_linear_geglu_fwd": (c_int, [c_int, c_void_p, c_void_p, c_void_p, c_void_p] + [c_int64] * 5 + [c_void_p]),
+    "pv_linear_residual_fwd": (c_int, [c_int, c_void_p, c_void_p, c_void_p, c_void_p, c_void_p] + [c_int64] * 6 + [c_void_p]),
     "pv_convert_fwd": (c_int, [c_int, c_int, c_void_p, c_void_p, c_int64, c_void_p]),
 }
 
diff --git a/photoverse_b200/csrc/pv_api.cu b/photoverse_b200/csrc/pv_api.cu
--- a/photoverse_b200/csrc/pv_api.cu
+++ b/photoverse_b200/csrc/pv_api.cu
@@ -92,6 +92,8 @@
 int linear_geglu_bf16(const void* x, const void* Wp, const float* bp, void* y, long long M, long long N, long long K,
                       long long ldx, long long ldy, cudaStream_t stream);
 int geglu_bwd(const void* h, const void* dy, void* dh, long long M, int N, long long ldh, cudaStream_t stream);
+int linear_residual_bf16(const void* x, const void* W, const float* bias, const void* r, void* y, long long M, long long N,
+                         long long K, long long ldx, long long ldr, long long ldy, cudaStream_t stream);
 int dropout_bwd_acc(bool bf16, void* dst, const void* src, const uint8_t* mask, float alpha, long long n,
                     cudaStream_t stream);
 
@@ -556,7 +558,7 @@
 int pv_add_bias_nhwc_fwd(pv_dtype dt, const void* a, const void* b, const float* bias, void* out, int64_t rows, int C,
                          void* stream) {
   PV_NO_F16(dt);
-  PV_REQUIRE(a && b && bias && out, "null pointer");
+  PV_REQUIRE(a && bias && out, "null pointer");
   PV_REQUIRE(dt == PV_BF16, "bf16 activations only");
   return add_bias_nhwc(a, b, bias, out, rows, C, as_stream(stream));
 }
@@ -599,4 +601,12 @@
   return linear_geglu_bf16(x, w_packed, b_packed, y, M, N, K, ldx, ldy, as_stream(stream));
 }
 
-}
+int pv_linear_residual_fwd(pv_dtype dt, const void* x, const void* W, const float* bias, const void* r, void* y, int64_t M,
+                           int64_t N, int64_t K, int64_t ldx, int64_t ldr, int64_t ldy, void* stream) {
+  PV_NO_F16(dt);
+  PV_REQUIRE(x && W && r && y, "null pointer");
+  PV_REQUIRE(dt == PV_BF16, "bf16 activations only");
+  return linear_residual_bf16(x, W, bias, r, y, M, N, K, ldx, ldr, ldy, as_stream(stream));
+}
+
+}
diff --git a/photoverse_b200/csrc/pv_backbone.cu b/photoverse_b200/csrc/pv_backbone.cu
--- a/photoverse_b200/csrc/pv_backbone.cu
+++ b/photoverse_b200/csrc/pv_backbone.cu
@@ -426,11 +426,16 @@
     const int v = static_cast<int>(i % vecs);
     float fa[8], fb[8];
     bf16x8_unpack(reinterpret_cast<const uint4*>(a)[i], fa);
-    bf16x8_unpack(reinterpret_cast<const uint4*>(b)[i], fb);
     const float4 b0 = __ldg(reinterpret_cast<const float4*>(bias) + 2 * v), b1 = __ldg(reinterpret_cast<const float4*>(bias) + 2 * v + 1);
     const float bb[8] = {b0.x, b0.y, b0.z, b0.w, b1.x, b1.y, b1.z, b1.w};
-#pragma unroll
-    for (int j = 0; j < 8; ++j) fa[j] = fa[j] + (fb[j] + bb[j]);
+    if (b) {
+      bf16x8_unpack(reinterpret_cast<const uint4*>(b)[i], fb);
+#pragma unroll
+      for (int j = 0; j < 8; ++j) fa[j] = fa[j] + (fb[j] + bb[j]);
+    } else {
+#pragma unroll
+      for (int j = 0; j < 8; ++j) fa[j] = fa[j] + bb[j];
+    }
     reinterpret_cast<uint4*>(out)[i] = bf16x8_pack(fa);
   }
 }
diff --git a/photoverse_b200/csrc/pv_gemm3.cu b/photoverse_b200/csrc/pv_gemm3.cu
--- a/photoverse_b200/csrc/pv_gemm3.cu
+++ b/photoverse_b200/csrc/pv_gemm3.cu
@@ -11,11 +11,11 @@
 __global__ void __cluster_dims__(2, 1, 1) __launch_bounds__(G3_THREADS, 1)
 gemm3_pair_persistent_kernel(const __grid_constant__ CUtensorMap tmA, const __grid_constant__ CUtensorMap tmW,
                              const __grid_constant__ CUtensorMap tmD, const float* __restrict__ bias, int G, int V, int K,
-                             int w_static) {
+                             int w_static, const __grid_constant__ CUtensorMap tmR) {
   extern __shared__ uint8_t smem_raw[];
   uint8_t* smem = reinterpret_cast<uint8_t*>((reinterpret_cast<uintptr_t>(smem_raw) + 1023) & ~uintptr_t(1023));
   uint64_t* bars = reinterpret_cast<uint64_t*>(smem + (Cfg::BYTES + 15) / 16 * 16);
-  uint32_t* tmem_slot = reinterpret_cast<uint32_t*>(bars + OP_BAR_BYTES / 8 + (EPI == OP_EPI_GEGLU ? 1 : 0));
+  uint32_t* tmem_slot = reinterpret_cast<uint32_t*>(bars + (EPI == OP_EPI_RESIDUAL ? OP_R_FULL + 8 : OP_BAR_BYTES / 8 + (EPI == OP_EPI_GEGLU ? 1 : 0)));
   const int warp = threadIdx.x >> 5;
   const int pair = blockIdx.x >> 1;
   const int npairs = gridDim.x >> 1;
@@ -37,8 +37,12 @@
     tma_prefetch_desc(&tmA);
     tma_prefetch_desc(&tmW);
     tma_prefetch_desc(&tmD);
+    if constexpr (EPI == OP_EPI_RESIDUAL) tma_prefetch_desc(&tmR);
     op_mbar_init(bars);
     if constexpr (EPI == OP_EPI_GEGLU) mbar_init(bars + OP_W_FREE, 1);
+    if constexpr (EPI == OP_EPI_RESIDUAL) {
+      for (int k = 0; k < 8; ++k) mbar_init(bars + OP_R_FULL + k, 1);
+    }
     fence_barrier_init();
   }
   if (warp == 2) tmem_alloc_2sm<512>(tmem_slot);
@@ -67,7 +71,7 @@
   oa.ready_target = 0;
   oa.w_preloaded = Cfg::WSTAT && w_static && u0 < u1;
   oa.trace = nullptr; oa.trace_cap = 0; oa.trace_block = 0;
-  outproj_phase<Cfg, EPI, T>(smem, bars, tmem, &tmA, &tmW, &tmD, oa);
+  outproj_phase<Cfg, EPI, T>(smem, bars, tmem, &tmA, &tmW, &tmD, oa, &tmR);
 
   tc_fence_before();
   __syncthreads();
@@ -78,16 +82,17 @@
 
 template <int KB_RES, int STAGES, int EPI, typename T>
 static int launch_g3(const CUtensorMap& tmA, const CUtensorMap& tmW, const CUtensorMap& tmD, const float* bias, int G, int V,
-                     int K, int w_static, cudaStream_t stream) {
+                     int K, int w_static, cudaStream_t stream, const CUtensorMap* tmR = nullptr) {
   using Cfg = OutProjCfg<KB_RES, STAGES>;
   constexpr int SMEM_BYTES = (Cfg::BYTES + 15) / 16 * 16 + 256 + 1024;
-  static_assert(OP_BAR_BYTES + 8 + 8 <= 256 && SMEM_BYTES <= 227 * 1024, "shared memory budget");
+  static_assert(OP_BAR_BYTES + 8 + 8 <= 256 && (OP_R_FULL + 8) * 8 + 8 <= 256 && SMEM_BYTES <= 227 * 1024, "shared memory budget");
   auto kern = gemm3_pair_persistent_kernel<Cfg, EPI, T>;
   PV_CUDA(set_max_smem_once(kern, SMEM_BYTES));
   const long long units = static_cast<long long>(G) * V;
   const long long max_pairs = sm_count() / 2;
   const int npairs = static_cast<int>(units < max_pairs ? units : max_pairs);
-  PV_CUDA(launch_pdl(kern, dim3(2 * npairs), dim3(G3_THREADS), SMEM_BYTES, stream, tmA, tmW, tmD, bias, G, V, K, w_static));
+  PV_CUDA(launch_pdl(kern, dim3(2 * npairs), dim3(G3_THREADS), SMEM_BYTES, stream, tmA, tmW, tmD, bias, G, V, K, w_static,
+                      tmR ? *tmR : tmD));
   PV_LAUNCHED();
   return PV_OK;
 }
@@ -131,4 +136,29 @@
   return launch_g3<0, 7, OP_EPI_GEGLU, __nv_bfloat16>(tmA, tmW, tmD, bp, static_cast<int>(G), static_cast<int>(V), static_cast<int>(K), 1, stream);
 }
 
+int linear_residual_bf16(const void* x, const void* W, const float* bias, const void* r, void* y, long long M, long long N,
+                         long long K, long long ldx, long long ldr, long long ldy, cudaStream_t stream) {
+  PV_REQUIRE(M > 0 && N > 0 && K > 0 && N % OP_BN == 0 && K % OP_BK == 0,
+             "linear_residual: need M > 0, N %% 160 == 0 and K %% 64 == 0 (M=%lld N=%lld K=%lld)", M, N, K);
+  PV_REQUIRE(ldx >= K && ldr >= N && ldy >= N && ldx % 8 == 0 && ldr % 8 == 0 && ldy % 8 == 0,
+             "linear_residual: row strides must be >= the row and 16-byte multiples (ldx=%lld ldr=%lld ldy=%lld)", ldx, ldr, ldy);
+  PV_REQUIRE((reinterpret_cast<uintptr_t>(x) | reinterpret_cast<uintptr_t>(W) | reinterpret_cast<uintptr_t>(r) |
+              reinterpret_cast<uintptr_t>(y)) % 16 == 0,
+             "linear_residual: pointers must be 16-byte aligned");
+  const long long G = N / OP_BN;
+  const long long V = (M + 255) / 256;
+  PV_REQUIRE(V * G < (1ll << 30), "too many tiles");
+  CUtensorMap tmA, tmW, tmD, tmR;
+  if (make_tmap_3d(&tmA, x, 2, K, M, 1, ldx * 2, ldx * M * 2, OP_BK, 128, 1, Swz::B128)) return PV_ERR_CUDA;
+  if (make_tmap_3d(&tmW, W, 2, K, N, 1, K * 2, K * N * 2, OP_BK, OP_BN / 2, 1, Swz::B128)) return PV_ERR_CUDA;
+  if (make_tmap_3d(&tmD, y, 2, N, M, 1, ldy * 2, ldy * M * 2, 80, 32, 1, Swz::None)) return PV_ERR_CUDA;
+  if (make_tmap_3d(&tmR, r, 2, N, M, 1, ldr * 2, ldr * M * 2, 80, 32, 1, Swz::None)) return PV_ERR_CUDA;
+#define PV_G3R(KB, ST) \
+  launch_g3<KB, ST, OP_EPI_RESIDUAL, __nv_bfloat16>(tmA, tmW, tmD, bias, static_cast<int>(G), static_cast<int>(V), static_cast<int>(K), 1, stream, &tmR)
+  if (K == 320) return PV_G3R(5, 8);
+  if (K == 640) return PV_G3R(10, 5);
+  return PV_G3R(0, 7);
+#undef PV_G3R
 }
+
+}
diff --git a/photoverse_b200/csrc/pv_outproj.cuh b/photoverse_b200/csrc/pv_outproj.cuh
--- a/photoverse_b200/csrc/pv_outproj.cuh
+++ b/photoverse_b200/csrc/pv_outproj.cuh
@@ -11,9 +11,11 @@
 constexpr int OP_MAX_STAGES = 8;
 constexpr int OP_BAR_BYTES = (2 * OP_MAX_STAGES + 5) * 8;
 constexpr int OP_W_FREE = 2 * OP_MAX_STAGES + 5;
+constexpr int OP_R_FULL = OP_W_FREE + 1;
 
 constexpr int OP_EPI_BIAS = 0;
 constexpr int OP_EPI_GEGLU = 1;
+constexpr int OP_EPI_RESIDUAL = 2;
 
 template <int KB_RES, int NSTAGES>
 struct OutProjCfg {
@@ -84,6 +86,11 @@
 template <int N>
 __device__ __forceinline__ void bulk_wait_all() {
   asm volatile("cp.async.bulk.wait_group %0;" ::"n"(N) : "memory");
+}
+
+__device__ __forceinline__ uint32_t op_add_bf16x2(uint32_t a, uint32_t b) {
+  return pack_bf16x2(__uint_as_float(a << 16) + __uint_as_float(b << 16),
+                     __uint_as_float(a & 0xffff0000u) + __uint_as_float(b & 0xffff0000u));
 }
 
 __device__ __forceinline__ float op_gelu_erf(float g) { return 0.5f * g * (1.f + erff(g * 0.70710678118654752f)); }
@@ -169,10 +176,13 @@
 
 template <typename Cfg, int EPI = OP_EPI_BIAS, typename T = __nv_bfloat16>
 __device__ __forceinline__ void outproj_phase(uint8_t* smem, uint64_t* pb, uint32_t tmem, const CUtensorMap* tmA,
-                                              const CUtensorMap* tmW, const CUtensorMap* tmD, const OutProjArgs& a) {
+                                              const CUtensorMap* tmW, const CUtensorMap* tmD, const OutProjArgs& a,
+                                              const CUtensorMap* tmR = nullptr) {
   constexpr bool WSTAT = Cfg::WSTAT;
   constexpr bool GEGLU = EPI == OP_EPI_GEGLU;
+  constexpr bool RESID = EPI == OP_EPI_RESIDUAL;
   static_assert(!GEGLU || std::is_same<T, __nv_bfloat16>::value, "the GEGLU epilogue rounds like the bf16 geglu_kernel");
+  static_assert(!RESID || std::is_same<T, __nv_bfloat16>::value, "the residual epilogue rounds like torch's bf16 add");
   constexpr int nst = Cfg::STAGES;
   uint64_t* full = pb;
   uint64_t* empty = full + OP_MAX_STAGES;
@@ -350,6 +360,7 @@
     uint8_t* ost = smem + Cfg::OFF_OST + (warp - 4) * Cfg::OST_WARP_BYTES;
     const uint32_t bias_a = smem_u32(sbias + 80 * w);
     const uint32_t ost_a = smem_u32(ost);
+    [[maybe_unused]] uint64_t* r_full = pb + OP_R_FULL + (warp - 4);
     for (int c = (warp & 3) * 32 + lane; c < 80; c += 128) sbias[80 * w + c] = a.bias ? a.bias[n0 + 80 * w + c] : 0.f;
     named_bar_sync(9 + w, 128);
     A3Trace tr = a3_trace_init_raw(a.trace, a.trace_cap, 6, a.trace_block);
@@ -359,6 +370,14 @@
       const int slot = i & 1;
       const int b = u / a.MTP;
       const int m0 = (2 * (u - b * a.MTP) + static_cast<int>(rank)) * 128;
+      if constexpr (RESID) {
+        if (elect_one()) {
+          bulk_wait_read<0>();
+          mbar_expect_tx(r_full, Cfg::OST_WARP_BYTES);
+          tma_load_3d(ost, tmR, r_full, n0 + 80 * w, m0 + q * 32, b);
+        }
+        __syncwarp();
+      }
       mbar_wait(&acc_full[slot], (i >> 1) & 1);
       tc_fence_after();
       a3_trace(tr, 70, i);
@@ -372,7 +391,9 @@
       __syncwarp();
       a3_trace(tr, 73, i);
       if (elect_one()) mbar_arrive_cluster(mapa_u32(smem_u32(&slot_free[slot]), 0));
-      if (elect_one()) bulk_wait_read<0>();
+      if constexpr (!RESID) {
+        if (elect_one()) bulk_wait_read<0>();
+      }
       __syncwarp();
       a3_trace(tr, 74, i);
 #pragma unroll
@@ -388,13 +409,22 @@
       {
         const bool hi = (lane & 4) != 0;
         const uint32_t row_a = ost_a + lane * 160;
+        if constexpr (RESID) mbar_wait(r_full, i & 1);
 #pragma unroll
         for (int c = 0; c < 10; ++c) {
           const int c2 = (c + 1) % 10;
-          const uint32_t w0 = hi ? v[4 * c2 + 0] : v[4 * c + 0];
-          const uint32_t w1 = hi ? v[4 * c2 + 1] : v[4 * c + 1];
-          const uint32_t w2 = hi ? v[4 * c2 + 2] : v[4 * c + 2];
-          const uint32_t w3 = hi ? v[4 * c2 + 3] : v[4 * c + 3];
+          uint32_t w0 = hi ? v[4 * c2 + 0] : v[4 * c + 0];
+          uint32_t w1 = hi ? v[4 * c2 + 1] : v[4 * c + 1];
+          uint32_t w2 = hi ? v[4 * c2 + 2] : v[4 * c + 2];
+          uint32_t w3 = hi ? v[4 * c2 + 3] : v[4 * c + 3];
+          if constexpr (RESID) {
+            uint32_t r0, r1, r2, r3;
+            asm volatile("ld.shared.v4.b32 {%0, %1, %2, %3}, [%4];" : "=r"(r0), "=r"(r1), "=r"(r2), "=r"(r3) : "r"(row_a + (hi ? c2 : c) * 16));
+            w0 = op_add_bf16x2(w0, r0);
+            w1 = op_add_bf16x2(w1, r1);
+            w2 = op_add_bf16x2(w2, r2);
+            w3 = op_add_bf16x2(w3, r3);
+          }
           st_shared_v4_a(row_a + (hi ? c2 : c) * 16, w0, w1, w2, w3);
         }
       }
diff --git a/photoverse_b200/host/unet_sd15.py b/photoverse_b200/host/unet_sd15.py
--- a/photoverse_b200/host/unet_sd15.py
+++ b/photoverse_b200/host/unet_sd15.py
@@ -37,6 +37,18 @@
             and not x.is_contiguous())
 
 
+def conv_bias(conv: nn.Conv2d, x: torch.Tensor) -> torch.Tensor:
+    if (FUSED_EPILOGUES and conv.bias is not None and x.is_cuda and x.dtype == torch.bfloat16 and conv.weight.dtype == torch.bfloat16
+            and not torch.is_grad_enabled() and conv.out_channels % 8 == 0 and conv.padding_mode == "zeros"
+            and x.is_contiguous(memory_format=torch.channels_last)):
+        y = F.conv2d(x, conv.weight, None, conv.stride, conv.padding, conv.dilation, conv.groups)
+        if _nhwc(y):
+            from .. import ops
+            return ops.add_bias_nhwc(y, None, _f32_params(conv, "bias")[0])
+        return y + conv.bias[:, None, None]
+    return conv(x)
+
+
 class _GroupNormActFn(torch.autograd.Function):
 
     @staticmethod
@@ -109,14 +121,52 @@
     return norm(x)
 
 
+def _pair_gemm(x: torch.Tensor, w: torch.Tensor, r: Optional[torch.Tensor] = None) -> bool:
+    if not (FUSED_EPILOGUES and x.is_cuda and x.dtype == torch.bfloat16 and w.dtype == torch.bfloat16 and not torch.is_grad_enabled()
+            and x.is_contiguous() and w.is_contiguous() and w.shape[0] % 160 == 0 and w.shape[1] % 64 == 0
+            and x.shape[-1] == w.shape[1] and (r is None or (r.dtype == torch.bfloat16 and r.is_contiguous()))):
+        return False
+    tiles = -(-(x.numel() // x.shape[-1]) // 256) * (w.shape[0] // 160)
+    return tiles >= torch.cuda.get_device_properties(x.device).multi_processor_count // 2
+
+
+def linear_residual(mod: nn.Module, w: torch.Tensor, x: torch.Tensor, r: Optional[torch.Tensor], fuse: bool) -> torch.Tensor:
+    if _pair_gemm(x, w, r):
+        from .. import ops
+        b = _f32_params(mod, "bias")[0] if mod.bias is not None else None
+        if r is not None and fuse:
+            return ops.linear_residual(x, w, b, r)
+        y = ops.linear(x.reshape(-1, x.shape[-1]), w, b).view(*x.shape[:-1], w.shape[0])
+        return y if r is None else y + r
+    y = F.linear(x, w, mod.bias)
+    return y if r is None else y + r
+
+
+def _qkv_weight(attn) -> torch.Tensor:
+    ps = (attn.to_q.weight, attn.to_k.weight, attn.to_v.weight)
+    key = tuple((p.data_ptr(), p._version) for p in ps)
+    cached = getattr(attn, "_pv_qkv", None)
+    if cached is None or cached[0] != key:
+        cached = (key, torch.cat([p.detach() for p in ps]).contiguous())
+        attn._pv_qkv = cached
+    return cached[1]
+
+
 class AttnProcessor2_0:
 
     def __call__(self, attn, hidden_states, encoder_hidden_states=None, attention_mask=None, temb=None, **kw):
         B, S, C = hidden_states.shape
+        h = attn.heads
+        if (encoder_hidden_states is None and hidden_states.is_cuda and not torch.is_grad_enabled()
+                and all(type(m) is nn.Linear for m in (attn.to_q, attn.to_k, attn.to_v))):
+            qkv = F.linear(hidden_states, _qkv_weight(attn))
+            q, k, v = (qkv[..., i * C:(i + 1) * C].view(B, S, h, C // h).transpose(1, 2) for i in range(3))
+            o = F.scaled_dot_product_attention(q, k, v, dropout_p=0.0, is_causal=False)
+            o = o.transpose(1, 2).reshape(B, -1, C).to(q.dtype)
+            return attn.to_out[1](attn.to_out[0](o))
         ctx = hidden_states if encoder_hidden_states is None else encoder_hidden_states
         if isinstance(ctx, tuple):
             ctx = ctx[0]
-        h = attn.heads
         q = attn.to_q(hidden_states).view(B, -1, h, C // h).transpose(1, 2)
         k = attn.to_k(ctx).view(B, -1, h, C // h).transpose(1, 2)
         v = attn.to_v(ctx).view(B, -1, h, C // h).transpose(1, 2)
@@ -208,10 +258,13 @@
         super().__init__()
         self.net = nn.ModuleList([GEGLU(dim, dim * 4), nn.Dropout(0.0), nn.Linear(dim * 4, dim)])
 
-    def forward(self, x):
-        for m in self.net:
-            x = m(x)
-        return x
+    def forward(self, x, residual: Optional[torch.Tensor] = None):
+        x = self.net[1](self.net[0](x))
+        out = self.net[2]
+        if type(out) is nn.Linear:
+            return linear_residual(out, out.weight, x, residual, fuse=True)
+        x = out(x)
+        return x if residual is None else x + residual
 
 
 class BasicTransformerBlock(nn.Module):
@@ -232,7 +285,7 @@
             x, n = ops.add_layer_norm(h.contiguous(), x, *_f32_params(self.norm2, "weight", "bias"), self.norm2.eps)
             h = self.attn2(n, encoder_hidden_states=encoder_hidden_states)
             x, n = ops.add_layer_norm(h.contiguous(), x, *_f32_params(self.norm3, "weight", "bias"), self.norm3.eps)
-            return self.ff(n) + x
+            return self.ff(n, residual=x)
         x = self.attn1(layer_norm(self.norm1, x)) + x
         x = self.attn2(layer_norm(self.norm2, x), encoder_hidden_states=encoder_hidden_states) + x
         return self.ff(layer_norm(self.norm3, x)) + x
@@ -254,15 +307,21 @@
             h = F.linear(h, self.proj_in.weight.view(C, C), self.proj_in.bias)
             for blk in self.transformer_blocks:
                 h = blk(h, encoder_hidden_states)
-            h = F.linear(h, self.proj_out.weight.view(C, C), self.proj_out.bias)
-            h = h + res.permute(0, 2, 3, 1).reshape(B, H * W, C)
-            return h.reshape(B, H, W, C).permute(0, 3, 1, 2)
+            return self._proj_out_residual(h, res, fuse=True)
         h = self.proj_in(group_norm_act(self.norm, x, False))
         h = h.permute(0, 2, 3, 1).reshape(B, H * W, C)
         for blk in self.transformer_blocks:
             h = blk(h, encoder_hidden_states)
+        if _nhwc(x) and _pair_gemm(h, self.proj_out.weight.view(C, C)):
+            return self._proj_out_residual(h, res, fuse=False)
         h = h.reshape(B, H, W, C).permute(0, 3, 1, 2)
         return self.proj_out(h) + res
+
+    def _proj_out_residual(self, h: torch.Tensor, res: torch.Tensor, fuse: bool) -> torch.Tensor:
+        B, C, H, W = res.shape
+        h = linear_residual(self.proj_out, self.proj_out.weight.view(C, C), h.contiguous(), res.permute(0, 2, 3, 1).reshape(B, H * W, C),
+                            fuse)
+        return h.reshape(B, H, W, C).permute(0, 3, 1, 2)
 
 
 class ResnetBlock2D(nn.Module):
@@ -320,7 +379,7 @@
         self.conv = nn.Conv2d(ch, ch, 3, stride=2, padding=1)
 
     def forward(self, x):
-        return self.conv(x)
+        return conv_bias(self.conv, x)
 
 
 class Upsample2D(nn.Module):
@@ -329,7 +388,7 @@
         self.conv = nn.Conv2d(ch, ch, 3, padding=1)
 
     def forward(self, x):
-        return self.conv(F.interpolate(x, scale_factor=2.0, mode="nearest"))
+        return conv_bias(self.conv, F.interpolate(x, scale_factor=2.0, mode="nearest"))
 
 
 class DownBlock(nn.Module):
@@ -470,7 +529,7 @@
             timestep = torch.tensor([timestep], device=sample.device)
         t = timestep.reshape(-1).expand(sample.shape[0]) if timestep.numel() == 1 else timestep
         temb = self.time_embedding(timestep_sinusoid(t, self.config.block_out_channels[0]).to(sample.dtype))
-        x = self.conv_in(sample)
+        x = conv_bias(self.conv_in, sample)
         skips = [x]
         for blk in self.down_blocks:
             x, outs = blk(x, temb, encoder_hidden_states)
diff --git a/photoverse_b200/ops.py b/photoverse_b200/ops.py
--- a/photoverse_b200/ops.py
+++ b/photoverse_b200/ops.py
@@ -410,15 +410,20 @@
     return dx
 
 
-def add_bias_nhwc(a: torch.Tensor, b: torch.Tensor, bias: torch.Tensor) -> torch.Tensor:
-    if not (a.is_cuda and a.dtype == torch.bfloat16 and b.dtype == torch.bfloat16 and a.shape == b.shape):
+def add_bias_nhwc(a: torch.Tensor, b: Optional[torch.Tensor], bias: torch.Tensor) -> torch.Tensor:
+    if b is None:
+        b_ok = True
+    else:
+        b_ok = b.dtype == torch.bfloat16 and b.shape == a.shape
+    if not (a.is_cuda and a.dtype == torch.bfloat16 and b_ok):
         raise _lib.PhotoverseB200Error("add_bias_nhwc: two CUDA bfloat16 tensors of one shape required (there is no CPU path)")
     if a.dim() == 4:
-        if not (a.is_contiguous(memory_format=torch.channels_last) and b.is_contiguous(memory_format=torch.channels_last)):
+        if not (a.is_contiguous(memory_format=torch.channels_last)
+                and (b is None or b.is_contiguous(memory_format=torch.channels_last))):
             raise _lib.PhotoverseB200Error("add_bias_nhwc: 4-D operands must be channels_last-contiguous")
         C = a.shape[1]
     else:
-        if not (a.is_contiguous() and b.is_contiguous()):
+        if not (a.is_contiguous() and (b is None or b.is_contiguous())):
             raise _lib.PhotoverseB200Error("add_bias_nhwc: operands must be contiguous")
         C = a.shape[-1]
     assert bias.dtype == torch.float32 and bias.is_contiguous() and bias.numel() == C
@@ -512,3 +517,22 @@
     dh = torch.empty_like(h)
     check(_lib.lib().pv_geglu_bwd(PV_BF16, _ptr(h), _ptr(dy), _ptr(dh), M, N, 2 * N, _stream()), "pv_geglu_bwd")
     return dh
+
+
+def linear_residual(x: torch.Tensor, w: torch.Tensor, b: Optional[torch.Tensor], r: torch.Tensor) -> torch.Tensor:
+    if not (x.is_cuda and x.dtype == torch.bfloat16 and x.is_contiguous() and r.dtype == x.dtype and r.is_contiguous()):
+        raise _lib.PhotoverseB200Error("linear_residual: contiguous CUDA bfloat16 input and residual required (there is no CPU path)")
+    if not (w.dtype == torch.bfloat16 and w.dim() == 2 and w.is_contiguous()):
+        raise _lib.PhotoverseB200Error("linear_residual: contiguous bfloat16 [N, K] weight required")
+    N, K = w.shape
+    if x.shape[-1] != K:
+        raise _lib.PhotoverseB200Error(f"linear_residual: input has {x.shape[-1]} features, the weight {K}")
+    if r.shape != (*x.shape[:-1], N):
+        raise _lib.PhotoverseB200Error(f"linear_residual: residual of shape {tuple(r.shape)}, expected {(*x.shape[:-1], N)}")
+    if b is not None and not (b.dtype == torch.float32 and b.is_contiguous() and b.numel() == N):
+        raise _lib.PhotoverseB200Error("linear_residual: contiguous float32 [N] bias required")
+    M = x.numel() // K
+    y = torch.empty(*x.shape[:-1], N, device=x.device, dtype=x.dtype)
+    check(_lib.lib().pv_linear_residual_fwd(PV_BF16, _ptr(x), _ptr(w), _ptr(b), _ptr(r), _ptr(y), M, N, K, K, N, N, _stream()),
+          "pv_linear_residual_fwd")
+    return y
```

After: 8.792 (median of 6 runs). 1.02x the previous value.
